# soedinglab/PEnG-motif

Measured on AMD Instinct MI355X. Metric: 4^W pattern z-scores/s + EM PWM-kmer evals/s at W=10; Gbp/s k-mer count, higher is better.
Workload: dtype u32 counts / f32 scores / f32 serial EM sums (f64 tree sums in the throughput EM mode)

## Files before the change

peng-motif_amd/csrc/api.hip:

```cpp
#include <stdarg.h>
#include <stdio.h>
#include <string.h>
#include <stdlib.h>
#include <time.h>

#include <new>

#include "pengk_internal.h"

namespace pengk {

static thread_local char g_err[512] = "";

int fail(int code, const char* fmt, ...) {
  va_list ap;
  va_start(ap, fmt);
  vsnprintf(g_err, sizeof g_err, fmt, ap);
  va_end(ap);
  return code;
}

int hip_fail(hipError_t e, const char* what) {
  return fail(PENGK_ERR_DEVICE, "%s: %s", what, hipGetErrorString(e));
}
// ... 64 lines not shown
  int n = 0;
  hipError_t e = hipGetDeviceCount(&n);
  lap("hipGetDeviceCount (runtime start)");
  if (e != hipSuccess || n <= 0)
    return fail(PENGK_ERR_DEVICE, "pengk_create: no HIP device (%s); this library has no CPU fallback",
                e == hipSuccess ? "device count 0" : hipGetErrorString(e));
  if (device < 0 || device >= n) return fail(PENGK_ERR_ARG, "pengk_create: device %d out of range [0,%d)", device, n);
  PENGK_HIP(hipSetDevice(device));
  hipDeviceProp_t prop;
  PENGK_HIP(hipGetDeviceProperties(&prop, device));
  lap("hipSetDevice + properties");
  if (strncmp(prop.gcnArchName, "gfx950", 6) != 0)
    return fail(PENGK_ERR_DEVICE, "pengk_create: device %d is %s; this build targets gfx950 only", device, prop.gcnArchName);
  pengk_ctx* c = new (std::nothrow) pengk_ctx();
  if (!c) return fail(PENGK_ERR_NOMEM, "pengk_create: out of host memory");
  c->device = device;
  c->num_cu = prop.multiProcessorCount;
  e = hipStreamCreateWithFlags(&c->stream, hipStreamNonBlocking);
  if (e != hipSuccess) {
    delete c;
    return hip_fail(e, "hipStreamCreate");
  }
  c->own_stream = true;
  lap("stream");
  int rc = count_init_device();
  lap("kernel attributes (code object load)");
  if (rc) {
    (void)hipStreamDestroy(c->stream);
    delete c;
    return rc;
  }
  *out = c;
  return PENGK_OK;
}

int pengk_destroy(pengk_ctx* ctx) {
  if (!ctx) return PENGK_OK;
  (void)hipSetDevice(ctx->device);
  (void)hipStreamSynchronize(ctx->stream);
  comm_release(ctx);
  if (ctx->d_defer) (void)hipFree(ctx->d_defer);
  if (ctx->d_em_partials) (void)hipFree(ctx->d_em_partials);
  if (ctx->d_em_tables) (void)hipFree(ctx->d_em_tables);
  if (ctx->d_em_blocks) (void)hipFree(ctx->d_em_blocks);
  if (ctx->d_em_counters) (void)hipFree(ctx->d_em_counters);
  if (ctx->d_em_look) (void)hipFree(ctx->d_em_look);
  if (ctx->d_pair_mids) (void)hipFree(ctx->d_pair_mids);
  for (int l = 0; l < 3; ++l) {
    if (ctx->em_streams[l]) (void)hipStreamDestroy(ctx->em_streams[l]);
    if (ctx->em_join[l]) (void)hipEventDestroy(ctx->em_join[l]);
  }
  if (ctx->em_fork) (void)hipEventDestroy(ctx->em_fork);
  if (ctx->d_misc) (void)hipFree(ctx->d_misc);
  if (ctx->d_keys) (void)hipFree(ctx->d_keys);
  if (ctx->d_iupac_big) (void)hipFree(ctx->d_iupac_big);
  if (ctx->d_bg_partials) (void)hipFree(ctx->d_bg_partials);
  if (ctx->d_count_aux) (void)hipFree(ctx->d_count_aux);
  if (ctx->d_sim) (void)hipFree(ctx->d_sim);
  if (ctx->d_score) (void)hipFree(ctx->d_score);
  if (ctx->d_sites) (void)hipFree(ctx->d_sites);
  if (ctx->own_stream && ctx->stream) (void)hipStreamDestroy(ctx->stream);
  delete ctx;
  return PENGK_OK;
}

int pengk_synchronize(pengk_ctx* ctx) {
  if (!ctx) return fail(PENGK_ERR_ARG, "ctx is NULL");
  PENGK_ENTER(ctx);
  PENGK_HIP(hipStreamSynchronize(ctx->stream));
  return PENGK_OK;
}

int pengk_set_option(pengk_ctx* ctx, const char* name, int64_t value) {
  if (!ctx || !name) return fail(PENGK_ERR_ARG, "pengk_set_option: NULL argument");
  if (strcmp(name, "count_impl") == 0) {
    if (value < 0 || value > 2) return fail(PENGK_ERR_ARG, "count_impl must be 0 (auto), 1 (direct) or 2 (partition)");
    ctx->count_impl = (int)value;
    return PENGK_OK;
  }
  if (strcmp(name, "key_cap_override") == 0) {
    ctx->key_cap_override = (uint64_t)value;
    return PENGK_OK;
  }
  if (strcmp(name, "em_fast") == 0) {
    if (value < 0 || value > 2) return fail(PENGK_ERR_ARG, "em_fast must be 0 (reference terms), 1 (fast) or 2 (serial, bit-exact)");
    ctx->em_fast = (int)value;
    return PENGK_OK;
  }
  if (strcmp(name, "em_serial_scan") == 0) {
    if (value < 2 || value > 3)
      return fail(PENGK_ERR_ARG, "em_serial_scan must be 2 (blocks evaluated ahead of their chain, three launches per iteration) or 3 (two: weights and block evaluation as one kernel); earlier generations: pengk_test_em_generation");
    ctx->em_serial_scan = (int)value;
    return PENGK_OK;
  }
  if (strcmp(name, "em_test_lookback") == 0) {
    if (value < 0 || value > 1000000) return fail(PENGK_ERR_ARG, "em_test_lookback must be 0 (off) or the n of 'every n-th workgroup'");
    ctx->em_test_lookback = (int)value;
    return PENGK_OK;
  }
  if (strcmp(name, "em_test_skew") == 0) {
    if (value < 0 || value > 1000000) return fail(PENGK_ERR_ARG, "em_test_skew must be 0 (off) or the n of 'every n-th block'");
    ctx->em_test_skew = (int)value;
    return PENGK_OK;
  }
  if (strcmp(name, "em_head_blocks") == 0) {
    if (value < 1 || value > 64) return PENGK_ERR_ARG;
    ctx->em_head_blocks = (int)value;
    return PENGK_OK;
  }
  if (strcmp(name, "sweep_pairs") == 0) {
    ctx->sweep_pairs = value != 0;
    return PENGK_OK;
  }
  if (strcmp(name, "em_lean_div") == 0) {
    ctx->em_lean_div = value != 0;
    return PENGK_OK;
  }
  if (strcmp(name, "em_overlap") == 0) {
    if (value < 1 || value > MAX_EM_LANES) return fail(PENGK_ERR_ARG, "em_overlap must be 1 .. %d streams", MAX_EM_LANES);
    ctx->em_overlap = (int)value;
    return PENGK_OK;
  }
  if (strcmp(name, "em_table_budget_mb") == 0) {
    if (value < 0) return fail(PENGK_ERR_ARG, "em_table_budget_mb must be >= 0 (0 = automatic)");
    ctx->em_table_budget_mb = (uint64_t)value;
    return PENGK_OK;
  }
  if (strcmp(name, "iupac_group_bytes") == 0) {
    ctx->iupac_group_bytes = (uint64_t)value;
    return PENGK_OK;
  }
  if (strcmp(name, "sites_record_budget") == 0) {
    if (value < 1) return fail(PENGK_ERR_ARG, "sites_record_budget must be >= 1 record");
    ctx->sites_record_budget = (uint64_t)value;
    return PENGK_OK;
  }
  if (strcmp(name, "scatter_blocks_per_cu") == 0) {
    if (value < 0 || value > 8) return fail(PENGK_ERR_ARG, "scatter_blocks_per_cu must be 0 (default) .. 8");
    ctx->scatter_blocks_per_cu = (int)value;
    return PENGK_OK;
  }
  if (strcmp(name, "n_windows_hint") == 0) {
    ctx->n_windows_hint = (uint64_t)value;
    return PENGK_OK;
  }
  return fail(PENGK_ERR_ARG, "unknown option '%s'", name);
}

int pengk_get_info(pengk_ctx* ctx, const char* name, int64_t* value) {
  if (!ctx || !name || !value) return fail(PENGK_ERR_ARG, "pengk_get_info: NULL argument");
  PENGK_ENTER(ctx);
  if (strcmp(name, "deferred_items") == 0) {
    uint32_t n = 0;
    if (ctx->d_defer) {
      PENGK_HIP(hipMemcpyAsync(&n, ctx->d_defer, sizeof n, hipMemcpyDeviceToHost, ctx->stream));
      PENGK_HIP(hipStreamSynchronize(ctx->stream));
    }
    *value = n;
    return PENGK_OK;
  }
  if (strcmp(name, "sites_record_budget") == 0) {
    *value = (int64_t)ctx->sites_record_budget;
    return PENGK_OK;
  }
  if (strcmp(name, "num_cu") == 0) {
    *value = ctx->num_cu;
    return PENGK_OK;
  }
  static const char* const em_names[4] = {"em_fetched_blocks", "em_mispredicted_blocks", "em_restaged_blocks", "em_restaged_waits"};
  for (int i = 0; i < 4; ++i)
    if (strcmp(name, em_names[i]) == 0) {
      unsigned long long v = 0;
      if (ctx->d_em_counters) {
        PENGK_HIP(hipMemcpyAsync(&v, ctx->d_em_counters + i, sizeof v, hipMemcpyDeviceToHost, ctx->stream));
        PENGK_HIP(hipStreamSynchronize(ctx->stream));
      }
      *value = (int64_t)v;
      return PENGK_OK;
    }
  return fail(PENGK_ERR_ARG, "unknown info '%s'", name);
}

void* pengk_stream(pengk_ctx* ctx) { return ctx ? (void*)ctx->stream : nullptr; }

int pengk_set_stream(pengk_ctx* ctx, void* s) {
  if (!ctx) return fail(PENGK_ERR_ARG, "ctx is NULL");
  PENGK_ENTER(ctx);
  PENGK_HIP(hipStreamSynchronize(ctx->stream));
  if (ctx->own_stream && ctx->stream) PENGK_HIP(hipStreamDestroy(ctx->stream));
  ctx->stream = (hipStream_t)s;
  ctx->own_stream = false;
  return PENGK_OK;
}

int pengk_malloc(pengk_ctx* ctx, size_t bytes, void** d_out) {
  if (!ctx || !d_out) return fail(PENGK_ERR_ARG, "pengk_malloc: NULL argument");
  PENGK_HIP(hipSetDevice(ctx->device));
  hipError_t e = hipMalloc(d_out, bytes ? bytes : 1);
  if (e != hipSuccess) return fail(PENGK_ERR_NOMEM, "hipMalloc(%zu): %s", bytes, hipGetErrorString(e));
  return PENGK_OK;
}

int pengk_free(pengk_ctx* ctx, void* d_ptr) {
  if (!ctx) return fail(PENGK_ERR_ARG, "ctx is NULL");
  PENGK_ENTER(ctx);
  if (d_ptr) {
    PENGK_HIP(hipStreamSynchronize(ctx->stream));
    PENGK_HIP(hipFree(d_ptr));
  }
  return PENGK_OK;
}

int pengk_host_alloc(pengk_ctx* ctx, size_t bytes, void** h_out) {
  if (!ctx || !h_out) return fail(PENGK_ERR_ARG, "pengk_host_alloc: NULL argument");
  PENGK_HIP(hipSetDevice(ctx->device));
  hipError_t e = hipHostMalloc(h_out, bytes ? bytes : 1, hipHostMallocDefault);
  if (e != hipSuccess) return fail(PENGK_ERR_NOMEM, "hipHostMalloc(%zu): %s", bytes, hipGetErrorString(e));
  return PENGK_OK;
}

int pengk_host_free(pengk_ctx* ctx, void* h_ptr) {
  if (!ctx) return fail(PENGK_ERR_ARG, "ctx is NULL");
  PENGK_ENTER(ctx);
  if (h_ptr) {
    PENGK_HIP(hipStreamSynchronize(ctx->stream));
    PENGK_HIP(hipHostFree(h_ptr));
  }
  return PENGK_OK;
}

int pengk_memcpy_h2d(pengk_ctx* ctx, void* d_dst, const void* h_src, size_t bytes) {
  if (!ctx || (bytes && (!d_dst || !h_src))) return fail(PENGK_ERR_ARG, "pengk_memcpy_h2d: NULL argument");
  PENGK_ENTER(ctx);
  PENGK_HIP(hipMemcpyAsync(d_dst, h_src, bytes, hipMemcpyHostToDevice, ctx->stream));
  PENGK_HIP(hipStreamSynchronize(ctx->stream));
  return PENGK_OK;
}

int pengk_warmup(pengk_ctx* ctx) {
  if (!ctx) return fail(PENGK_ERR_ARG, "ctx is NULL");
  PENGK_ENTER(ctx);
  constexpr size_t N = (size_t)4 << 20;
  void* d = nullptr;
  void* h = nullptr;
  hipError_t e = hipMalloc(&d, N);
  if (e == hipSuccess) e = hipHostMalloc(&h, N, hipHostMallocDefault);
  if (e == hipSuccess) e = hipMemcpyAsync(h, d, N, hipMemcpyDeviceToHost, ctx->stream);
  if (e == hipSuccess) e = hipStreamSynchronize(ctx->stream);
  if (h) (void)hipHostFree(h);
  if (d) (void)hipFree(d);
  if (e != hipSuccess) return hip_fail(e, "pengk_warmup");
  return warm_code_objects();
}

int pengk_memcpy_d2h(pengk_ctx* ctx, void* h_dst, const void* d_src, size_t bytes) {
  if (!ctx || (bytes && (!h_dst || !d_src))) return fail(PENGK_ERR_ARG, "pengk_memcpy_d2h: NULL argument");
  PENGK_ENTER(ctx);
  PENGK_HIP(hipMemcpyAsync(h_dst, d_src, bytes, hipMemcpyDeviceToHost, ctx->stream));
  PENGK_HIP(hipStreamSynchronize(ctx->stream));
  return PENGK_OK;
}

int pengk_memset(pengk_ctx* ctx, void* d_dst, int byte, size_t bytes) {
  if (!ctx || (bytes && !d_dst)) return fail(PENGK_ERR_ARG, "pengk_memset: NULL argument");
  PENGK_ENTER(ctx);
  PENGK_HIP(hipMemsetAsync(d_dst, byte, bytes, ctx->stream));
  return PENGK_OK;
}

int pengk_timer_create(pengk_ctx* ctx, void** out) {
  if (!ctx || !out) return fail(PENGK_ERR_ARG, "pengk_timer_create: NULL argument");
  PENGK_ENTER(ctx);
  hipEvent_t ev;
  PENGK_HIP(hipEventCreate(&ev));
  *out = (void*)ev;
  return PENGK_OK;
}
int pengk_timer_record(pengk_ctx* ctx, void* t) {
  if (!ctx || !t) return fail(PENGK_ERR_ARG, "pengk_timer_record: NULL argument");
  PENGK_ENTER(ctx);
  PENGK_HIP(hipEventRecord((hipEvent_t)t, ctx->stream));
  return PENGK_OK;
}
int pengk_timer_elapsed_ms(pengk_ctx* ctx, void* a, void* b, float* ms) {
  if (!ctx || !a || !b || !ms) return fail(PENGK_ERR_ARG, "pengk_timer_elapsed_ms: NULL argument");
  PENGK_ENTER(ctx);
  PENGK_HIP(hipEventSynchronize((hipEvent_t)b));
  PENGK_HIP(hipEventElapsedTime(ms, (hipEvent_t)a, (hipEvent_t)b));
  return PENGK_OK;
}
int pengk_timer_destroy(pengk_ctx* ctx, void* t) {
  (void)ctx;
  if (t) PENGK_HIP(hipEventDestroy((hipEvent_t)t));
  return PENGK_OK;
}

int pengk_set_sequences(pengk_ctx* ctx, const uint64_t* d_words, uint64_t n_words, const uint64_t* d_items,
                        uint64_t n_items, int W, int item_windows, uint64_t max_bin_bound, int all_whole) {
  if (!ctx) return fail(PENGK_ERR_ARG, "ctx is NULL");
  if (!valid_w(W)) return fail(PENGK_ERR_ARG, "pattern length %d unsupported (even, %d..%d)", W, PENGK_MIN_W, PENGK_MAX_W);
  if (item_windows < PENGK_MIN_ITEM_WINDOWS || item_windows > 65535)
    return fail(PENGK_ERR_ARG, "item_windows %d out of range [%d,65535]", item_windows, PENGK_MIN_ITEM_WINDOWS);
  if (!d_words || n_words < (PENGK_FRONT_PAD_BASES / 32) + 2) return fail(PENGK_ERR_ARG, "packed stream missing or too short");
  if (n_items && !d_items) return fail(PENGK_ERR_ARG, "items missing");
  if (n_items >= (1ull << 32)) return fail(PENGK_ERR_RANGE, "too many scan items for one shard (%llu)", (unsigned long long)n_items);
  ctx->d_words = d_words;
  ctx->n_words = n_words;
  ctx->d_items = d_items;
// ... 222 lines not shown
```

peng-motif_amd/csrc/count.hip:

```cpp
#include <stdlib.h>

#include <type_traits>

#include "pengk_internal.h"

namespace pengk {

namespace {

constexpr uint32_t INVALID_ID = 0xFFFFFFFFu;

__device__ __forceinline__ uint32_t funnel(uint32_t hi, uint32_t lo, uint32_t shift) {
  return __builtin_amdgcn_alignbit(hi, lo, shift);
}

template <int W>
struct Geo {
  static constexpr int P = ((3 * W - 3 + 15) / 16) * 16;
  static constexpr uint32_t MASK = (1u << (2 * W)) - 1u;
  static constexpr int TOP = 2 * (W - 1);
  static constexpr int PER = (32 - 2 * W) / 2 + 1;
  static constexpr int NVIEW = (W - 1 + PER - 1) / PER;
};

// ... 138 lines not shown
        const uint32_t hi = words32[wi + 1];
        ++wi;
        const uint32_t chunk = funnel(hi, lo, shift);
        lo = hi;
        pchunk = chunk;
#pragma unroll
        for (int u = 0; u < 16; ++u) {
          const int b = ch * 16 + u;
          const uint32_t c = (chunk >> (2 * u)) & 3u;
          id = (id >> 2) | (c << G::TOP);
          rc = ((rc << 2) & G::MASK) | (c ^ 3u);
          bgc.head(id, b - (G::P - (W - 1)), live && !cont && nw > 0);
          if (b >= W - 1) {
            const uint32_t can = BOTH ? min(id, rc) : id;
            bool match = false;
#pragma unroll
            for (int d = 1; d <= W - 1; ++d)
              if (b - d >= W - 1) match |= (can == ring[(u - d) & 15]);
            dirty |= match;
            ring[u] = (cont && !match) ? can : INVALID_ID;
          }
        }
      }
      if (cont && dirty) {
        const uint32_t slot = atomicAdd(&defer[0], 1u);
        defer[1 + slot] = it;
        nw = 0;
      }
    } else {
      wi += (G::P / 16) - 1;
      lo = words32[wi];
      const uint32_t hi = words32[wi + 1];
      ++wi;
      const uint32_t chunk = funnel(hi, lo, shift);
      lo = hi;
      pchunk = chunk;
#pragma unroll
      for (int u = 0; u < 16; ++u) {
        const uint32_t c = (chunk >> (2 * u)) & 3u;
        id = (id >> 2) | (c << G::TOP);
        rc = ((rc << 2) & G::MASK) | (c ^ 3u);
        bgc.head(id, u - (17 - W), live && nw > 0);
      }
    }

    const uint32_t nw_scan = BG ? nw_all : nw;
    uint32_t nw_max = nw_scan;
#pragma unroll
    for (int off = 32; off > 0; off >>= 1) nw_max = max(nw_max, (uint32_t)__shfl_xor((int)nw_max, off, 64));
    uint32_t nxt = (0u < nw_scan) ? words32[wi + 1] : 0u;
    uint32_t rprev = revcomp16(pchunk);
    for (uint32_t t0 = 0; t0 < nw_max; t0 += 16) {
      const uint32_t hi = nxt;
      ++wi;
      nxt = (t0 + 16u < nw_scan) ? words32[wi + 1] : 0u;
      const uint32_t chunk = funnel(hi, lo, shift);
      lo = hi;
      const uint32_t rchunk = BOTH ? revcomp16(chunk) : 0u;
      uint32_t view[G::NVIEW], rview[G::NVIEW];
#pragma unroll
      for (int j = 0; j < G::NVIEW; ++j) {
        view[j] = funnel(chunk, pchunk, 2u * (uint32_t)(j * G::PER + 17 - W));
        rview[j] = BOTH ? funnel(rprev, rchunk, 2u * (uint32_t)(j * G::PER + 17 - W)) : 0u;
      }
      auto body = [&](auto full_tag) {
        constexpr bool FULL = decltype(full_tag)::value;
#pragma unroll
        for (int u = 0; u < 16; ++u) {
          uint32_t id_u, rc_u = 0;
          if (u >= W - 1) {
            id_u = __builtin_amdgcn_ubfe(chunk, 2u * (uint32_t)(u - (W - 1)), 2u * W);
            if (BOTH) rc_u = __builtin_amdgcn_ubfe(rchunk, 2u * (uint32_t)(15 - u), 2u * W);
          } else {
            const int j = u / G::PER, k = W - 2 - u, jr = k / G::PER;
            id_u = __builtin_amdgcn_ubfe(view[j], 2u * (uint32_t)(u - j * G::PER), 2u * W);
            if (BOTH) rc_u = __builtin_amdgcn_ubfe(rview[jr], 2u * (uint32_t)(k - jr * G::PER), 2u * W);
          }
          const uint32_t can = BOTH ? min(id_u, rc_u) : id_u;
#ifdef PENGK_ABLATE_NOSUPPRESS
          const uint32_t key = can;
#else
          const uint32_t key = Suppress<W>::apply(can, ring, u);
#endif
          ring[u] = key;
          if (FULL) {
            if (BG && (u & 1)) {
              const uint32_t v4 = u >= 3 ? __builtin_amdgcn_ubfe(chunk, 2u * (uint32_t)(u - 3), 8u)
                                         : funnel(chunk, pchunk, 2u * (uint32_t)(13 + u)) & 0xFFu;
              bgc.kmer4(v4);
            }
            emit.full(key);
          } else {
            bgc.kmer3(id_u, t0 + (uint32_t)u < nw_all);
            emit.masked(key, key != INVALID_ID && t0 + (uint32_t)u < nw);
          }
        }
      };
      if (__all((t0 + 16u <= nw && nw == nw_all) ? 1 : 0)) body(std::true_type{});
      else body(std::false_type{});
      pchunk = chunk;
      rprev = rchunk;
    }
  }

#pragma unroll
  for (int off = 32; off > 0; off >>= 1) my_windows += __shfl_down(my_windows, off, 64);
  if ((threadIdx.x & 63u) == 0 && my_windows) atomicAdd(ltot, my_windows);
}

struct DirectEmit {
  uint32_t* __restrict__ hist;
  __device__ __forceinline__ void masked(uint32_t key, bool active) const {
    if (active) __hip_atomic_fetch_add(&hist[key], 1u, __ATOMIC_RELAXED, __HIP_MEMORY_SCOPE_AGENT);
  }
  __device__ __forceinline__ void full(uint32_t key) const { masked(key, key != INVALID_ID); }
};

template <int W, bool BOTH, bool BG>
__global__ __launch_bounds__(256) void count_kernel(const uint32_t* __restrict__ words32,
                                                    const uint64_t* __restrict__ items, uint32_t n_items,
                                                    uint32_t* __restrict__ hist,
                                                    unsigned long long* __restrict__ ltot,
                                                    uint32_t* __restrict__ defer, uint32_t* __restrict__ bg_partials) {
  bg_begin<BG>();
  if (BG) __syncthreads();
  DirectEmit e{hist};
  scan_items<W, BOTH, BG>(words32, items, n_items, ltot, defer, e);
  bg_end<BG>(bg_partials);
}

constexpr int RING_CAP = 128;
constexpr int GROUP = RING_CAP / 2;
constexpr uint32_t KEY_INVALID = 0xFFFFu;
constexpr int PAYLOAD_BITS = 15;

template <int W, int NBITS>
struct KeySplit {
  static constexpr int S = ((2 * W - NBITS) / 2) & ~1;
  static constexpr uint32_t LOW = (1u << S) - 1u;
  static constexpr uint32_t NB = 1u << NBITS;
  __host__ __device__ static inline uint32_t bucket(uint32_t id) { return (id >> S) & (NB - 1u); }
  __host__ __device__ static inline uint32_t payload(uint32_t id) {
#if defined(__HIP_DEVICE_COMPILE__)
    uint32_t r;
    asm("v_bfi_b32 %0, %1, %2, %3" : "=v"(r) : "s"(LOW), "v"(id), "v"(id >> NBITS));
    return r;
#else
    return (id & LOW) | ((id >> NBITS) & ~LOW);
#endif
  }
  __host__ __device__ static inline uint32_t join(uint32_t b, uint32_t p, uint32_t  = 0) {
    return (p & LOW) | (b << S) | ((p >> S) << (S + NBITS));
  }
  __host__ __device__ static inline bool valid(uint32_t p) { return p != KEY_INVALID; }
};

#ifndef PENGK_W12_L1_BITS
#define PENGK_W12_L1_BITS 4
#endif
struct Split12L1 {
  static constexpr int NBITS = PENGK_W12_L1_BITS;
  static constexpr uint32_t NB = 1u << NBITS;
  static constexpr uint32_t PBITS = 24 - NBITS;
  __host__ __device__ static inline uint32_t bucket(uint32_t id) { return (id >> 8) & (NB - 1u); }
  __host__ __device__ static inline uint32_t payload(uint32_t id) { return (id & 0xFFu) | ((id >> (8 + NBITS)) << 8); }
  __host__ __device__ static inline uint32_t join(uint32_t b1, uint32_t p1, uint32_t  = 0) { return (p1 & 0xFFu) | (b1 << 8) | ((p1 >> 8) << (8 + NBITS)); }
  __host__ __device__ static inline bool valid(uint32_t p1) { return p1 < (1u << PBITS); }
};
struct Split12L2 {
  static constexpr int NBITS = 9 - Split12L1::NBITS;
  static constexpr uint32_t NB = 1u << NBITS;
  __host__ __device__ static inline uint32_t bucket(uint32_t p1) { return (p1 >> 8) & (NB - 1u); }
  __host__ __device__ static inline uint32_t payload(uint32_t p1) { return (p1 & 0xFFu) | ((p1 >> (8 + NBITS)) << 8); }
  __host__ __device__ static inline uint32_t join(uint32_t b2, uint32_t p2, uint32_t outer) {
    const uint32_t p1 = (p2 & 0xFFu) | (b2 << 8) | ((p2 >> 8) << (8 + NBITS));
    return Split12L1::join(outer, p1);
  }
  __host__ __device__ static inline bool valid(uint32_t p2) { return p2 != KEY_INVALID; }
};

struct Split14L1 {
  static constexpr int NBITS = 4;
  static constexpr uint32_t NB = 16;
  __host__ __device__ static inline uint32_t bucket(uint32_t id) { return (id >> 10) & 15u; }
  __host__ __device__ static inline uint32_t payload(uint32_t id) { return (id & 0x3FFu) | ((id >> 14) << 10); }
  __host__ __device__ static inline uint32_t join(uint32_t b1, uint32_t p1, uint32_t  = 0) { return (p1 & 0x3FFu) | (b1 << 10) | ((p1 >> 10) << 14); }
  __host__ __device__ static inline bool valid(uint32_t p1) { return p1 < (1u << 24); }
};
struct Split14L2 {
  static constexpr int NBITS = 4;
  static constexpr uint32_t NB = 16;
  __host__ __device__ static inline uint32_t bucket(uint32_t p1) { return (p1 >> 9) & 15u; }
  __host__ __device__ static inline uint32_t payload(uint32_t p1) { return (p1 & 0x1FFu) | ((p1 >> 13) << 9); }
  __host__ __device__ static inline uint32_t join(uint32_t b2, uint32_t p2, uint32_t outer) {
    return Split14L1::join(outer, (p2 & 0x1FFu) | (b2 << 9) | ((p2 >> 9) << 13));
  }
  __host__ __device__ static inline bool valid(uint32_t p2) { return p2 < (1u << 20); }
};
struct Split14L3 {
  static constexpr int NBITS = 5;
  static constexpr uint32_t NB = 32;
  __host__ __device__ static inline uint32_t bucket(uint32_t p2) { return (p2 >> 8) & 31u; }
  __host__ __device__ static inline uint32_t payload(uint32_t p2) { return (p2 & 0xFFu) | ((p2 >> 13) << 8); }
  __host__ __device__ static inline uint32_t join(uint32_t b3, uint32_t p3, uint32_t outer) {
    return Split14L2::join(outer & 15u, (p3 & 0xFFu) | (b3 << 8) | ((p3 >> 8) << 13), outer >> 4);
  }
  __host__ __device__ static inline bool valid(uint32_t p3) { return p3 != KEY_INVALID; }
};

template <class E>
struct ScatterRowT {
  E ring[RING_CAP];
  uint32_t fill4;
};
typedef ScatterRowT<uint16_t> ScatterRow;
template <int NBITS, int WPW, class E = uint16_t>
struct ScatterShared {
  static constexpr int NB = 1 << NBITS;
  ScatterRowT<E> row[WPW][NB];
};

template <int NBITS, int WPW, class E = uint16_t>
__device__ __forceinline__ ScatterShared<NBITS, WPW, E>& scatter_lds() {
  __shared__ ScatterShared<NBITS, WPW, E> sh;
  return sh;
}

template <class KS, int NBITS, int WPW = 4, class E = uint16_t>
struct ScatterEmit {
  static constexpr int NB = 1 << NBITS;
  static constexpr uint32_t ES = (uint32_t)sizeof(E);
  static constexpr uint32_t ESH = ES == 2u ? 1u : 2u;
  static constexpr uint32_t PAD = ES == 2u ? KEY_INVALID : 0xFFFFFFFFu;
  typedef ScatterRowT<E> Row;
  static_assert(GROUP == 64, "a group is one entry per lane");
  static_assert(RING_CAP == 128, "byte 0 of the counter addresses the ring");
  E* __restrict__ keys;
  uint32_t slice_cap;
  uint32_t* __restrict__ slice_fill;
  uint32_t* __restrict__ hist;
  uint32_t wave, lane, wave_global;
  uint32_t outer;

  static __device__ __forceinline__ void init_lds() {
    ScatterShared<NBITS, WPW, E>& sh = scatter_lds<NBITS, WPW, E>();
    static_assert(sizeof(Row) == ES * RING_CAP + 4, "row = ring + counter");
    uint32_t* w = reinterpret_cast<uint32_t*>(&sh.row[0][0]);
    for (uint32_t i = threadIdx.x; i < (uint32_t)WPW * NB * (sizeof(Row) / 4u); i += blockDim.x)
      w[i] = (i % (uint32_t)(sizeof(Row) / 4u)) == (uint32_t)(ES * RING_CAP / 4u) ? 0u : 0xFFFFFFFFu;
  }

  typedef __attribute__((address_space(3))) uint32_t lds_u32_t;
  typedef __attribute__((address_space(3))) E lds_e_t;
  typedef __attribute__((address_space(1))) E global_e_t;

  __device__ __forceinline__ void flush_triggered(unsigned long long trig, uint32_t row, uint32_t b, uint32_t s4) {
    asm volatile("");
    const uint32_t g4 = s4 - 4u * (uint32_t)(GROUP - 1);
    const uint32_t src = row + ((g4 >> (2u - ESH)) & (ES * (uint32_t)GROUP));
    const uint32_t dst = b * (ES * slice_cap) + (g4 >> (2u - ESH));
    const unsigned long long fits = __builtin_amdgcn_ballot_w64(g4 + 4u * GROUP <= 4u * slice_cap);
    unsigned long long todo = trig & fits;
    unsigned long long over = trig & ~fits;
    while (todo) {
      const int p = __builtin_ctzll(todo);
      todo &= todo - 1;
      const uint32_t s_src = (uint32_t)__builtin_amdgcn_readlane((int)src, p);
      const uint32_t s_dst = (uint32_t)__builtin_amdgcn_readlane((int)dst, p);
      uint32_t v = *(lds_e_t*)(uintptr_t)(s_src + ES * lane);
      asm volatile("" : "+v"(v));
      global_e_t* out = (global_e_t*)((char*)region + s_dst);
      __builtin_nontemporal_store((E)v, &out[lane]);
    }
    while (over) {
      const int p = __builtin_ctzll(over);
      over &= over - 1;
      const uint32_t s_src = (uint32_t)__builtin_amdgcn_readlane((int)src, p);
      const uint32_t fb = (uint32_t)__builtin_amdgcn_readlane((int)b, p);
      const uint32_t v = *(lds_e_t*)(uintptr_t)(s_src + ES * lane);
      if (KS::valid(v)) __hip_atomic_fetch_add(&hist[KS::join(fb, v, outer)], 1u, __ATOMIC_RELAXED, __HIP_MEMORY_SCOPE_AGENT);
    }
  }

  uint32_t rowbase = 0;
  __device__ __forceinline__ void bind() {
    rowbase = (uint32_t)(uintptr_t)(__attribute__((address_space(3))) char*)&scatter_lds<NBITS, WPW, E>().row[wave][0];
    asm volatile("" : "+v"(rowbase));
    region = keys + (size_t)wave_global * NB * slice_cap;
  }
  E* region = nullptr;

  __device__ __forceinline__ uint32_t append(uint32_t b, uint32_t key, uint32_t& row) const {
    row = b * (uint32_t)sizeof(Row) + rowbase;
    const uint32_t s4 = __hip_atomic_fetch_add((lds_u32_t*)(uintptr_t)(row + ES * RING_CAP), 4u, __ATOMIC_RELAXED,
                                               __HIP_MEMORY_SCOPE_WORKGROUP);
    *(lds_e_t*)(uintptr_t)(row + ((s4 >> (2u - ESH)) & (ES * RING_CAP - 1u))) = (E)KS::payload(key);
    return s4;
  }

  __device__ __forceinline__ void full(uint32_t key) {
    const uint32_t b = KS::bucket(key);
    uint32_t row;
    const uint32_t s4 = append(b, key, row);
    const unsigned long long trig = __builtin_amdgcn_ballot_w64((s4 & 0xFFu) == 4u * (uint32_t)(GROUP - 1));
    if (trig) flush_triggered(trig, row, b, s4);
  }

  __device__ __forceinline__ void masked(uint32_t key, bool active) {
    const uint32_t b = KS::bucket(key);
    uint32_t s4 = 0, row = 0;
    if (active) s4 = append(b, key, row);
    const unsigned long long trig = __builtin_amdgcn_ballot_w64(active && (s4 & 0xFFu) == 4u * (uint32_t)(GROUP - 1));
    if (trig) flush_triggered(trig, row, b, s4);
  }

  __device__ __forceinline__ void drain() {
    __builtin_amdgcn_wave_barrier();
    uint32_t row = 0, s4_last = 0;
    bool padded = false;
    if (lane < (uint32_t)NB) {
      row = lane * (uint32_t)sizeof(Row) + rowbase;
      const uint32_t c4 = __hip_atomic_load((lds_u32_t*)(uintptr_t)(row + ES * RING_CAP), __ATOMIC_RELAXED, __HIP_MEMORY_SCOPE_WAVEFRONT);
      const uint32_t r = (c4 >> 2) & (uint32_t)(GROUP - 1);
      if (r) {
        for (uint32_t i = r; i < (uint32_t)GROUP; ++i)
          *(lds_e_t*)(uintptr_t)(row + (((c4 >> (2u - ESH)) & (ES * RING_CAP - 1u)) + ES * (i - r))) = (E)PAD;
        s4_last = c4 + 4u * ((uint32_t)GROUP - r) - 4u;
        padded = true;
      }
      const uint32_t full = ((c4 >> 2) + (uint32_t)(GROUP - 1)) & ~(uint32_t)(GROUP - 1);
      slice_fill[(size_t)wave_global * NB + lane] = full < slice_cap ? full : slice_cap;
    }
    __builtin_amdgcn_wave_barrier();
    const unsigned long long trig = __builtin_amdgcn_ballot_w64(padded);
    if (trig) flush_triggered(trig, row, lane, s4_last);
  }
};

#ifndef PENGK_SCATTER_WPW
#define PENGK_SCATTER_WPW 4
#endif
constexpr int SCATTER_WPW = PENGK_SCATTER_WPW;
template <int W, bool BOTH, int NBITS, bool BG>
__global__ __launch_bounds__(64 * SCATTER_WPW) void count_scatter_kernel(const uint32_t* __restrict__ words32,
                                                            const uint64_t* __restrict__ items, uint32_t n_items,
                                                            uint16_t* __restrict__ keys, uint32_t slice_cap,
                                                            uint32_t* __restrict__ slice_fill, uint32_t* __restrict__ hist,
                                                            unsigned long long* __restrict__ ltot,
                                                            uint32_t* __restrict__ defer,
                                                            uint32_t* __restrict__ bg_partials) {
  static_assert(2 * W - NBITS == PAYLOAD_BITS, "payload must be 15 bits");
  ScatterEmit<KeySplit<W, NBITS>, NBITS, SCATTER_WPW>::init_lds();
  bg_begin<BG>();
  __syncthreads();
  const uint32_t wave = (uint32_t)__builtin_amdgcn_readfirstlane((int)(threadIdx.x >> 6));
  ScatterEmit<KeySplit<W, NBITS>, NBITS, SCATTER_WPW> e{keys, slice_cap, slice_fill, hist, wave, threadIdx.x & 63u, blockIdx.x * (uint32_t)SCATTER_WPW + wave, 0u};
  e.bind();
  scan_items<W, BOTH, BG>(words32, items, n_items, ltot, defer, e);
  e.drain();
  bg_end<BG>(bg_partials);
}

#ifndef PENGK_SCATTER12_WPW
#define PENGK_SCATTER12_WPW 3
#endif
constexpr int SCATTER12_WPW = PENGK_SCATTER12_WPW;
#ifndef PENGK_SCATTER12L1_WPW
#define PENGK_SCATTER12L1_WPW (PENGK_W12_L1_BITS == 5 ? 3 : 4)
#endif
constexpr int SCATTER12L1_WPW = PENGK_SCATTER12L1_WPW;
typedef ScatterEmit<Split12L1, Split12L1::NBITS, SCATTER12L1_WPW, uint32_t> Scatter12Emit;

template <bool BOTH, bool BG>
__global__ __launch_bounds__(64 * SCATTER12L1_WPW) void count_scatter12_kernel(const uint32_t* __restrict__ words32,
                                                              const uint64_t* __restrict__ items, uint32_t n_items,
                                                              uint32_t* __restrict__ keys, uint32_t slice_cap,
                                                              uint32_t* __restrict__ slice_fill, uint32_t* __restrict__ hist,
                                                              unsigned long long* __restrict__ ltot,
                                                              uint32_t* __restrict__ defer, uint32_t* __restrict__ bg_partials) {
  Scatter12Emit::init_lds();
  bg_begin<BG>();
  __syncthreads();
  const uint32_t wave = (uint32_t)__builtin_amdgcn_readfirstlane((int)(threadIdx.x >> 6));
  Scatter12Emit e{keys, slice_cap, slice_fill, hist, wave, threadIdx.x & 63u, blockIdx.x * (uint32_t)SCATTER12L1_WPW + wave, 0u};
  e.bind();
  scan_items<12, BOTH, BG>(words32, items, n_items, ltot, defer, e);
  e.drain();
  bg_end<BG>(bg_partials);
}

__global__ __launch_bounds__(256) void count_rescatter12_kernel(const uint32_t* __restrict__ keys1, uint32_t cap1,
                                                                const uint32_t* __restrict__ fill1, uint32_t n_slices1,
                                                                uint32_t bpb1, uint16_t* __restrict__ keys2, uint32_t cap2,
                                                                uint32_t* __restrict__ fill2, uint32_t* __restrict__ hist) {
  ScatterEmit<Split12L2, Split12L2::NBITS>::init_lds();
  __syncthreads();
  const uint32_t b1 = blockIdx.x / bpb1, j = blockIdx.x % bpb1;
  const uint32_t wave = (uint32_t)__builtin_amdgcn_readfirstlane((int)(threadIdx.x >> 6)), lane = threadIdx.x & 63u;
  ScatterEmit<Split12L2, Split12L2::NBITS> e{keys2, cap2, fill2, hist, wave, lane, blockIdx.x * 4u + wave, b1};
  e.bind();
  const uint32_t per = (n_slices1 + bpb1 - 1) / bpb1;
  const uint32_t first = j * per, last = min(n_slices1, first + per);
  for (uint32_t s = first + wave; s < last; s += 4) {
    const uint32_t n = fill1[(size_t)s * Split12L1::NB + b1];
    const uint32_t* src = keys1 + ((size_t)s * Split12L1::NB + b1) * cap1;
    typedef uint32_t u4 __attribute__((ext_vector_type(4)));
    const u4 pad = {0xFFFFFFFFu, 0xFFFFFFFFu, 0xFFFFFFFFu, 0xFFFFFFFFu};
    const u4* src4 = reinterpret_cast<const u4*>(src);
    const uint32_t n4 = n / 4u;
    u4 nxt = lane < n4 ? __builtin_nontemporal_load(&src4[lane]) : pad;
    for (uint32_t i = 0; i < n4; i += 64) {
      const u4 k = nxt;
      nxt = (i + 64u + lane < n4) ? __builtin_nontemporal_load(&src4[i + 64u + lane]) : pad;
      e.full(k.x);
      e.full(k.y);
      e.full(k.z);
      e.full(k.w);
    }
  }
  e.drain();
}

typedef ScatterEmit<Split14L1, Split14L1::NBITS, SCATTER12L1_WPW, uint32_t> Scatter14Emit;

template <bool BOTH, bool BG>
__global__ __launch_bounds__(64 * SCATTER12L1_WPW) void count_scatter14_kernel(const uint32_t* __restrict__ words32,
                                                              const uint64_t* __restrict__ items, uint32_t n_items,
                                                              uint32_t* __restrict__ keys, uint32_t slice_cap,
                                                              uint32_t* __restrict__ slice_fill, uint32_t* __restrict__ hist,
                                                              unsigned long long* __restrict__ ltot,
                                                              uint32_t* __restrict__ defer, uint32_t* __restrict__ bg_partials) {
  Scatter14Emit::init_lds();
  bg_begin<BG>();
  __syncthreads();
  const uint32_t wave = (uint32_t)__builtin_amdgcn_readfirstlane((int)(threadIdx.x >> 6));
  Scatter14Emit e{keys, slice_cap, slice_fill, hist, wave, threadIdx.x & 63u, blockIdx.x * (uint32_t)SCATTER12L1_WPW + wave, 0u};
  e.bind();
  scan_items<14, BOTH, BG>(words32, items, n_items, ltot, defer, e);
  e.drain();
  bg_end<BG>(bg_partials);
}

template <class KS, class E_OUT, uint32_t NB_IN>
__global__ __launch_bounds__(256) void count_rescatter_kernel(const uint32_t* __restrict__ keys_in, uint32_t cap_in,
                                                              const uint32_t* __restrict__ fill_in, uint32_t n_slices_in,
                                                              uint32_t slices_per_group, uint32_t bpb, E_OUT* __restrict__ keys_out,
                                                              uint32_t cap_out, uint32_t* __restrict__ fill_out,
                                                              uint32_t* __restrict__ hist) {
  typedef ScatterEmit<KS, KS::NBITS, 4, E_OUT> Emit;
  Emit::init_lds();
  __syncthreads();
  const uint32_t o = blockIdx.x / bpb, j = blockIdx.x % bpb;
  const uint32_t b_in = slices_per_group ? o % NB_IN : o;
  const uint32_t slice0 = slices_per_group ? (o / NB_IN) * slices_per_group : 0u;
  const uint32_t n_in = slices_per_group ? slices_per_group : n_slices_in;
  const uint32_t wave = (uint32_t)__builtin_amdgcn_readfirstlane((int)(threadIdx.x >> 6)), lane = threadIdx.x & 63u;
  Emit e{keys_out, cap_out, fill_out, hist, wave, lane, blockIdx.x * 4u + wave, o};
  e.bind();
  const uint32_t per = (n_in + bpb - 1) / bpb;
  const uint32_t first = j * per, last = min(n_in, first + per);
  for (uint32_t t = first + wave; t < last; t += 4) {
    const uint32_t sl = slice0 + t;
    const uint32_t n = fill_in[(size_t)sl * NB_IN + b_in];
    typedef uint32_t u4 __attribute__((ext_vector_type(4)));
    const u4 pad = {0xFFFFFFFFu, 0xFFFFFFFFu, 0xFFFFFFFFu, 0xFFFFFFFFu};
    const u4* src4 = reinterpret_cast<const u4*>(keys_in + ((size_t)sl * NB_IN + b_in) * cap_in);
    const uint32_t n4 = n / 4u;
    u4 nxt = lane < n4 ? __builtin_nontemporal_load(&src4[lane]) : pad;
    for (uint32_t i = 0; i < n4; i += 64) {
      const u4 k = nxt;
      nxt = (i + 64u + lane < n4) ? __builtin_nontemporal_load(&src4[i + 64u + lane]) : pad;
      e.full(k.x);
      e.full(k.y);
      e.full(k.z);
      e.full(k.w);
    }
  }
  e.drain();
}

__global__ __launch_bounds__(256) void count_gather14_kernel(const uint32_t* __restrict__ temp, uint32_t* __restrict__ hist) {
  const uint32_t np = 1u << 28;
  for (uint32_t x = blockIdx.x * blockDim.x + threadIdx.x; x < np; x += gridDim.x * blockDim.x) {
    const uint32_t p1 = Split14L1::payload(x), p2 = Split14L2::payload(p1);
    const uint32_t fb = (Split14L1::bucket(x) * Split14L2::NB + Split14L2::bucket(p1)) * Split14L3::NB + Split14L3::bucket(p2);
    const uint32_t v = temp[((size_t)fb << PAYLOAD_BITS) | Split14L3::payload(p2)];
    if (v) hist[x] += v;
  }
}

__global__ __launch_bounds__(1024) void count_hist_kernel(const uint16_t* __restrict__ keys, uint32_t slice_cap,
                                                          uint32_t n_slices, uint32_t nb,
                                                          const uint32_t* __restrict__ slice_fill, uint32_t bpb,
                                                          uint32_t* __restrict__ temp, uint32_t slices_per_outer) {
  extern __shared__ uint32_t h[];
  const uint32_t f = blockIdx.x / bpb, j = blockIdx.x % bpb;
  const uint32_t b = slices_per_outer ? f % nb : f;
  const uint32_t slice0 = slices_per_outer ? (f / nb) * slices_per_outer : 0u;
  if (slices_per_outer) n_slices = slices_per_outer;
  for (uint32_t i = threadIdx.x; i < (1u << PAYLOAD_BITS); i += blockDim.x) h[i] = 0;
  __syncthreads();
  const uint32_t per = (n_slices + bpb - 1) / bpb;
  const uint32_t first = slice0 + j * per, last = slice0 + min(n_slices, j * per + per);
  const uint32_t wave = threadIdx.x >> 6, lane = threadIdx.x & 63u;
  uint32_t fill_next = first + wave < last ? slice_fill[(size_t)(first + wave) * nb + b] : 0u;
  for (uint32_t s = first + wave; s < last; s += 16) {
    const uint32_t n8 = fill_next >> 3;
    if (s + 16 < last) fill_next = slice_fill[(size_t)(s + 16) * nb + b];
    const uint4* src = reinterpret_cast<const uint4*>(keys + ((size_t)s * nb + b) * slice_cap);
    auto count8 = [&](const uint4& v) {
      const uint32_t k[8] = {v.x & 0xFFFFu, v.x >> 16, v.y & 0xFFFFu, v.y >> 16, v.z & 0xFFFFu, v.z >> 16, v.w & 0xFFFFu, v.w >> 16};
#pragma unroll
      for (int q = 0; q < 8; ++q)
        if (k[q] < (1u << PAYLOAD_BITS)) atomicAdd(&h[k[q]], 1u);
    };
    uint32_t i = lane;
    for (; i + 448 < n8; i += 512) {
      uint4 v[8];
#pragma unroll
      for (int q = 0; q < 8; ++q) {
        typedef uint32_t u32x4 __attribute__((ext_vector_type(4)));
        const u32x4 t = __builtin_nontemporal_load(reinterpret_cast<const u32x4*>(&src[i + 64 * q]));
        v[q] = make_uint4(t.x, t.y, t.z, t.w);
      }
#pragma unroll
      for (int q = 0; q < 8; ++q) count8(v[q]);
    }
    if (i < n8) {
      uint4 v[7];
#pragma unroll
      for (int q = 0; q < 7; ++q) {
        typedef uint32_t u32x4 __attribute__((ext_vector_type(4)));
        const u32x4 ones = {0xFFFFFFFFu, 0xFFFFFFFFu, 0xFFFFFFFFu, 0xFFFFFFFFu};
        const u32x4 t = i + 64u * q < n8 ? __builtin_nontemporal_load(reinterpret_cast<const u32x4*>(&src[i + 64 * q])) : ones;
        v[q] = make_uint4(t.x, t.y, t.z, t.w);
      }
#pragma unroll
      for (int q = 0; q < 7; ++q) count8(v[q]);
    }
  }
  __syncthreads();
  uint32_t* dst = temp + ((size_t)f << PAYLOAD_BITS);
  for (uint32_t i = threadIdx.x; i < (1u << PAYLOAD_BITS); i += blockDim.x) {
    const uint32_t v = h[i];
    if (v) __hip_atomic_fetch_add(&dst[i], v, __ATOMIC_RELAXED, __HIP_MEMORY_SCOPE_AGENT);
  }
}

__global__ __launch_bounds__(256) void count_gather12_kernel(const uint32_t* __restrict__ temp, uint32_t* __restrict__ hist) {
  const uint32_t np = 1u << 24;
  for (uint32_t x = blockIdx.x * blockDim.x + threadIdx.x; x < np; x += gridDim.x * blockDim.x) {
    const uint32_t p1 = Split12L1::payload(x);
    const uint32_t fb = Split12L1::bucket(x) * Split12L2::NB + Split12L2::bucket(p1);
    const uint32_t v = temp[((size_t)fb << PAYLOAD_BITS) | Split12L2::payload(p1)];
    if (v) hist[x] += v;
  }
}

template <int W, int NBITS>
__global__ __launch_bounds__(256) void count_gather_kernel(const uint32_t* __restrict__ temp, uint32_t np,
                                                           uint32_t* __restrict__ hist) {
  using KS = KeySplit<W, NBITS>;
  for (uint32_t x = blockIdx.x * blockDim.x + threadIdx.x; x < np; x += gridDim.x * blockDim.x) {
    const uint32_t v = temp[((size_t)KS::bucket(x) << PAYLOAD_BITS) | KS::payload(x)];
    if (v) hist[x] += v;
  }
}

__device__ __forceinline__ uint32_t base_at(const uint32_t* __restrict__ words32, uint64_t g) {
  return (words32[g >> 4] >> (2u * (uint32_t)(g & 15u))) & 3u;
}

__global__ __launch_bounds__(64) void count_fixup_kernel(const uint32_t* __restrict__ words32,
                                                         const uint64_t* __restrict__ items, int W, int both,
                                                         uint32_t* __restrict__ hist,
                                                         const uint32_t* __restrict__ defer) {
  const uint32_t n = defer[0];
  const uint32_t mask = (1u << (2 * W)) - 1u;
  const int top = 2 * (W - 1);
  for (uint32_t q = blockIdx.x * blockDim.x + threadIdx.x; q < n; q += gridDim.x * blockDim.x) {
    const uint32_t it = defer[1 + q];
    const uint64_t rec = items[it];
    const uint32_t nw = (uint32_t)((rec >> ITEM_NW_SHIFT) & ITEM_NW_MASK);
    const uint64_t ws = rec & ITEM_WS_MASK;
    uint32_t j = it;
    while ((items[j] >> ITEM_CONT_SHIFT) & 1ull) --j;
    const uint64_t head = items[j] & ITEM_WS_MASK;
    uint64_t back = 8ull * (uint64_t)(W - 1);
    for (;;) {
      const uint64_t p0 = (ws - head > back) ? ws - back : head;
      bool certified = (p0 == head);
      uint32_t ring[16];
      for (int i = 0; i < 16; ++i) ring[i] = INVALID_ID;
      uint32_t id = 0, rc = 0;
      for (int b = 0; b < W - 1; ++b) {
        const uint32_t c = base_at(words32, p0 + b);
        id = (id >> 2) | (c << top);
        rc = ((rc << 2) & mask) | (c ^ 3u);
      }
      uint32_t clean = 0;
      bool ok = true;
      for (uint64_t t = p0; t < ws + nw; ++t) {
        const uint32_t c = base_at(words32, t + (uint64_t)(W - 1));
        id = (id >> 2) | (c << top);
        rc = ((rc << 2) & mask) | (c ^ 3u);
        const uint32_t can = both ? min(id, rc) : id;
        bool match = false;
        for (int d = 1; d <= W - 1; ++d) match |= (ring[(uint32_t)(t - d) & 15u] == can);
        if (t < ws) {
          clean = match ? 0u : clean + 1u;
          if (clean >= 2u * (uint32_t)(W - 1)) certified = true;
        } else {
          if (!certified) {
            ok = false;
            break;
          }
          if (!match) __hip_atomic_fetch_add(&hist[can], 1u, __ATOMIC_RELAXED, __HIP_MEMORY_SCOPE_AGENT);
        }
        ring[(uint32_t)t & 15u] = match ? INVALID_ID : can;
      }
      if (ok) break;
      back *= 4ull;
    }
  }
}

__global__ __launch_bounds__(256) void mirror_kernel(uint32_t* __restrict__ hist, int W, uint32_t np) {
  for (uint32_t x = blockIdx.x * blockDim.x + threadIdx.x; x < np; x += gridDim.x * blockDim.x) {
    const uint32_t r = revcomp32(x, W);
    if (x > r) hist[x] = hist[r];
  }
}

__global__ __launch_bounds__(256) void bg_count_kernel(const uint32_t* __restrict__ words32,
                                                       const uint64_t* __restrict__ items, uint32_t n_items, int W,
                                                       unsigned long long* __restrict__ out ) {
  __shared__ uint32_t h3[64][65];
  __shared__ uint32_t hfirst[20];
  for (int i = threadIdx.x; i < 64 * 65; i += blockDim.x) (&h3[0][0])[i] = 0;
  if (threadIdx.x < 20) hfirst[threadIdx.x] = 0;
  __syncthreads();
  const uint32_t col = threadIdx.x & 63u;
  for (uint32_t it = blockIdx.x * blockDim.x + threadIdx.x; it < n_items; it += gridDim.x * blockDim.x) {
    const uint64_t rec = items[it];
    const uint32_t nw = (uint32_t)((rec >> ITEM_NW_SHIFT) & ITEM_NW_MASK);
    const uint64_t ws = rec & ITEM_WS_MASK;
    const bool cont = ((rec >> ITEM_CONT_SHIFT) & 1ull) != 0;
    const bool last = (it + 1 == n_items) || (((items[it + 1] >> ITEM_CONT_SHIFT) & 1ull) == 0);
    const uint32_t nb = nw + (last ? (uint32_t)(W - 1) : 0u);
    uint32_t y = 0;
    uint32_t pos = 2;
    if (cont) {
      y = (base_at(words32, ws - 2) << 2) | base_at(words32, ws - 1);
    } else {
      pos = 0;
    }
    for (uint32_t b = 0; b < nb; ++b) {
      const uint32_t c = base_at(words32, ws + b);
      y = ((y << 2) | c) & 63u;
      if (pos >= 2) {
        atomicAdd(&h3[y][col], 1u);
      } else if (pos == 1) {
        atomicAdd(&hfirst[4 + (y & 15u)], 1u);
        pos = 2;
      } else {
        atomicAdd(&hfirst[c], 1u);
        pos = 1;
      }
    }
  }
  __syncthreads();
  if (threadIdx.x < 64) {
    unsigned long long s = 0;
    for (int i = 0; i < 64; ++i) s += h3[threadIdx.x][i];
    if (s) atomicAdd(&out[threadIdx.x], s);
  } else if (threadIdx.x < 84) {
    const uint32_t v = hfirst[threadIdx.x - 64];
    if (v) atomicAdd(&out[threadIdx.x], (unsigned long long)v);
  }
}

__global__ void bg_finish_kernel(const unsigned long long* __restrict__ raw, unsigned long long* __restrict__ out) {
  const int t = threadIdx.x;
  __shared__ unsigned long long n2[16];
  if (t < 16) {
    unsigned long long s = raw[64 + 4 + t];
    for (int c = 0; c < 4; ++c) s += raw[c * 16 + t];
    n2[t] = s;
    out[4 + t] = s;
  }
  __syncthreads();
  if (t < 4) {
    unsigned long long s = raw[64 + t];
    for (int b = 0; b < 4; ++b) s += n2[b * 4 + t];
    out[t] = s;
  }
  if (t < 64) out[20 + t] = raw[t];
}

__global__ void bg_finish_fused_kernel(const uint32_t* __restrict__ partials, uint32_t n_blocks,
                                       unsigned long long* __restrict__ out) {
  __shared__ unsigned long long raw[84];
  __shared__ unsigned long long n3[64];
  __shared__ unsigned long long n2[16];
  __shared__ unsigned long long part[12][84];
  const int t = threadIdx.x;
  {
    const int bin = t % 84, strand = t / 84;
    if (strand < 12) {
      unsigned long long acc[8] = {0, 0, 0, 0, 0, 0, 0, 0};
      uint32_t b = strand;
      for (; b + 31u * 12u < n_blocks; b += 32u * 12u) {
        uint32_t v[32];
#pragma unroll
        for (uint32_t j = 0; j < 32u; ++j) v[j] = partials[(size_t)(b + 12u * j) * 84 + bin];
#pragma unroll
        for (uint32_t j = 0; j < 32u; ++j) acc[j & 7u] += v[j];
      }
      for (; b < n_blocks; b += 12) acc[0] += partials[(size_t)b * 84 + bin];
      part[strand][bin] = ((acc[0] + acc[1]) + (acc[2] + acc[3])) + ((acc[4] + acc[5]) + (acc[6] + acc[7]));
    }
  }
  __syncthreads();
  if (t < 84) {
    unsigned long long s = 0;
    for (int k = 0; k < 12; ++k) s += part[k][t];
    raw[t] = s;
  }
  __syncthreads();
  if (t < 64) {
    const int d0 = t >> 4, d1 = (t >> 2) & 3, d2 = t & 3;
    n3[t] = raw[d0 | (d1 << 2) | (d2 << 4)];
    out[20 + t] = n3[t];
  }
  __syncthreads();
  if (t < 16) {
    const int a = t >> 2, b = t & 3;
    unsigned long long s = raw[68 + (a | (b << 2))];
    for (int c = 0; c < 4; ++c) s += n3[c * 16 + t];
    n2[t] = s;
    out[4 + t] = s;
  }
  __syncthreads();
  if (t < 4) {
    unsigned long long s = raw[64 + t];
    for (int b = 0; b < 4; ++b) s += n2[b * 4 + t];
    out[t] = s;
  }
}

__global__ __launch_bounds__(128) void bg_model_kernel(const unsigned long long* __restrict__ n, int K, float a0, float a1, float a2,
                                                       float* __restrict__ V) {
  __shared__ float cnt[84];
  __shared__ float v[84];
  const int t = threadIdx.x;
  const float alpha[3] = {a0, a1, a2};
  const int off[3] = {0, 4, 20};
  if (t < 84) cnt[t] = (float)n[t];
  __shared__ float base_f;
  if (t == 0) {
    unsigned long long base_counts = 0;
    for (int y = 0; y < 4; ++y) base_counts += n[y];
    base_f = (float)base_counts;
  }
  __syncthreads();
  if (t < 4) v[t] = (cnt[t] + alpha[0] * 0.25f) / (base_f + alpha[0]);
  __syncthreads();
  for (int k = 1; k <= K; ++k) {
    const int ny = 1 << (2 * (k + 1));
    const int yk = 1 << (2 * k);
    if (t < ny) v[off[k] + t] = (cnt[off[k] + t] + alpha[k] * v[off[k - 1] + t % yk]) / (cnt[off[k - 1] + t / 4] + alpha[k]);
    __syncthreads();
    if (t < ny / 4) {
      float* g = v + off[k] + 4 * t;
      float factor = 0.0f;
      for (int a = 0; a < 4; ++a) factor += g[a];
      for (int a = 0; a < 4; ++a) g[a] /= factor;
    }
    __syncthreads();
  }
  const int used = off[K] + (1 << (2 * (K + 1)));
  if (t < 84) V[t] = t < used ? v[t] : 0.0f;
}

__device__ __forceinline__ uint64_t mix64(uint64_t x) {
  x ^= x >> 30;
  x *= 0xBF58476D1CE4E5B9ull;
  x ^= x >> 27;
  x *= 0x94D049BB133111EBull;
  x ^= x >> 31;
  return x;
}

__global__ __launch_bounds__(256) void synth_words_kernel(uint64_t seed, uint64_t seq0, uint64_t n_seq, uint32_t L,
                                                          uint64_t* __restrict__ words, uint64_t n_words) {
  const uint64_t motif = 2ull | (1ull << 2) | (3ull << 4) | (2ull << 6) | (0ull << 8) | (2ull << 10) | (3ull << 12) |
                         (1ull << 14) | (0ull << 16) | (3ull << 18);
  const uint64_t total = n_seq * (uint64_t)L;
  for (uint64_t w = blockIdx.x * (uint64_t)blockDim.x + threadIdx.x; w < n_words; w += (uint64_t)gridDim.x * blockDim.x) {
    uint64_t v = 0;
    for (int k = 0; k < 32; ++k) {
      const uint64_t g = w * 32 + k;
      if (g < PENGK_FRONT_PAD_BASES) continue;
      const uint64_t li = g - PENGK_FRONT_PAD_BASES;
      if (li >= total) break;
      const uint64_t n = seq0 + li / L;
      const uint32_t j = (uint32_t)(li % L);
      uint64_t d = mix64(seed + 0x9E3779B97F4A7C15ull * (n * (uint64_t)L + j + 1)) >> 62;
      if (L >= 10 && mix64(seed ^ 0xA5A5A5A5ull ^ (n + 1)) % 10 == 0) {
        const uint64_t q = mix64(seed ^ 0x5A5A5A5Aull ^ (n + 1)) % (L - 9);
        if (j >= q && j < q + 10) d = (motif >> (2 * (j - q))) & 3ull;
      }
      v |= d << (2 * k);
    }
    words[w] = v;
  }
}

__global__ __launch_bounds__(256) void synth_items_kernel(uint64_t n_seq, uint32_t L, int W, uint32_t M,
                                                          uint64_t* __restrict__ items) {
  const uint64_t nwin = (uint64_t)L - W + 1;
  const uint64_t per = (nwin + M - 1) / M;
  const uint64_t n = n_seq * per;
  for (uint64_t i = blockIdx.x * (uint64_t)blockDim.x + threadIdx.x; i < n; i += (uint64_t)gridDim.x * blockDim.x) {
    const uint64_t s = i / per;
    const uint64_t f = (i % per) * M;
    const uint64_t nw = nwin - f < M ? nwin - f : M;
    items[i] = (PENGK_FRONT_PAD_BASES + s * L + f) | (nw << ITEM_NW_SHIFT) | ((uint64_t)(f ? 1 : 0) << ITEM_CONT_SHIFT);
  }
}

#define PENGK_LAUNCH_BB(KERNEL, TARGS, both, bg, grid, block, ...)                                              \
  do {                                                                                                         \
    if (both) {                                                                                                \
      if (bg) hipLaunchKernelGGL((KERNEL<TARGS(true, true)>), grid, block, 0, ctx->stream, __VA_ARGS__);        \
      else hipLaunchKernelGGL((KERNEL<TARGS(true, false)>), grid, block, 0, ctx->stream, __VA_ARGS__);          \
    } else {                                                                                                   \
      if (bg) hipLaunchKernelGGL((KERNEL<TARGS(false, true)>), grid, block, 0, ctx->stream, __VA_ARGS__);       \
      else hipLaunchKernelGGL((KERNEL<TARGS(false, false)>), grid, block, 0, ctx->stream, __VA_ARGS__);         \
    }                                                                                                          \
  } while (0)

int bg_partials_buffer(pengk_ctx* ctx, uint32_t blocks, uint32_t** out) {
  int rc = ensure_scratch(ctx, &ctx->d_bg_partials, &ctx->bg_partials_bytes, (size_t)blocks * 84 * sizeof(uint32_t));
  *out = (uint32_t*)ctx->d_bg_partials;
  return rc;
}

int bg_finish_fused(pengk_ctx* ctx, uint32_t blocks, uint64_t* d_bg) {
  hipLaunchKernelGGL(bg_finish_fused_kernel, dim3(1), dim3(1024), 0, ctx->stream, (const uint32_t*)ctx->d_bg_partials, blocks,
                     (unsigned long long*)d_bg);
  PENGK_HIP(hipGetLastError());
  return PENGK_OK;
}

template <int W>
int launch_direct_w(pengk_ctx* ctx, int both, uint32_t* d_counts, uint64_t* d_ltot, uint32_t n_items, uint64_t* d_bg) {
  const uint32_t* w32 = (const uint32_t*)ctx->d_words;
  const uint32_t blocks_needed = (n_items + 255) / 256;
  const uint32_t max_blocks = (uint32_t)ctx->num_cu * 8u;
  const uint32_t blocks = blocks_needed < max_blocks ? blocks_needed : max_blocks;
  unsigned long long* lt = (unsigned long long*)d_ltot;
  uint32_t* bgp = nullptr;
  if (d_bg) {
    int rc = bg_partials_buffer(ctx, blocks, &bgp);
    if (rc) return rc;
  }
#define TA_DIRECT(B, G) W, B, G
  PENGK_LAUNCH_BB(count_kernel, TA_DIRECT, both, d_bg != nullptr, dim3(blocks), dim3(256), w32, ctx->d_items, n_items, d_counts,
                  lt, ctx->d_defer, bgp);
#undef TA_DIRECT
  PENGK_HIP(hipGetLastError());
  return d_bg ? bg_finish_fused(ctx, blocks, d_bg) : PENGK_OK;
}

template <int W>
int launch_partition_w(pengk_ctx* ctx, int both, uint32_t* d_counts, uint64_t* d_ltot, uint32_t n_items, uint64_t* d_bg) {
  constexpr int NBITS = 2 * W - PAYLOAD_BITS;
  constexpr uint32_t NB = 1u << NBITS;
  const uint32_t np = 1u << (2 * W);
  const uint32_t* w32 = (const uint32_t*)ctx->d_words;
  constexpr uint32_t TPB = 64u * SCATTER_WPW;
  const uint32_t blocks_needed = (n_items + TPB - 1) / TPB;
  constexpr uint32_t lds_per_wg = (uint32_t)(sizeof(ScatterShared<NBITS, SCATTER_WPW>) + sizeof(BgLds) + 511u) & ~511u;
  const uint32_t per_cu = ctx->scatter_blocks_per_cu ? (uint32_t)ctx->scatter_blocks_per_cu : (160u * 1024u) / lds_per_wg;
  const uint32_t max_blocks = (uint32_t)ctx->num_cu * per_cu;
  const uint32_t blocks = blocks_needed < max_blocks ? blocks_needed : max_blocks;
  const uint32_t n_waves = blocks * (uint32_t)SCATTER_WPW;
  uint64_t windows = ctx->n_windows_hint ? ctx->n_windows_hint : ctx->n_items * (uint64_t)ctx->item_windows;
  const uint64_t share = windows / ((uint64_t)NB * n_waves);
  uint64_t cap64 = share + share / 2 + 512;
  if (ctx->key_cap_override) cap64 = ctx->key_cap_override;
  cap64 = (cap64 + 63) / 64 * 64;
  if (cap64 * NB >= (1ull << 31))
    return fail(PENGK_ERR_RANGE, "shard too large for the partitioned count (slice of %llu keys)", (unsigned long long)cap64);
  const uint32_t slice_cap = (uint32_t)cap64;
  int rc = ensure_scratch(ctx, &ctx->d_keys, &ctx->keys_bytes, (size_t)NB * n_waves * slice_cap * sizeof(uint16_t));
  if (rc) return rc;
  const size_t fill_words = ((size_t)NB * n_waves + 63) / 64 * 64;
  const size_t aux_need = fill_words * sizeof(uint32_t) + (size_t)np * sizeof(uint32_t);
  rc = ensure_scratch(ctx, &ctx->d_count_aux, &ctx->count_aux_bytes, aux_need);
  if (rc) return rc;
  uint32_t* slice_fill = (uint32_t*)ctx->d_count_aux;
  uint32_t* temp = slice_fill + fill_words;
  PENGK_HIP(hipMemsetAsync(ctx->d_count_aux, 0, aux_need, ctx->stream));
  unsigned long long* lt = (unsigned long long*)d_ltot;
  uint16_t* keys = (uint16_t*)ctx->d_keys;
  uint32_t* bgp = nullptr;
  if (d_bg) {
    rc = bg_partials_buffer(ctx, blocks, &bgp);
    if (rc) return rc;
  }
#define TA_SCATTER(B, G) W, B, NBITS, G
  PENGK_LAUNCH_BB(count_scatter_kernel, TA_SCATTER, both, d_bg != nullptr, dim3(blocks), dim3(TPB), w32, ctx->d_items, n_items,
                  keys, slice_cap, slice_fill, d_counts, lt, ctx->d_defer, bgp);
#undef TA_SCATTER
  PENGK_HIP(hipGetLastError());
  if (d_bg) {
    rc = bg_finish_fused(ctx, blocks, d_bg);
    if (rc) return rc;
  }
  uint32_t bpb = ((uint32_t)ctx->num_cu * 2u + NB - 1) / NB;
  const uint64_t per_bucket = windows / NB + 1;
  const uint32_t useful = (uint32_t)((per_bucket + 65535) / 65536);
  if (bpb > useful) bpb = useful;
  if (bpb > n_waves) bpb = n_waves;
  if (bpb < 1) bpb = 1;
  hipLaunchKernelGGL(count_hist_kernel, dim3(NB * bpb), dim3(1024), 4 << PAYLOAD_BITS, ctx->stream, keys, slice_cap, n_waves,
                     NB, slice_fill, bpb, temp, 0u);
  PENGK_HIP(hipGetLastError());
  const uint32_t gb = (np + 255) / 256 < 2048u ? (np + 255) / 256 : 2048u;
  hipLaunchKernelGGL((count_gather_kernel<W, NBITS>), dim3(gb), dim3(256), 0, ctx->stream, temp, np, d_counts);
  PENGK_HIP(hipGetLastError());
  return PENGK_OK;
}

int launch_partition12(pengk_ctx* ctx, int both, uint32_t* d_counts, uint64_t* d_ltot, uint32_t n_items, uint64_t* d_bg) {
  const uint32_t np = 1u << 24;
  const uint32_t* w32 = (const uint32_t*)ctx->d_words;
  constexpr uint32_t TPB1 = 64u * SCATTER12L1_WPW;
  constexpr uint32_t NB1 = Split12L1::NB, NB2 = Split12L2::NB;
  const uint32_t blocks_needed = (n_items + TPB1 - 1) / TPB1;
  constexpr uint32_t lds_per_wg1 = (uint32_t)(sizeof(ScatterShared<Split12L1::NBITS, SCATTER12L1_WPW, uint32_t>) + sizeof(BgLds) + 511u) & ~511u;
  const uint32_t max_blocks = (uint32_t)ctx->num_cu * ((160u * 1024u) / lds_per_wg1);
  const uint32_t blocks1 = blocks_needed < max_blocks ? blocks_needed : max_blocks;
  const uint32_t n_waves1 = blocks1 * (uint32_t)SCATTER12L1_WPW;
  const uint64_t windows = ctx->n_windows_hint ? ctx->n_windows_hint : ctx->n_items * (uint64_t)ctx->item_windows;
  uint64_t share1 = windows / ((uint64_t)NB1 * n_waves1);
  uint64_t cap1_64 = share1 + share1 / 2 + 256;
  if (ctx->key_cap_override) cap1_64 = ctx->key_cap_override;
  cap1_64 = (cap1_64 + 63) / 64 * 64;
  uint32_t bpb1 = ((uint32_t)ctx->num_cu * 8u + NB1 - 1u) / NB1;
  if (bpb1 > n_waves1) bpb1 = n_waves1;
  if (bpb1 < 1) bpb1 = 1;
  const uint32_t blocks2 = NB1 * bpb1;
  const uint32_t n_waves2 = blocks2 * 4u;
  uint64_t share2 = windows / ((uint64_t)NB2 * n_waves2);
  uint64_t cap2_64 = share2 + share2 / 2 + 512;
  if (ctx->key_cap_override) cap2_64 = ctx->key_cap_override;
  cap2_64 = (cap2_64 + 63) / 64 * 64;
  if (cap1_64 * NB1 >= (1ull << 30) || cap2_64 * NB2 >= (1ull << 31)) return fail(
      PENGK_ERR_RANGE, "shard too large for the partitioned count");
  const uint32_t cap1 = (uint32_t)cap1_64, cap2 = (uint32_t)cap2_64;
  const size_t bytes1 = (size_t)n_waves1 * NB1 * cap1 * sizeof(uint32_t);
  const size_t bytes2 = (size_t)n_waves2 * NB2 * cap2 * sizeof(uint16_t);
  int rc = ensure_scratch(ctx, &ctx->d_keys, &ctx->keys_bytes, bytes1 + bytes2);
  if (rc) return rc;
  uint32_t* keys1 = (uint32_t*)ctx->d_keys;
  uint16_t* keys2 = (uint16_t*)((char*)ctx->d_keys + bytes1);
  const size_t fill1_words = ((size_t)n_waves1 * NB1 + 63) / 64 * 64, fill2_words = ((size_t)n_waves2 * NB2 + 63) / 64 * 64;
  const size_t aux_need = (fill1_words + fill2_words + (size_t)np) * sizeof(uint32_t);
  rc = ensure_scratch(ctx, &ctx->d_count_aux, &ctx->count_aux_bytes, aux_need);
  if (rc) return rc;
  uint32_t* fill1 = (uint32_t*)ctx->d_count_aux;
  uint32_t* fill2 = fill1 + fill1_words;
  uint32_t* temp = fill2 + fill2_words;
  PENGK_HIP(hipMemsetAsync(ctx->d_count_aux, 0, aux_need, ctx->stream));
  unsigned long long* lt = (unsigned long long*)d_ltot;
  uint32_t* bgp = nullptr;
  if (d_bg) {
    rc = bg_partials_buffer(ctx, blocks1, &bgp);
    if (rc) return rc;
  }
#define TA_S12(B, G) B, G
  PENGK_LAUNCH_BB(count_scatter12_kernel, TA_S12, both, d_bg != nullptr, dim3(blocks1), dim3(TPB1), w32, ctx->d_items, n_items, keys1,
                  cap1, fill1, d_counts, lt, ctx->d_defer, bgp);
#undef TA_S12
  PENGK_HIP(hipGetLastError());
  if (d_bg) {
    rc = bg_finish_fused(ctx, blocks1, d_bg);
    if (rc) return rc;
  }
  hipLaunchKernelGGL(count_rescatter12_kernel, dim3(blocks2), dim3(256), 0, ctx->stream, keys1, cap1, fill1, n_waves1, bpb1, keys2,
                     cap2, fill2, d_counts);
  PENGK_HIP(hipGetLastError());
  hipLaunchKernelGGL(count_hist_kernel, dim3(512), dim3(1024), 4 << PAYLOAD_BITS, ctx->stream, keys2, cap2, n_waves2, NB2, fill2, 1u,
                     temp, bpb1 * 4u);
  PENGK_HIP(hipGetLastError());
  hipLaunchKernelGGL(count_gather12_kernel, dim3(4096), dim3(256), 0, ctx->stream, temp, d_counts);
  PENGK_HIP(hipGetLastError());
  return PENGK_OK;
}

int launch_partition14(pengk_ctx* ctx, int both, uint32_t* d_counts, uint64_t* d_ltot, uint32_t n_items, uint64_t* d_bg) {
  const size_t np = (size_t)1 << 28;
  const uint32_t* w32 = (const uint32_t*)ctx->d_words;
  constexpr uint32_t TPB1 = 64u * SCATTER12L1_WPW;
  constexpr uint32_t NB1 = Split14L1::NB, NB2 = Split14L2::NB, NB3 = Split14L3::NB;
  static_assert(NB1 * NB2 * NB3 == 8192, "2^13 LDS histograms");
  const uint32_t blocks_needed = (n_items + TPB1 - 1) / TPB1;
  constexpr uint32_t lds_per_wg1 = (uint32_t)(sizeof(ScatterShared<Split14L1::NBITS, SCATTER12L1_WPW, uint32_t>) + sizeof(BgLds) + 511u) & ~511u;
  const uint32_t max_blocks = (uint32_t)ctx->num_cu * ((160u * 1024u) / lds_per_wg1);
  const uint32_t blocks1 = blocks_needed < max_blocks ? blocks_needed : max_blocks;
  const uint32_t n_waves1 = blocks1 * (uint32_t)SCATTER12L1_WPW;
  const uint64_t windows = ctx->n_windows_hint ? ctx->n_windows_hint : ctx->n_items * (uint64_t)ctx->item_windows;
  auto cap_of = [&](uint64_t slices, uint64_t slack) {
    uint64_t c = windows / slices;
    c = c + c / 2 + slack;
    if (ctx->key_cap_override) c = ctx->key_cap_override;
    return (c + 63) / 64 * 64;
  };
  uint32_t bpb1 = ((uint32_t)ctx->num_cu * 8u + NB1 - 1u) / NB1;
  if (bpb1 > n_waves1) bpb1 = n_waves1;
  if (bpb1 < 1) bpb1 = 1;
  const uint32_t blocks2 = NB1 * bpb1, n_waves2 = blocks2 * 4u;
  uint32_t bpb2 = ((uint32_t)ctx->num_cu * 8u + NB1 * NB2 - 1u) / (NB1 * NB2);
  if (bpb2 > bpb1 * 4u) bpb2 = bpb1 * 4u;
  if (bpb2 < 1) bpb2 = 1;
  const uint32_t blocks3 = NB1 * NB2 * bpb2, n_waves3 = blocks3 * 4u;
  const uint64_t cap1_64 = cap_of((uint64_t)NB1 * n_waves1, 256), cap2_64 = cap_of((uint64_t)NB2 * n_waves2, 256), cap3_64 = cap_of((uint64_t)NB3 * n_waves3, 256);
  if (cap1_64 * NB1 >= (1ull << 30) || cap2_64 * NB2 >= (1ull << 30) || cap3_64 * NB3 >= (1ull << 31))
    return fail(PENGK_ERR_RANGE, "shard too large for the partitioned count");
  const uint32_t cap1 = (uint32_t)cap1_64, cap2 = (uint32_t)cap2_64, cap3 = (uint32_t)cap3_64;
  const size_t bytes1 = (size_t)n_waves1 * NB1 * cap1 * sizeof(uint32_t);
  const size_t bytes2 = (size_t)n_waves2 * NB2 * cap2 * sizeof(uint32_t);
  const size_t bytes3 = (size_t)n_waves3 * NB3 * cap3 * sizeof(uint16_t);
  int rc = ensure_scratch(ctx, &ctx->d_keys, &ctx->keys_bytes, bytes1 + bytes2 + bytes3);
  if (rc) return rc;
  uint32_t* keys1 = (uint32_t*)ctx->d_keys;
  uint32_t* keys2 = (uint32_t*)((char*)ctx->d_keys + bytes1);
  uint16_t* keys3 = (uint16_t*)((char*)ctx->d_keys + bytes1 + bytes2);
  const size_t f1 = ((size_t)n_waves1 * NB1 + 63) / 64 * 64, f2 = ((size_t)n_waves2 * NB2 + 63) / 64 * 64,
               f3 = ((size_t)n_waves3 * NB3 + 63) / 64 * 64;
  const size_t aux_need = (f1 + f2 + f3 + np) * sizeof(uint32_t);
  rc = ensure_scratch(ctx, &ctx->d_count_aux, &ctx->count_aux_bytes, aux_need);
  if (rc) return rc;
  uint32_t* fill1 = (uint32_t*)ctx->d_count_aux;
  uint32_t* fill2 = fill1 + f1;
  uint32_t* fill3 = fill2 + f2;
  uint32_t* temp = fill3 + f3;
  PENGK_HIP(hipMemsetAsync(ctx->d_count_aux, 0, aux_need, ctx->stream));
  unsigned long long* lt = (unsigned long long*)d_ltot;
  uint32_t* bgp = nullptr;
  if (d_bg) {
    rc = bg_partials_buffer(ctx, blocks1, &bgp);
    if (rc) return rc;
  }
#define TA_S14(B, G) B, G
  PENGK_LAUNCH_BB(count_scatter14_kernel, TA_S14, both, d_bg != nullptr, dim3(blocks1), dim3(TPB1), w32, ctx->d_items, n_items, keys1,
                  cap1, fill1, d_counts, lt, ctx->d_defer, bgp);
#undef TA_S14
  PENGK_HIP(hipGetLastError());
  if (d_bg) {
    rc = bg_finish_fused(ctx, blocks1, d_bg);
    if (rc) return rc;
  }
  hipLaunchKernelGGL((count_rescatter_kernel<Split14L2, uint32_t, NB1>), dim3(blocks2), dim3(256), 0, ctx->stream, keys1, cap1, fill1,
                     n_waves1, 0u, bpb1, keys2, cap2, fill2, d_counts);
  PENGK_HIP(hipGetLastError());
  hipLaunchKernelGGL((count_rescatter_kernel<Split14L3, uint16_t, NB2>), dim3(blocks3), dim3(256), 0, ctx->stream, keys2, cap2, fill2,
                     n_waves2, bpb1 * 4u, bpb2, keys3, cap3, fill3, d_counts);
  PENGK_HIP(hipGetLastError());
  hipLaunchKernelGGL(count_hist_kernel, dim3(8192), dim3(1024), 4 << PAYLOAD_BITS, ctx->stream, keys3, cap3, n_waves3, NB3, fill3, 1u,
                     temp, bpb2 * 4u);
  PENGK_HIP(hipGetLastError());
  hipLaunchKernelGGL(count_gather14_kernel, dim3(8192), dim3(256), 0, ctx->stream, temp, d_counts);
  PENGK_HIP(hipGetLastError());
  return PENGK_OK;
}

template <int W>
int launch_count_w(pengk_ctx* ctx, int both, uint32_t* d_counts, uint64_t* d_ltot, uint64_t* d_bg) {
  const uint32_t n_items = (uint32_t)ctx->n_items;
  if (n_items == 0) {
    if (d_bg) PENGK_HIP(hipMemsetAsync(d_bg, 0, 84 * sizeof(uint64_t), ctx->stream));
    return PENGK_OK;
  }
  if constexpr (W < 4) {
    if (d_bg) {
      const int rc_bg = launch_bg_count(ctx, d_bg);
      if (rc_bg) return rc_bg;
      d_bg = nullptr;
    }
  }
  int impl = ctx->count_impl;
  constexpr bool can_partition = (W == 8 || W == 10 || W == 12 || W == 14);
  if (impl == 0) impl = can_partition ? 2 : 1;
  if (impl == 2 && !can_partition) return fail(PENGK_ERR_UNSUPPORTED, "partitioned count is built for W = 8 .. 14 only");
  int rc;
  if constexpr (W == 14) {
    rc = impl == 2 ? launch_partition14(ctx, both, d_counts, d_ltot, n_items, d_bg)
                   : launch_direct_w<W>(ctx, both, d_counts, d_ltot, n_items, d_bg);
  } else if constexpr (W == 12) {
    rc = impl == 2 ? launch_partition12(ctx, both, d_counts, d_ltot, n_items, d_bg)
                   : launch_direct_w<W>(ctx, both, d_counts, d_ltot, n_items, d_bg);
  } else if constexpr (can_partition) {
    rc = impl == 2 ? launch_partition_w<W>(ctx, both, d_counts, d_ltot, n_items, d_bg)
                   : launch_direct_w<W>(ctx, both, d_counts, d_ltot, n_items, d_bg);
  } else {
    rc = launch_direct_w<W>(ctx, both, d_counts, d_ltot, n_items, d_bg);
  }
  if (rc) return rc;
  hipLaunchKernelGGL(count_fixup_kernel, dim3(64), dim3(64), 0, ctx->stream, (const uint32_t*)ctx->d_words, ctx->d_items, W,
                     both, d_counts, ctx->d_defer);
  PENGK_HIP(hipGetLastError());
  return PENGK_OK;
}

}

int count_init_device() {
  PENGK_HIP(hipFuncSetAttribute((const void*)count_hist_kernel, hipFuncAttributeMaxDynamicSharedMemorySize, 4 << PAYLOAD_BITS));
  return PENGK_OK;
}

int launch_count(pengk_ctx* ctx, int both, uint32_t* d_counts, uint64_t* d_ltot, uint64_t* d_bg) {
  const int W = ctx->W;
  const size_t np = (size_t)1 << (2 * W);
  {
    const size_t need = (ctx->n_items + 2) * sizeof(uint32_t);
    size_t have = ctx->defer_cap * sizeof(uint32_t);
    if (have < need) {
      int rc = ensure_scratch(ctx, (void**)&ctx->d_defer, &have, need);
      if (rc) return rc;
      ctx->defer_cap = have / sizeof(uint32_t);
    }
  }
  PENGK_HIP(hipMemsetAsync(ctx->d_defer, 0, sizeof(uint32_t), ctx->stream));
  PENGK_HIP(hipMemsetAsync(d_counts, 0, np * sizeof(uint32_t), ctx->stream));
  PENGK_HIP(hipMemsetAsync(d_ltot, 0, sizeof(uint64_t), ctx->stream));
  switch (W) {
    case 2: return launch_count_w<2>(ctx, both, d_counts, d_ltot, d_bg);
    case 4: return launch_count_w<4>(ctx, both, d_counts, d_ltot, d_bg);
    case 6: return launch_count_w<6>(ctx, both, d_counts, d_ltot, d_bg);
    case 8: return launch_count_w<8>(ctx, both, d_counts, d_ltot, d_bg);
    case 10: return launch_count_w<10>(ctx, both, d_counts, d_ltot, d_bg);
    case 12: return launch_count_w<12>(ctx, both, d_counts, d_ltot, d_bg);
    case 14: return launch_count_w<14>(ctx, both, d_counts, d_ltot, d_bg);
    default: return fail(PENGK_ERR_ARG, "pattern length %d unsupported", W);
  }
}

int launch_mirror(pengk_ctx* ctx, int W, uint32_t* d_counts) {
  const uint32_t np = 1u << (2 * W);
  const uint32_t blocks = (np + 255) / 256 < 4096u ? (np + 255) / 256 : 4096u;
  hipLaunchKernelGGL(mirror_kernel, dim3(blocks), dim3(256), 0, ctx->stream, d_counts, W, np);
  PENGK_HIP(hipGetLastError());
  return PENGK_OK;
}

int launch_bg_count(pengk_ctx* ctx, uint64_t* d_bg) {
  int rc = ensure_scratch(ctx, &ctx->d_misc, &ctx->misc_bytes, 84 * sizeof(uint64_t));
  if (rc) return rc;
  unsigned long long* raw = (unsigned long long*)ctx->d_misc;
  PENGK_HIP(hipMemsetAsync(raw, 0, 84 * sizeof(uint64_t), ctx->stream));
  const uint32_t n_items = (uint32_t)ctx->n_items;
  if (n_items) {
    const uint32_t need = (n_items + 255) / 256;
    const uint32_t blocks = need < (uint32_t)ctx->num_cu * 4u ? need : (uint32_t)ctx->num_cu * 4u;
    hipLaunchKernelGGL(bg_count_kernel, dim3(blocks), dim3(256), 0, ctx->stream, (const uint32_t*)ctx->d_words,
                       ctx->d_items, n_items, ctx->W, raw);
    PENGK_HIP(hipGetLastError());
  }
  hipLaunchKernelGGL(bg_finish_kernel, dim3(1), dim3(64), 0, ctx->stream, raw, (unsigned long long*)d_bg);
  PENGK_HIP(hipGetLastError());
  return PENGK_OK;
}

int launch_bg_model(pengk_ctx* ctx, const uint64_t* d_bg, int K, const float* h_alpha, float* d_V) {
  hipLaunchKernelGGL(bg_model_kernel, dim3(1), dim3(128), 0, ctx->stream, (const unsigned long long*)d_bg, K, h_alpha[0],
                     h_alpha[1], h_alpha[2], d_V);
  PENGK_HIP(hipGetLastError());
  return PENGK_OK;
}

int launch_synth(pengk_ctx* ctx, uint64_t seed, uint64_t seq0, uint64_t n_seq, uint32_t L, int W, int item_windows,
                 uint64_t* d_words, uint64_t* d_items) {
  uint64_t nw = 0, ni = 0;
  int rc = pengk_synth_sizes(n_seq, L, W, item_windows, &nw, &ni);
  if (rc) return rc;
  hipLaunchKernelGGL(synth_words_kernel, dim3(4096), dim3(256), 0, ctx->stream, seed, seq0, n_seq, L, d_words, nw);
  PENGK_HIP(hipGetLastError());
  if (ni) {
    hipLaunchKernelGGL(synth_items_kernel, dim3(2048), dim3(256), 0, ctx->stream, n_seq, L, W, (uint32_t)item_windows, d_items);
    PENGK_HIP(hipGetLastError());
  }
  return PENGK_OK;
}

}
```

peng-motif_amd/csrc/em.hip:

```cpp
#include "em_serial.h"

namespace pengk {
namespace {
#ifdef PENGK_WG_TRACE
constexpr unsigned WG_TRACE_MAX = 1u << 20;
__device__ unsigned long long g_wg_trace[3 * WG_TRACE_MAX];
__device__ unsigned g_wg_trace_n;
struct WgTrace {
  unsigned long long t0;
  unsigned kernel;
  __device__ __forceinline__ WgTrace(unsigned k) : t0(__builtin_amdgcn_s_memrealtime()), kernel(k) {}
  __device__ __forceinline__ void end(unsigned kind, unsigned wg) const {
    if (threadIdx.x != 0) return;
    const unsigned long long t1 = __builtin_amdgcn_s_memrealtime();
    const unsigned xcc = __builtin_amdgcn_s_getreg((4 << 11) | (0 << 6) | 20) & 0xFu;
    const unsigned i = atomicAdd(&g_wg_trace_n, 1u);
    if (i < WG_TRACE_MAX) {
      g_wg_trace[3 * i] = ((unsigned long long)kernel << 56) | ((unsigned long long)kind << 48) | ((unsigned long long)xcc << 40) | wg;
      g_wg_trace[3 * i + 1] = t0;
      g_wg_trace[3 * i + 2] = t1;
    }
  }
};
#define PENGK_WG_TRACE_BEGIN(k) const WgTrace wg_trace(k)
// ... 87 lines not shown
  if constexpr (G::HI == 0) {
    leaf(xlow, pr, S);
  } else {
    static_assert(G::HI >= 2, "EM geometry");
    constexpr int OUT = G::HI - 2;
    double so[P][OUT > 0 ? OUT : 1];
#pragma unroll
    for (int q = 0; q < P; ++q)
#pragma unroll
      for (int jo = 0; jo < (OUT > 0 ? OUT : 1); ++jo) so[q][jo] = 0.0;
#pragma unroll 1
    for (int o = 0; o < (1 << (2 * OUT)); ++o) {
      float po[P];
      uint32_t xo = xlow;
#pragma unroll
      for (int q = 0; q < P; ++q) po[q] = pr[q];
#pragma unroll
      for (int jo = 0; jo < OUT; ++jo) {
        const int dj = (o >> (2 * jo)) & 3;
        xo |= (uint32_t)dj << (2 * (G::PB + jo));
#pragma unroll
        for (int q = 0; q < P; ++q) po[q] = po[q] * s_pwm[q][(G::PB + jo) * 4 + dj];
      }
      double s1[P];
#pragma unroll
      for (int q = 0; q < P; ++q) s1[q] = 0.0;
      if constexpr (FAST) {
        float wf[P][4][4];
#pragma unroll
        for (int d2 = 0; d2 < 4; ++d2) {
          float p2[P];
#pragma unroll
          for (int q = 0; q < P; ++q) p2[q] = po[q] * s_pwm[q][(G::PB + OUT) * 4 + d2];
#pragma unroll
          for (int d3 = 0; d3 < 4; ++d3) {
            const uint32_t off = (xo | ((uint32_t)d2 << (2 * (G::PB + OUT))) | ((uint32_t)d3 << (2 * (G::PB + OUT + 1)))) << 2;
            const float cs = *reinterpret_cast<const float*>(reinterpret_cast<const char*>(counts) + off);
            const float sb = *reinterpret_cast<const float*>(reinterpret_cast<const char*>(bg) + off);
#pragma unroll
            for (int q = 0; q < P; ++q) {
              const float p3 = p2[q] * s_pwm[q][(G::PB + OUT + 1) * 4 + d3];
              wf[q][d2][d3] = cs * p3 * __builtin_amdgcn_rcpf(sb + p3);
            }
          }
        }
#pragma unroll
        for (int q = 0; q < P; ++q) {
          float tot = 0.0f;
#pragma unroll
          for (int d = 0; d < 4; ++d) {
            const float row = (wf[q][d][0] + wf[q][d][1]) + (wf[q][d][2] + wf[q][d][3]);
            const float col = (wf[q][0][d] + wf[q][1][d]) + (wf[q][2][d] + wf[q][3][d]);
            acc[q][OUT][d] += (double)row;
            acc[q][OUT + 1][d] += (double)col;
            tot += row;
          }
          s1[q] = (double)tot;
        }
      } else
#pragma unroll
      for (int d2 = 0; d2 < 4; ++d2) {
        float p2[P];
        double s2[P];
#pragma unroll
        for (int q = 0; q < P; ++q) {
          p2[q] = po[q] * s_pwm[q][(G::PB + OUT) * 4 + d2];
          s2[q] = 0.0;
        }
#pragma unroll
        for (int d3 = 0; d3 < 4; ++d3) {
          float p3[P];
          double w[P];
#pragma unroll
          for (int q = 0; q < P; ++q) p3[q] = p2[q] * s_pwm[q][(G::PB + OUT + 1) * 4 + d3];
          const uint32_t x = xo | ((uint32_t)d2 << (2 * (G::PB + OUT))) | ((uint32_t)d3 << (2 * (G::PB + OUT + 1)));
          leaf(x, p3, w);
#pragma unroll
          for (int q = 0; q < P; ++q) {
            acc[q][OUT + 1][d3] += w[q];
            s2[q] += w[q];
          }
        }
#pragma unroll
        for (int q = 0; q < P; ++q) {
          acc[q][OUT][d2] += s2[q];
          s1[q] += s2[q];
        }
      }
#pragma unroll
      for (int q = 0; q < P; ++q) {
#pragma unroll
        for (int jo = 0; jo < OUT; ++jo) {
          so[q][jo] += s1[q];
          if ((o & ((1 << (2 * jo)) - 1)) == (1 << (2 * jo)) - 1) {
            const int dj = (o >> (2 * jo)) & 3;
#pragma unroll
            for (int a = 0; a < 4; ++a) acc[q][jo][a] += (a == dj) ? so[q][jo] : 0.0;
            so[q][jo] = 0.0;
          }
        }
        S[q] += s1[q];
      }
    }
  }

  const int wave = tid >> 6, lane = tid & 63;
#pragma unroll
  for (int q = 0; q < P; ++q) {
#pragma unroll
    for (int p = 0; p < 3; ++p) {
      double v = S[q];
#pragma unroll
      for (int b = 0; b < 6; ++b)
        if ((b >> 1) != p) v += __shfl_xor(v, 1 << b, 64);
      if ((lane & ~(3 << (2 * p))) == 0) s_cls[q][wave][p][(lane >> (2 * p)) & 3] = v;
      if (p == 0) {
        double t = v;
        t += __shfl_xor(t, 1, 64);
        t += __shfl_xor(t, 2, 64);
        if (lane == 0) s_T[q][wave] = t;
      }
    }
    if constexpr (G::HI > 0) {
#pragma unroll
      for (int h = 0; h < G::HI; ++h)
#pragma unroll
        for (int a = 0; a < 4; ++a) {
          const double v = wave_sum(acc[q][h][a]);
          if (lane == 0) s_red[q][wave][h * 4 + a] = v;
        }
    }
  }
  __syncthreads();
  if (tid < (uint32_t)G::CELLS) {
    const int p = tid >> 2, a = tid & 3;
#pragma unroll
    for (int q = 0; q < P; ++q) {
      if (!live[q]) continue;
      double v = 0.0;
      if (p < 3) {
        v = ((s_cls[q][0][p][a] + s_cls[q][1][p][a]) + s_cls[q][2][p][a]) + s_cls[q][3][p][a];
      } else if (p == 3) {
        v = s_T[q][a];
      } else if (p < G::PB) {
        if ((int)((mid >> (2 * (p - G::LO))) & 3u) == a) v = ((s_T[q][0] + s_T[q][1]) + s_T[q][2]) + s_T[q][3];
      } else {
        if constexpr (G::HI > 0) {
          const int h = p - G::PB;
          v = ((s_red[q][0][h * 4 + a] + s_red[q][1][h * 4 + a]) + s_red[q][2][h * 4 + a]) + s_red[q][3][h * 4 + a];
        }
      }
      partials[((size_t)(pw0 + q) * G::NB + blockIdx.x) * G::CELLS + tid] = v;
    }
  }
}

__global__ __launch_bounds__(1024) void em_bg_range_kernel(const float* __restrict__ bg, uint32_t np, uint32_t* __restrict__ range) {
  __shared__ uint32_t s_lo[16], s_hi[16];
  uint32_t lo = 0xFFFFFFFFu, hi = 0u;
  const uint4* v = reinterpret_cast<const uint4*>(bg);
  for (uint32_t i = blockIdx.x * 1024u + threadIdx.x; i < np / 4u; i += gridDim.x * 1024u) {
    const uint4 b = v[i];
    lo = min(min(lo, b.x), min(min(b.y, b.z), b.w));
    hi = max(max(hi, b.x), max(max(b.y, b.z), b.w));
  }
#pragma unroll
  for (int m = 1; m < 64; m <<= 1) {
    lo = min(lo, (uint32_t)__shfl_xor((int)lo, m, 64));
    hi = max(hi, (uint32_t)__shfl_xor((int)hi, m, 64));
  }
  if ((threadIdx.x & 63u) == 0u) {
    s_lo[threadIdx.x >> 6] = lo;
    s_hi[threadIdx.x >> 6] = hi;
  }
  __syncthreads();
  if (threadIdx.x == 0) {
    for (int w = 1; w < 16; ++w) {
      lo = min(lo, s_lo[w]);
      hi = max(hi, s_hi[w]);
    }
    atomicMin(range, lo);
    atomicMax(range + 1, hi);
  }
}

__global__ __launch_bounds__(256) void em_div_check_kernel(unsigned long long seed, uint32_t per_thread, unsigned long long* __restrict__ out) {
  unsigned long long st = seed + 0x9E3779B97F4A7C15ull * (blockIdx.x * 256ull + threadIdx.x + 1ull);
  auto next = [&]() {
    unsigned long long z = (st += 0x9E3779B97F4A7C15ull);
    z = (z ^ (z >> 30)) * 0xBF58476D1CE4E5B9ull;
    z = (z ^ (z >> 27)) * 0x94D049BB133111EBull;
    return z ^ (z >> 31);
  };
  unsigned long long checked = 0, bad = 0, zero = 0;
  for (uint32_t i = 0; i < per_thread; ++i) {
    const unsigned long long r = next(), q = next();
    uint32_t ma = (uint32_t)r & 0x7FFFFFu, mb = (uint32_t)(r >> 23) & 0x7FFFFFu;
    const uint32_t kind = (uint32_t)(q >> 60);
    if (kind == 0u) ma = 0u;
    else if (kind == 1u) mb = 0u;
    else if (kind == 2u) ma = 0x7FFFFFu;
    else if (kind == 3u) mb = 0x7FFFFFu;
    else if (kind == 4u) mb = 1u << ((q >> 40) % 23u);
    const uint32_t ea = 1u + (uint32_t)(q % 254ull), eb = 1u + (uint32_t)((q >> 8) % 254ull);
    float a = __uint_as_float((ea << 23) | ma);
    const float b = __uint_as_float((eb << 23) | mb);
    if (!lean_div_ok(a, a, b, b)) continue;
    if (((q >> 50) & 63ull) == 0ull) {
      a = 0.0f;
      ++zero;
    }
    const float lean = lean_div(a, b);
    float full;
    asm volatile("" : "+v"(a));
    full = a / b;
    ++checked;
    bad += __float_as_uint(lean) != __float_as_uint(full);
  }
  atomicAdd(out, checked);
  atomicAdd(out + 1, bad);
  atomicAdd(out + 2, zero);
}

template <int W>
__global__ __launch_bounds__(256) void em_weights_span_kernel(const uint32_t* __restrict__ counts, const float* __restrict__ bg,
                                                              float saturation, float* __restrict__ wbuf,
                                                              float* __restrict__ sums, const uint32_t* __restrict__ bg_range,
                                                              FusedState fs, uint32_t k, float threshold, int max_it) {
  using G = BlockGeo<W>;
  PENGK_WG_TRACE_BEGIN(1);
  const uint32_t pw = blockIdx.y, sp = blockIdx.x;
  __shared__ __attribute__((aligned(16))) float s_pwm[W * 4], s_old[W * 4];
  __shared__ float part[4][28];
  __shared__ uint32_t s_lean;
  const uint32_t t = threadIdx.x, lane = t & 63u, wave = t >> 6;
  const uint32_t bg_lo = bg_range[0], bg_hi = bg_range[1];
  if (!fused_head<W>(fs, pw, k, threshold, max_it, sp == 0u, s_pwm, s_old, t)) return;
  uint32_t* bad = fs.bad + (size_t)(k & 1u) * fs.bad_stride;
  if (t == 0) s_lean = lean_ranges_ok<W>(s_pwm, bg_lo, bg_hi, saturation) ? 1u : 0u;
  __syncthreads();
  const bool lean = s_lean != 0u;
  float* out = wbuf + (size_t)pw * G::NP + (size_t)sp * 16384u;
  const uint32_t* cnt = counts + (size_t)sp * 16384u;
  const float* bgs = bg + (size_t)sp * 16384u;
  float p3 = 1.0f;
#pragma unroll
  for (int p = 0; p < 4; ++p) p3 = p3 * s_pwm[p * 4 + ((t >> (2 * p)) & 3u)];
  float hi[W - 7];
#pragma unroll
  for (int p = 7; p < W; ++p) hi[p - 7] = s_pwm[p * 4 + ((sp >> (2 * (p - 7))) & 3u)];
  float f4_[4], f5_[4], f6_[4];
#pragma unroll
  for (int a = 0; a < 4; ++a) {
    f4_[a] = s_pwm[16 + a];
    f5_[a] = s_pwm[20 + a];
    f6_[a] = s_pwm[24 + a];
  }
  float c4[4] = {0, 0, 0, 0}, c5[4] = {0, 0, 0, 0}, c6[4] = {0, 0, 0, 0};
  bool flagged = false;
  auto body = [&](auto lean_tag) {
    constexpr bool LEAN = decltype(lean_tag)::value;
#pragma unroll 1
    for (uint32_t d6 = 0; d6 < 4u; ++d6) {
#pragma unroll
      for (uint32_t d5 = 0; d5 < 4u; ++d5) {
        float s5 = 0.0f;
#pragma unroll
        for (uint32_t d4 = 0; d4 < 4u; ++d4) {
          const uint32_t xl = t + 256u * (d4 + 4u * d5 + 16u * d6);
          float pr = ((p3 * f4_[d4]) * f5_[d5]) * f6_[d6];
#pragma unroll
          for (int p = 7; p < W; ++p) pr = pr * hi[p - 7];
          const float odds = em_div<LEAN>(pr, bgs[xl]);
          const float v = em_div<LEAN>((float)cnt[xl] * saturation, 1 + em_div<LEAN>(saturation, odds));
          out[xl] = v;
          flagged |= __float_as_uint(v) > 0x7F7FFFFFu;
          c4[d4] += v;
          s5 += v;
        }
        c5[d5] += s5;
        c6[d6] += s5;
      }
    }
  };
  if (lean) body(std::true_type{});
  else body(std::false_type{});
  if (flagged) bad[pw] = 1u;
  const float tot = (c6[0] + c6[1]) + (c6[2] + c6[3]);
  auto all = [](float v) {
#pragma unroll
    for (int m = 1; m < 64; m <<= 1) v += __shfl_xor(v, m, 64);
    return v;
  };
#pragma unroll
  for (int a = 0; a < 4; ++a) {
    const float s4 = all(c4[a]), s5 = all(c5[a]), s6 = all(c6[a]);
    if (lane == 0) {
      part[wave][12 + a] = s4;
      part[wave][16 + a] = s5;
      part[wave][20 + a] = s6;
    }
  }
#pragma unroll
  for (int d = 0; d < 3; ++d) {
    float v = tot;
#pragma unroll
    for (int m = 1; m < 64; m <<= 1)
      if (m != (1 << (2 * d)) && m != (2 << (2 * d))) v += __shfl_xor(v, m, 64);
    if ((lane & ~(3u << (2 * d))) == 0u) part[wave][4 * d + (lane >> (2 * d))] = v;
  }
  {
    const float v = all(tot);
    if (lane == 0) part[wave][24] = v;
  }
  __syncthreads();
  if (t < G::CELLS) {
    const uint32_t p = t >> 2, a = t & 3u;
    float* o = sums + (size_t)pw * G::CELLS * G::NBLK;
    if (p <= 6u) {
      float v;
      if (p == 3u) v = part[a][24];
      else {
        const uint32_t at = p <= 2u ? 4u * p + a : 4u * (p - 1u) + a;
        v = (part[0][at] + part[1][at]) + (part[2][at] + part[3][at]);
      }
      o[(size_t)t * G::NBLK + sp] = v;
    } else {
      const float v = (part[0][20 + a] + part[1][20 + a]) + (part[2][20 + a] + part[3][20 + a]);
      o[(size_t)(4u * p + G::high_digit(p, sp)) * G::NBLK + G::high_block(p, sp, a)] = v;
    }
  }
  PENGK_WG_TRACE_END(0, blockIdx.x + gridDim.x * blockIdx.y);
}

template <int W>
__global__ __launch_bounds__(64) void em_block_predict_kernel(const uint32_t* __restrict__ run_now, const uint32_t* __restrict__ bad,
                                                              const float* __restrict__ sums, seqsum::BlockRecord* __restrict__ rec,
                                                              uint32_t skew) {
  using G = BlockGeo<W>;
  const uint32_t pw = blockIdx.y, cell = blockIdx.x, lane = threadIdx.x;
  if (run_now[pw] == 0u || bad[pw]) return;
  constexpr uint32_t PER = G::NBLK / 64u;
  static_assert(G::NBLK % 64u == 0u, "whole lanes");
  const float* in = sums + ((size_t)pw * G::CELLS + cell) * G::NBLK + (size_t)lane * PER;
  seqsum::BlockRecord* out = rec + ((size_t)pw * G::CELLS + cell) * G::NBLK + (size_t)lane * PER;
  double mine = 0.0;
  for (uint32_t i = 0; i < PER; ++i) mine += (double)in[i];
  double before = mine;
#pragma unroll
  for (int d = 1; d < 64; d <<= 1) {
    const double o = __shfl_up(before, d, 64);
    if ((int)lane >= d) before += o;
  }
  before -= mine;
  for (uint32_t i = 0; i < PER; ++i) {
    const double after = before + (double)in[i];
    const uint32_t e = block_binade(before, after, skew, cell * G::NBLK + lane * PER + i);
    seqsum::BlockRecord r;
    r.e = e;
    r.d0 = 0.0f;
    r.d1 = 0.0f;
    r.pad = 0u;
    out[i] = r;
    before = after;
  }
}

constexpr uint32_t SPAN_EVAL_WAVES = 8;
template <int W>
__global__ __launch_bounds__(64 * SPAN_EVAL_WAVES) void em_span_eval_kernel(const uint32_t* __restrict__ run_now, const float* __restrict__ wbuf,
                                                                            seqsum::BlockRecord* __restrict__ rec,
                                                                            const uint32_t* __restrict__ bad, uint32_t n_pwm,
                                                                            const float* __restrict__ sums, uint32_t skew,
                                                                            uint32_t extra_wgs, uint32_t head_blocks) {
  using G = BlockGeo<W>;
  PENGK_WG_TRACE_BEGIN(2);
  const uint32_t lin = blockIdx.x + gridDim.x * blockIdx.y;
  __shared__ __attribute__((aligned(16))) float span[16384];
  const uint32_t t = threadIdx.x, lane = t & 63u;
  const uint32_t wave = (uint32_t)__builtin_amdgcn_readfirstlane((int)(t >> 6));
  if (lin < extra_wgs) {
    constexpr uint32_t XW = (G::CELLS + 3u) / 4u;
    uint32_t pw, xunit;
    if (!group_map(lin, n_pwm, XW, pw, xunit)) return;
    const uint32_t cell = 4u * xunit + wave;
    if (wave >= 4u || cell >= G::CELLS || run_now[pw] == 0u || bad[pw]) return;
    seqsum::lds_float* buf = (seqsum::lds_float*)span + wave * seqsum::BLOCK;
    const float* w = wbuf + (size_t)pw * G::NP;
    seqsum::Row mine;
// ... 51 lines not shown
  uint32_t binades = seqsum::NO_BINADE;
  if constexpr (G::PREDICT_IN_EVAL) {
    constexpr uint32_t LOADS = G::NBLK / 64u, GROUP = LOADS <= 4u ? TASKS : 2u;
#pragma unroll 1
    for (uint32_t i0 = 0; i0 < TASKS; i0 += GROUP) {
      float part[GROUP], own[GROUP];
#pragma unroll
      for (uint32_t g = 0; g < GROUP; ++g) {
        const uint32_t task = min(wave + SPAN_EVAL_WAVES * (i0 + g), G::CELLS - 1u);
        const uint32_t cell = cell_of(task), b = block_of(task);
        const float* cs = sums + ((size_t)pw * G::CELLS + cell) * G::NBLK;
        float acc = 0.0f;
#pragma unroll
        for (uint32_t c = 0; c < G::NBLK; c += 64u) {
          const float x = cs[c + lane];
          acc += c + lane < b ? x : 0.0f;
        }
        part[g] = acc;
        own[g] = cs[b];
      }
#pragma unroll
      for (uint32_t g = 0; g < GROUP; ++g) {
        const uint32_t i = i0 + g, task = wave + SPAN_EVAL_WAVES * i;
        float acc = part[g];
#pragma unroll
        for (int m = 1; m < 64; m <<= 1) acc += __shfl_xor(acc, m, 64);
        if (i < TASKS && task < G::CELLS) {
          const uint32_t e = block_binade((double)acc, (double)acc + (double)own[g], skew, cell_of(task) * G::NBLK + block_of(task));
          if (lane == i) binades = e;
        }
      }
    }
  } else {
#pragma unroll 1
    for (uint32_t i = 0; i < TASKS; ++i) {
      const uint32_t task = wave + SPAN_EVAL_WAVES * i;
      if (task < G::CELLS) {
        const uint32_t e = cells[(size_t)cell_of(task) * G::NBLK + block_of(task)].e;
        if (lane == i) binades = e;
      }
    }
  }
  if (running == 0 || flagged) return;
  {
    seqsum::f4* dst = reinterpret_cast<seqsum::f4*>(span);
#pragma unroll
    for (uint32_t k = 0; k < PER; ++k) {
      const uint32_t idx = t + T * k;
      dst[SpanLds::slot_of(idx >> 4, idx & 15u)] = v[k];
    }
  }
  __syncthreads();
  PENGK_WG_TRACE_END(2, lin);
#pragma unroll 1
  for (uint32_t task = wave, i = 0; task < G::CELLS; task += SPAN_EVAL_WAVES, ++i) {
    const uint32_t p = task >> 2, j = task & 3u;
    if (block_of(task) < head_blocks) continue;
    seqsum::BlockRecord* r = cells + (size_t)cell_of(task) * G::NBLK + block_of(task);
    const uint32_t e = (uint32_t)__builtin_amdgcn_readlane((int)binades, (int)i);
    if (e == seqsum::NO_BINADE) {
      if (G::PREDICT_IN_EVAL && lane == 0) r->e = seqsum::NO_BINADE;
      continue;
    }
    seqsum::Row mine;
    span_row<W>(span, p, j, lane, mine);
    float d0, d1;
    const bool ok = seqsum::block_increments(mine, lane, seqsum::bases_of_binade(e), d0, d1);
    if (lane == 0) {
      seqsum::BlockRecord out;
      out.e = ok ? e : seqsum::NO_BINADE;
      out.d0 = d0;
      out.d1 = d1;
      out.pad = 0u;
      *r = out;
    }
  }
  PENGK_WG_TRACE_END(0, lin);
}

template <int W>
__global__ __launch_bounds__(64) void em_chain_store_kernel(const uint32_t* __restrict__ run, const uint32_t* __restrict__ bad,
                                                            const float* __restrict__ wbuf, const seqsum::BlockRecord* __restrict__ rec,
                                                            float* __restrict__ cellsum, uint32_t n_pwm,
                                                            unsigned long long* __restrict__ counters) {
  using G = BlockGeo<W>;
  PENGK_WG_TRACE_BEGIN(3);
  const uint32_t lin = blockIdx.x + gridDim.x * blockIdx.y;
  uint32_t pw, cell;
  if (!group_map(lin, n_pwm, G::CELLS, pw, cell)) return;
  __shared__ __attribute__((aligned(16))) float lds[seqsum::WALK_LDS_FLOATS];
  seqsum::WalkCounts wc;
  const uint32_t lane = threadIdx.x;
  const seqsum::BlockRecord* r = rec + ((size_t)pw * G::CELLS + cell) * G::NBLK;
  uint32_t running = run[pw];
  uint32_t flagged = bad[pw];
  uint4 first = reinterpret_cast<const uint4*>(r)[lane];
  asm volatile("" : "+s"(running), "+s"(flagged), "+v"(first.x), "+v"(first.y), "+v"(first.z), "+v"(first.w));
  if (running == 0u) return;
  float s = 0.0f;
  const float* w = wbuf + (size_t)pw * G::NP;
  if (flagged) {
    const uint32_t p = cell >> 2, a = cell & 3u;
    for (uint32_t c = 0; c < (1u << (2 * W - 2)); ++c)
      s += w[((c >> (2u * p)) << (2u * p + 2u)) | (a << (2u * p)) | (c & ((1u << (2u * p)) - 1u))];
  } else if ((cell >> 2) == 0u) {
    EmTerms0<W> src0{w, cell & 3u};
    src0.bind_stage(lane);
    s = seqsum::walk_chain(src0, r, first, G::NBLK, (seqsum::lds_float*)lds, lane, wc);
  } else {
    EmTerms<W> src{w, cell >> 2, cell & 3u};
    src.bind_stage(lane);
    s = seqsum::walk_chain(src, r, first, G::NBLK, (seqsum::lds_float*)lds, lane, wc);
  }
  if (lane == 0) {
    cellsum[(size_t)pw * G::CELLS + cell] = s;
    if (wc.fetched) __hip_atomic_fetch_add(counters + 0, (unsigned long long)wc.fetched, __ATOMIC_RELAXED, __HIP_MEMORY_SCOPE_AGENT);
    if (wc.mispredicted) __hip_atomic_fetch_add(counters + 1, (unsigned long long)wc.mispredicted, __ATOMIC_RELAXED, __HIP_MEMORY_SCOPE_AGENT);
    if (wc.restaged) __hip_atomic_fetch_add(counters + 2, (unsigned long long)wc.restaged, __ATOMIC_RELAXED, __HIP_MEMORY_SCOPE_AGENT);
    if (wc.restaged_waits) __hip_atomic_fetch_add(counters + 3, (unsigned long long)wc.restaged_waits, __ATOMIC_RELAXED, __HIP_MEMORY_SCOPE_AGENT);
  }
  PENGK_WG_TRACE_END(wc.fetched > 255u ? 255u : wc.fetched, lin);
}

template <int W>
__global__ __launch_bounds__(64) void em_serial_finish_kernel(FusedState fs, uint32_t K, float threshold, int max_it) {
  constexpr uint32_t CELLS = 4u * W;
  const uint32_t pw = blockIdx.x, t = threadIdx.x;
  __shared__ __attribute__((aligned(16))) float s_pwm[CELLS], s_old[CELLS];
  const uint32_t running = fs.run[(size_t)((K - 1u) & 1u) * fs.run_stride + pw];
  if (running) {
    const float* prev = ((K - 1u) & 1u) ? fs.pwm1 : fs.pwm0;
    if (t < CELLS) {
      s_old[t] = prev[(size_t)pw * CELLS + t];
      s_pwm[t] = fs.cellsum[(size_t)pw * CELLS + t];
    }
    __syncthreads();
    const float change = finalize_rows<W>(s_pwm, s_old, t);
    if (t < CELLS) fs.pwm0[(size_t)pw * CELLS + t] = s_pwm[t];
    if (t == 0) {
      fs.state[2 * pw] = (int)K;
      fs.state[2 * pw + 1] = !(change <= threshold || (int)K >= max_it);
      fs.change[pw] = change;
    }
  } else {
    const int it = fs.state[2 * pw];
    if ((it & 1) && t < CELLS) fs.pwm0[(size_t)pw * CELLS + t] = fs.pwm1[(size_t)pw * CELLS + t];
  }
  if (t == 0) {
    fs.bad[pw] = 0u;
    fs.bad[(size_t)fs.bad_stride + pw] = 0u;
  }
}

__global__ __launch_bounds__(256) void em_serial_setup_kernel(uint32_t n, int W, float threshold, int max_it, int32_t* __restrict__ state,
                                                             float* __restrict__ change, uint32_t* __restrict__ run,
                                                             unsigned long long* __restrict__ counters, uint32_t* __restrict__ bg_range,
                                                             uint32_t lean, uint32_t* __restrict__ bad, uint32_t bad_words) {
  const uint32_t i = blockIdx.x * 256u + threadIdx.x;
  if (i < (uint32_t)EM_COUNTERS) counters[i] = 0ull;
  if (i == 0) {
    bg_range[0] = lean ? 0xFFFFFFFFu : 0u;
    bg_range[1] = lean ? 0u : 0xFFFFFFFFu;
  }
  for (uint32_t j = i; j < bad_words; j += gridDim.x * 256u) bad[j] = 0u;
  if (i >= n) return;
  const float c0 = (float)W;
  const uint32_t r = !(c0 <= threshold || 0 >= max_it);
  state[2 * i] = 0;
  state[2 * i + 1] = (int32_t)r;
  change[i] = c0;
  run[i] = r;
  run[n + i] = r;
}

template <int W, int HIMAX, bool FAST, int P>
int launch_geo(pengk_ctx* ctx, int64_t n_pwm, float* d_pwms, float saturation, float threshold, int max_it,
               const uint32_t* d_counts, const float* d_bg, int32_t* d_state, float* d_change) {
  using G = EmGeo<W, HIMAX>;
  hipLaunchKernelGGL(em_init_kernel, dim3((unsigned)((n_pwm + 255) / 256)), dim3(256), 0, ctx->stream, (int)n_pwm, W, threshold,
                     max_it, d_state, d_change);
  PENGK_HIP(hipGetLastError());
  const size_t per_pwm = (size_t)G::NB * G::CELLS * sizeof(double);
  const size_t budget = (size_t)256 << 20;
  int64_t batch = (int64_t)(budget / per_pwm);
  if (batch < 1) batch = 1;
  if (batch > n_pwm) batch = n_pwm;
  if (batch > 65535) batch = 65535;
  if (batch > P) batch -= batch % P;
  int rc = ensure_scratch(ctx, (void**)&ctx->d_em_partials, &ctx->em_partials_bytes, (size_t)batch * per_pwm);
  if (rc) return rc;
  if (FAST) {
    const uint32_t np = 1u << (2 * W);
    rc = ensure_scratch(ctx, (void**)&ctx->d_em_tables, &ctx->em_tables_bytes, (size_t)2 * np * sizeof(float));
    if (rc) return rc;
    float* cs = ctx->d_em_tables;
    float* sb = cs + np;
    const unsigned pb = (np + 255) / 256 < 4096u ? (np + 255) / 256 : 4096u;
    hipLaunchKernelGGL(em_prepare_kernel, dim3(pb), dim3(256), 0, ctx->stream, d_counts, d_bg, saturation, np, cs, sb);
    PENGK_HIP(hipGetLastError());
    d_counts = reinterpret_cast<const uint32_t*>(cs);
    d_bg = sb;
  }
  for (int64_t first = 0; first < n_pwm; first += batch) {
    const int64_t nb = n_pwm - first < batch ? n_pwm - first : batch;
    for (int it = 0; it < max_it; ++it) {
      hipLaunchKernelGGL((em_accumulate_kernel<W, HIMAX, FAST, P>), dim3(G::NB, (unsigned)((nb + P - 1) / P)), dim3(256), 0,
                         ctx->stream, d_pwms + (size_t)first * W * 4, d_state + 2 * first, d_counts, d_bg, saturation,
                         ctx->d_em_partials, (int)nb);
      hipLaunchKernelGGL((em_finalize_kernel<W, HIMAX>), dim3((unsigned)nb), dim3(64), 0, ctx->stream,
                         d_pwms + (size_t)first * W * 4, d_state + 2 * first, d_change + first, ctx->d_em_partials, threshold, max_it,
                         (uint32_t*)nullptr, (const float*)nullptr, 0u);
    }
    PENGK_HIP(hipGetLastError());
  }
  return PENGK_OK;
}

#ifdef PENGK_WG_TRACE
}
}
extern "C" __attribute__((visibility("default"))) long long pengk_debug_wg_trace(unsigned long long* out, unsigned max) {
  unsigned n = 0;
  if (hipDeviceSynchronize() != hipSuccess) return -1;
  if (hipMemcpyFromSymbol(&n, HIP_SYMBOL(pengk::g_wg_trace_n), sizeof n) != hipSuccess) return -1;
  const unsigned m = n < max ? n : max;
  if (m && hipMemcpyFromSymbol(out, HIP_SYMBOL(pengk::g_wg_trace), (size_t)m * 3 * sizeof(unsigned long long)) != hipSuccess) return -1;
  const unsigned zero = 0;
  if (hipMemcpyToSymbol(HIP_SYMBOL(pengk::g_wg_trace_n), &zero, sizeof zero) != hipSuccess) return -1;
  return (long long)n;
}
namespace pengk {
namespace {
#endif

#ifdef PENGK_SEQSUM_STATS
}
}
extern "C" __attribute__((visibility("default"))) int pengk_debug_seqsum_stats(unsigned long long* out, int reset) {
  if (hipMemcpyFromSymbol(out, HIP_SYMBOL(pengk::seqsum::g_stats), 12 * sizeof(unsigned long long)) != hipSuccess) return 1;
  if (reset) {
    unsigned long long z[12] = {0};
    if (hipMemcpyToSymbol(HIP_SYMBOL(pengk::seqsum::g_stats), z, sizeof z) != hipSuccess) return 1;
  }
  return 0;
}
namespace pengk {
namespace {
#endif

template <int W>
int launch_serial_ahead(pengk_ctx* ctx, int64_t n_pwm, float* d_pwms, float saturation, float threshold, int max_it,
                        const uint32_t* d_counts, const float* d_bg, int32_t* d_state, float* d_change, size_t budget, bool split) {
  using B = BlockGeo<W>;
  using LG = LookGeo<W>;
  const size_t np = (size_t)1 << (2 * W);
  int lanes = ctx->em_overlap < 1 ? 1 : ctx->em_overlap > MAX_EM_LANES ? MAX_EM_LANES : ctx->em_overlap;
  while (lanes > 1 && n_pwm < 8 * (int64_t)lanes) --lanes;
  const int64_t fit = std::max<int64_t>(1, (int64_t)(budget / lanes / (np * sizeof(float))));
  int64_t batch = fit;
  if (batch * lanes > n_pwm) {
    batch = lanes > 1 ? ((n_pwm + lanes - 1) / lanes + 7) / 8 * 8 : n_pwm;
    if (batch > fit) batch = fit >= 8 ? fit / 8 * 8 : fit;
  }
  if (batch > 16384) batch = 16384;
  const size_t tables_b = (size_t)batch * np * sizeof(float);
  const size_t sums_b = split ? ((size_t)batch * B::CELLS * B::NBLK * sizeof(float) + 255) / 256 * 256 : 0;
  const size_t rec_b = sums_b + ((size_t)batch * B::CELLS * B::NBLK * sizeof(seqsum::BlockRecord) + 255) / 256 * 256;
  const size_t look_b = split ? 0 : ((size_t)batch * LG::WORDS_PER_PWM * sizeof(unsigned long long) + 255) / 256 * 256;
  const size_t flags_at = ((size_t)batch * B::CELLS * sizeof(float) + 255) / 256 * 256;
  const size_t small_b = (flags_at + (size_t)2 * batch * sizeof(uint32_t) + 255) / 256 * 256;
  const size_t run_at = lanes * small_b;
  const size_t pwm1_at = (run_at + (size_t)2 * n_pwm * sizeof(uint32_t) + 255) / 256 * 256;
  int rc = ensure_scratch(ctx, (void**)&ctx->d_em_tables, &ctx->em_tables_bytes, lanes * tables_b);
  if (rc) return rc;
  rc = ensure_scratch(ctx, (void**)&ctx->d_em_partials, &ctx->em_partials_bytes, pwm1_at + (size_t)n_pwm * B::CELLS * sizeof(float));
  if (rc) return rc;
  rc = ensure_scratch(ctx, &ctx->d_em_blocks, &ctx->em_blocks_bytes, lanes * rec_b);
  if (rc) return rc;
  if (look_b) {
    const size_t had = ctx->em_look_bytes;
    rc = ensure_scratch(ctx, &ctx->d_em_look, &ctx->em_look_bytes, lanes * look_b);
    if (rc) return rc;
    if (ctx->em_look_bytes != had || ctx->em_epoch >= 0xFFFF0000u) {
      PENGK_HIP(hipStreamSynchronize(ctx->stream));
      for (int l = 0; l < MAX_EM_LANES - 1; ++l)
        if (ctx->em_streams[l]) PENGK_HIP(hipStreamSynchronize(ctx->em_streams[l]));
      PENGK_HIP(hipMemsetAsync(ctx->d_em_look, 0, ctx->em_look_bytes, ctx->stream));
      ctx->em_epoch = 0;
    }
  }
  if (!ctx->d_em_counters) PENGK_HIP(hipMalloc((void**)&ctx->d_em_counters, (EM_COUNTERS + 1) * sizeof(unsigned long long)));
  uint32_t* bg_range = reinterpret_cast<uint32_t*>(ctx->d_em_counters + EM_COUNTERS);
  char* small = reinterpret_cast<char*>(ctx->d_em_partials);
  uint32_t* run = reinterpret_cast<uint32_t*>(small + run_at);
  float* pwm1 = reinterpret_cast<float*>(small + pwm1_at);
  {
    const uint32_t words = (uint32_t)((run_at - flags_at) / sizeof(uint32_t));
    hipLaunchKernelGGL(em_serial_setup_kernel, dim3((unsigned)((std::max<int64_t>(n_pwm, 1024) + 255) / 256)), dim3(256), 0, ctx->stream,
                       (uint32_t)n_pwm, W, threshold, max_it, d_state, d_change, run, ctx->d_em_counters, bg_range,
                       ctx->em_lean_div ? 1u : 0u, reinterpret_cast<uint32_t*>(small + flags_at), words);
    if (ctx->em_lean_div)
      hipLaunchKernelGGL(em_bg_range_kernel, dim3(32), dim3(1024), 0, ctx->stream, d_bg, (uint32_t)np, bg_range);
    PENGK_HIP(hipGetLastError());
  }
  if (max_it <= 0) return PENGK_OK;
  hipStream_t streams[MAX_EM_LANES];
  streams[0] = ctx->stream;
  for (int l = 1; l < lanes; ++l) {
    if (!ctx->em_streams[l - 1]) PENGK_HIP(hipStreamCreateWithFlags(&ctx->em_streams[l - 1], hipStreamNonBlocking));
    if (!ctx->em_join[l - 1]) PENGK_HIP(hipEventCreateWithFlags(&ctx->em_join[l - 1], hipEventDisableTiming));
    streams[l] = ctx->em_streams[l - 1];
  }
  if (lanes > 1 && !ctx->em_fork) PENGK_HIP(hipEventCreateWithFlags(&ctx->em_fork, hipEventDisableTiming));
  if (lanes > 1) {
    PENGK_HIP(hipEventRecord(ctx->em_fork, ctx->stream));
    for (int l = 1; l < lanes; ++l) PENGK_HIP(hipStreamWaitEvent(streams[l], ctx->em_fork, 0));
  }
  const int rc_launch = [&]() -> int {
    for (int64_t round0 = 0; round0 < n_pwm; round0 += batch * lanes) {
      for (int it = 1; it <= max_it + 1; ++it) {
        for (int l = 0; l < lanes; ++l) {
          const int64_t first = round0 + (int64_t)l * batch;
          if (first >= n_pwm) break;
          const int64_t nb = n_pwm - first < batch ? n_pwm - first : batch;
          hipStream_t st = streams[l];
          float* tables = reinterpret_cast<float*>(reinterpret_cast<char*>(ctx->d_em_tables) + l * tables_b);
          float* sums = reinterpret_cast<float*>(reinterpret_cast<char*>(ctx->d_em_blocks) + l * rec_b);
          seqsum::BlockRecord* rec = reinterpret_cast<seqsum::BlockRecord*>(reinterpret_cast<char*>(ctx->d_em_blocks) + l * rec_b + sums_b);
          unsigned long long* look = reinterpret_cast<unsigned long long*>(reinterpret_cast<char*>(ctx->d_em_look) + l * look_b);
          float* cellsum = reinterpret_cast<float*>(small + l * small_b);
          uint32_t* bad = reinterpret_cast<uint32_t*>(small + l * small_b + flags_at);
          FusedState fs;
          fs.run = run + first;
          fs.pwm0 = d_pwms + (size_t)first * W * 4;
          fs.pwm1 = pwm1 + (size_t)first * W * 4;
          fs.bad = bad;
          fs.cellsum = cellsum;
          fs.state = d_state + 2 * first;
          fs.change = d_change + first;
          fs.n = (uint32_t)nb;
          fs.run_stride = (uint32_t)n_pwm;
          fs.bad_stride = (uint32_t)batch;
          if (it > max_it) {
            hipLaunchKernelGGL((em_serial_finish_kernel<W>), dim3((unsigned)nb), dim3(64), 0, st, fs, (uint32_t)max_it, threshold, max_it);
            continue;
          }
          const uint32_t k = (uint32_t)it;
          const unsigned groups = (unsigned)((nb + 7) / 8 * 8);
          const uint32_t* run_now = run + (size_t)((k - 1u) & 1u) * n_pwm + first;
          const uint32_t* bad_now = bad + (size_t)(k & 1u) * batch;
          if (split) {
            hipLaunchKernelGGL((em_weights_span_kernel<W>), dim3(B::SPANS, (unsigned)nb), dim3(256), 0, st, d_counts, d_bg, saturation, tables,
                               sums, (const uint32_t*)bg_range, fs, k, threshold, max_it);
            if (!B::PREDICT_IN_EVAL)
              hipLaunchKernelGGL((em_block_predict_kernel<W>), dim3(B::CELLS, (unsigned)nb), dim3(64), 0, st, run_now, bad_now,
                                 (const float*)sums, rec, (uint32_t)ctx->em_test_skew);
            const uint64_t xwgs = (uint64_t)nb * ((B::CELLS + 3) / 4), swgs = xwgs + (uint64_t)nb * B::SPANS;
            hipLaunchKernelGGL((em_span_eval_kernel<W>), dim3(1024u, (unsigned)((swgs + 1023u) / 1024u)), dim3(64 * SPAN_EVAL_WAVES), 0, st,
                               run_now, (const float*)tables, rec, bad_now, (uint32_t)nb, (const float*)sums,
                               (uint32_t)ctx->em_test_skew, (uint32_t)xwgs, (uint32_t)std::min<uint64_t>(ctx->em_head_blocks, B::NBLK));
            hipLaunchKernelGGL((em_chain_store_kernel<W>), dim3((unsigned)(4 * W), (unsigned)nb), dim3(64), 0, st, run_now, bad_now,
                               (const float*)tables, (const seqsum::BlockRecord*)rec, cellsum, (uint32_t)nb, ctx->d_em_counters);
            continue;
          }
          if constexpr (LG::SUPPORTED) {
            const uint64_t wgs = (uint64_t)groups * B::SPANS;
            const unsigned gx = 1024u;
            const uint32_t epoch = ++ctx->em_epoch;
            const int rc_fused = launch_span_fused(W, gx, (unsigned)((wgs + gx - 1) / gx), st, fs, k, threshold, max_it, d_counts, d_bg, saturation,
                                                   tables, rec, look, epoch, (const uint32_t*)bg_range, (uint32_t)ctx->em_test_skew,
                                                   (uint32_t)ctx->em_test_lookback);
            if (rc_fused) return rc_fused;
          }
          hipLaunchKernelGGL((em_chain_store_kernel<W>), dim3((unsigned)(4 * W), (unsigned)nb), dim3(64), 0, st, run_now, bad_now,
                             (const float*)tables, (const seqsum::BlockRecord*)rec, cellsum, (uint32_t)nb, ctx->d_em_counters);
        }
      }
      PENGK_HIP(hipGetLastError());
    }
    return PENGK_OK;
  }();
  int rc_join = PENGK_OK;
  for (int l = 1; l < lanes; ++l) {
    hipError_t e = hipEventRecord(ctx->em_join[l - 1], streams[l]);
    if (e == hipSuccess) e = hipStreamWaitEvent(ctx->stream, ctx->em_join[l - 1], 0);
    if (e != hipSuccess) {
      (void)hipStreamSynchronize(streams[l]);
      if (!rc_join) rc_join = hip_fail(e, "joining the EM's streams");
    }
  }
  return rc_launch ? rc_launch : rc_join;
}

#ifndef PENGK_EM_BUDGET_GIB
#define PENGK_EM_BUDGET_GIB 24
#endif
template <int W>
int launch_serial(pengk_ctx* ctx, int64_t n_pwm, float* d_pwms, float saturation, float threshold, int max_it,
                  const uint32_t* d_counts, const float* d_bg, int32_t* d_state, float* d_change) {
  const size_t np = (size_t)1 << (2 * W);
  size_t budget = (size_t)ctx->em_table_budget_mb << 20;
  if (budget == 0) {
    if (2 * np * sizeof(float) <= ((size_t)16 << 20)) {
      budget = (size_t)192 << 20;
    } else {
      size_t free_b = 0, total_b = 0;
      budget = (size_t)1 << 30;
      if (hipMemGetInfo(&free_b, &total_b) == hipSuccess)
        budget = std::min(std::max(budget, (free_b + ctx->em_tables_bytes) / 4), (size_t)PENGK_EM_BUDGET_GIB << 30);
    }
  }
  if constexpr (W >= 10) {
    if (ctx->em_serial_scan >= 2)
      return launch_serial_ahead<W>(ctx, n_pwm, d_pwms, saturation, threshold, max_it, d_counts, d_bg, d_state, d_change, budget,
                                    ctx->em_serial_scan != 3 || !LookGeo<W>::SUPPORTED);
  }
  return launch_em_serial_legacy(ctx, W, ctx->em_serial_scan != 0 ? 1 : 0, n_pwm, d_pwms, saturation, threshold, max_it, d_counts, d_bg,
                                 d_state, d_change, budget);
}

__global__ __launch_bounds__(64) void em_w2_kernel(float* __restrict__ pwms, int32_t* __restrict__ state, float* __restrict__ change_out,
                                                   const uint32_t* __restrict__ counts, const float* __restrict__ bg, float saturation,
                                                   float threshold, int max_it, int mode) {
  const int pw = blockIdx.x, lane = threadIdx.x;
  __shared__ float s_pwm[8], s_w[16];
  __shared__ int s_active;
  float* old = pwms + (size_t)pw * 8;
  if (lane < 8) s_pwm[lane] = old[lane];
  if (lane == 0) s_active = state[2 * pw + 1];
  __syncthreads();
  const float cs = lane < 16 ? (float)counts[lane] * saturation : 0.0f;
  const float b = lane < 16 ? bg[lane] : 1.0f;
  while (s_active) {
    if (lane < 16) {
      const float pr = (1.0f * s_pwm[lane & 3]) * s_pwm[4 + (lane >> 2)];
      float w;
      if (mode == 1) {
        w = cs * pr * __builtin_amdgcn_rcpf(saturation * b + pr);
      } else {
        const float odds = pr / b;
        w = cs / (1 + saturation / odds);
      }
      s_w[lane] = w;
    }
    __syncthreads();
    if (lane == 0) {
      float nw[8];
      for (int c = 0; c < 8; ++c) {
        const int p = c >> 2, a = c & 3;
        if (mode == 2) {
          float acc = 0.0f;
          for (int x = 0; x < 16; ++x)
            if (((x >> (2 * p)) & 3) == a) acc += s_w[x];
          nw[c] = acc;
        } else {
          double acc = 0.0;
          for (int x = 0; x < 16; ++x)
            if (((x >> (2 * p)) & 3) == a) acc += (double)s_w[x];
          nw[c] = (float)acc;
        }
      }
      float change = 0.0f;
      for (int p = 0; p < 2; ++p) {
        float sum = 0.0f;
        for (int a = 0; a < 4; ++a) sum += nw[p * 4 + a];
        for (int a = 0; a < 4; ++a) nw[p * 4 + a] /= sum;
      }
      for (int c = 0; c < 8; ++c) {
        change += fabsf(nw[c] - s_pwm[c]);
        s_pwm[c] = nw[c];
      }
      const int it = state[2 * pw] + 1;
      state[2 * pw] = it;
      s_active = !(change <= threshold || it >= max_it);
      state[2 * pw + 1] = s_active;
      change_out[pw] = change;
    }
    __syncthreads();
  }
  if (lane < 8) old[lane] = s_pwm[lane];
}

template <int W>
int launch_w(pengk_ctx* ctx, int64_t n_pwm, float* d_pwms, float saturation, float threshold, int max_it,
             const uint32_t* d_counts, const float* d_bg, int32_t* d_state, float* d_change) {
#define PENGK_EM_GEO(H, F, PP) launch_geo<W, H, F, PP>(ctx, n_pwm, d_pwms, saturation, threshold, max_it, d_counts, d_bg, d_state, d_change)
  if (ctx->em_fast == 2) return launch_serial<W>(ctx, n_pwm, d_pwms, saturation, threshold, max_it, d_counts, d_bg, d_state, d_change);
  const bool fast = ctx->em_fast != 0;
  if constexpr (W >= 8) {
    const int64_t wg4 = n_pwm * EmGeo<W, 4>::NB;
    if (wg4 * 4 < (int64_t)ctx->num_cu * 4) return fast ? PENGK_EM_GEO(2, true, 1) : PENGK_EM_GEO(2, false, 1);
    if (wg4 < (int64_t)ctx->num_cu * 8) return fast ? PENGK_EM_GEO(3, true, 1) : PENGK_EM_GEO(3, false, 1);
  }
  return fast ? PENGK_EM_GEO(4, true, 1) : PENGK_EM_GEO(4, false, 1);
#undef PENGK_EM_GEO
}

}

int launch_em(pengk_ctx* ctx, int W, int64_t n_pwm, float* d_pwms, float saturation, float threshold, int max_it,
              const uint32_t* d_counts, const float* d_bg, int32_t* d_state, float* d_change) {
  if (ctx->d_em_counters) PENGK_HIP(hipMemsetAsync(ctx->d_em_counters, 0, EM_COUNTERS * sizeof(unsigned long long), ctx->stream));
  switch (W) {
    case 2:
      hipLaunchKernelGGL(em_init_kernel, dim3((unsigned)((n_pwm + 255) / 256)), dim3(256), 0, ctx->stream, (int)n_pwm, W, threshold, max_it,
                         d_state, d_change);
      hipLaunchKernelGGL(em_w2_kernel, dim3((unsigned)n_pwm), dim3(64), 0, ctx->stream, d_pwms, d_state, d_change, d_counts, d_bg,
                         saturation, threshold, max_it, ctx->em_fast);
      PENGK_HIP(hipGetLastError());
      return PENGK_OK;
    case 4: return launch_w<4>(ctx, n_pwm, d_pwms, saturation, threshold, max_it, d_counts, d_bg, d_state, d_change);
    case 6: return launch_w<6>(ctx, n_pwm, d_pwms, saturation, threshold, max_it, d_counts, d_bg, d_state, d_change);
    case 8: return launch_w<8>(ctx, n_pwm, d_pwms, saturation, threshold, max_it, d_counts, d_bg, d_state, d_change);
    case 10: return launch_w<10>(ctx, n_pwm, d_pwms, saturation, threshold, max_it, d_counts, d_bg, d_state, d_change);
    case 12: return launch_w<12>(ctx, n_pwm, d_pwms, saturation, threshold, max_it, d_counts, d_bg, d_state, d_change);
    case 14: return launch_w<14>(ctx, n_pwm, d_pwms, saturation, threshold, max_it, d_counts, d_bg, d_state, d_change);
    default: return fail(PENGK_ERR_ARG, "pattern length %d unsupported", W);
  }
}

int warm_em() {
  hipFuncAttributes a;
  PENGK_HIP(hipFuncGetAttributes(&a, (const void*)em_init_kernel));
  return PENGK_OK;
}

}

extern "C" int pengk_selftest_division(pengk_ctx* ctx, uint64_t seed, uint32_t pairs_per_thread, uint64_t* h_out) {
  using namespace pengk;
  if (!ctx || !h_out) return fail(PENGK_ERR_ARG, "pengk_selftest_division: NULL argument");
  int rc = enter(ctx);
  if (rc) return rc;
  rc = ensure_scratch(ctx, &ctx->d_misc, &ctx->misc_bytes, 3 * sizeof(unsigned long long));
  if (rc) return rc;
  PENGK_HIP(hipMemsetAsync(ctx->d_misc, 0, 3 * sizeof(unsigned long long), ctx->stream));
  hipLaunchKernelGGL(em_div_check_kernel, dim3(4096), dim3(256), 0, ctx->stream, (unsigned long long)seed, pairs_per_thread,
                     (unsigned long long*)ctx->d_misc);
  PENGK_HIP(hipGetLastError());
  PENGK_HIP(hipMemcpyAsync(h_out, ctx->d_misc, 3 * sizeof(unsigned long long), hipMemcpyDeviceToHost, ctx->stream));
  PENGK_HIP(hipStreamSynchronize(ctx->stream));
  return PENGK_OK;
}
```

peng-motif_amd/csrc/em_fused.hip:

```cpp
#include "em_serial.h"

#define PENGK_WG_TRACE_BEGIN(k)
#define PENGK_WG_TRACE_END(kind, wg)

namespace pengk {
namespace {
__device__ __forceinline__ unsigned long long look_word(uint32_t epoch, float v) {
  uint32_t b = __float_as_uint(v);
  if (b > 0x7F800000u) b = 0x7F800000u;
  return ((unsigned long long)epoch << 32) | b;
}
__device__ __forceinline__ unsigned long long look_load(const unsigned long long* p) {
  return __hip_atomic_load(p, __ATOMIC_RELAXED, __HIP_MEMORY_SCOPE_AGENT);
}

template <int W>
__global__ __launch_bounds__(FusedGeo::THREADS) __attribute__((amdgpu_waves_per_eu(4, 4))) void em_span_fused_kernel(FusedState fs, uint32_t k, float threshold, int max_it,
                                                                          const uint32_t* __restrict__ counts,
                                                                          const float* __restrict__ bg, float saturation,
                                                                          float* __restrict__ wbuf, seqsum::BlockRecord* __restrict__ rec,
                                                                          unsigned long long* __restrict__ look, uint32_t epoch,
                                                                          const uint32_t* __restrict__ bg_range, uint32_t skew,
                                                                          uint32_t test_lookback) {
  using G = BlockGeo<W>;
  using LG = LookGeo<W>;
  constexpr uint32_t CELLS = G::CELLS, WAVES = FusedGeo::WAVES;
  PENGK_WG_TRACE_BEGIN(2);
  const uint32_t lin = blockIdx.x + gridDim.x * blockIdx.y;
  __shared__ __attribute__((aligned(16))) float span[16384];
  __shared__ __attribute__((aligned(16))) float s_pwm[CELLS], s_old[CELLS];
  __shared__ float s_part[WAVES][28];
  __shared__ float s_cell[CELLS];
  __shared__ float s_look[2][WAVES][CELLS];
  __shared__ uint32_t s_ok[WAVES];
  __shared__ uint32_t s_lean;
  const uint32_t t = threadIdx.x, lane = t & 63u;
  const uint32_t wave = (uint32_t)__builtin_amdgcn_readfirstlane((int)(t >> 6));
  uint32_t* bad_now = fs.bad + (size_t)(k & 1u) * fs.bad_stride;
  const uint32_t bg_lo = bg_range[0], bg_hi = bg_range[1];

  const uint32_t sl = lin, slot = sl >> 3;
  const uint32_t pw = (sl & 7u) + 8u * (slot / G::SPANS), sp = slot % G::SPANS;
  if (pw >= fs.n) return;
  const uint32_t* cnt = counts + (size_t)sp * 16384u;
  const float* bgs = bg + (size_t)sp * 16384u;
  if (!fused_head<W>(fs, pw, k, threshold, max_it, sp == 0u, s_pwm, s_old, t)) return;
  if (t == 0) s_lean = lean_ranges_ok<W>(s_pwm, bg_lo, bg_hi, saturation) ? 1u : 0u;
  __syncthreads();
  const bool lean = s_lean != 0u;
  PENGK_WG_TRACE_END(4, lin);

  unsigned long long* my_look = look + (size_t)pw * LG::WORDS_PER_PWM;
  const uint32_t chunk = sp / FusedGeo::CHUNK, c0 = chunk * FusedGeo::CHUNK, n0 = sp - c0;
  constexpr uint32_t PER = FusedGeo::CHUNK / WAVES;
  constexpr uint32_t PERC = (LG::CHUNKS + WAVES - 1u) / WAVES;
  const unsigned long long* src[PER + PERC];
  unsigned long long v[PER + PERC];
  bool need[PER + PERC];
  {
    float* out_t = wbuf + (size_t)pw * G::NP + (size_t)sp * 16384u + (t & 255u);
    const uint32_t* cnt_t = cnt + (t & 255u);
    const float* bg_t = bgs + (t & 255u);
    const uint32_t tl = t & 255u, h = t >> 8, w3 = (t >> 6) & 3u;
    float p3 = 1.0f;
#pragma unroll
    for (int p = 0; p < 4; ++p) p3 = p3 * s_pwm[p * 4 + ((tl >> (2 * p)) & 3u)];
    float hi[W - 7];
#pragma unroll
    for (int p = 7; p < W; ++p) hi[p - 7] = s_pwm[p * 4 + ((sp >> (2 * (p - 7))) & 3u)];
    float f4_[4], f5_[4];
#pragma unroll
    for (int a = 0; a < 4; ++a) {
      f4_[a] = s_pwm[16 + a];
      f5_[a] = s_pwm[20 + a];
    }
    float c4[4] = {0, 0, 0, 0}, c5[4] = {0, 0, 0, 0}, c6[2] = {0, 0};
    uint32_t worst = 0u;
    const uint32_t kslot = (tl >> 2) & 15u, comp = tl & 3u;
    char* span_b = reinterpret_cast<char*>(span);
    auto body = [&](auto lean_tag) {
      constexpr bool LEAN = decltype(lean_tag)::value;
#pragma unroll 1
      for (uint32_t i6 = 0; i6 < 2u; ++i6) {
        const uint32_t d6 = 2u * h + i6;
        const float f6 = s_pwm[24 + d6];
        const uint32_t g6 = (((d6 & 1u) << 3) ^ ((d6 & 3u) << 2)) & 15u;
        const uint32_t a6 = 256u * (w3 + 64u * d6) + 4u * comp + 16u * ((kslot ^ w3 ^ g6) & 15u);
        float* out6 = out_t + 4096u * d6;
        const uint32_t* cnt6 = cnt_t + 4096u * d6;
        const float* bg6 = bg_t + 4096u * d6;
        float s6 = 0.0f;
#pragma unroll
        for (uint32_t d5 = 0; d5 < 4u; ++d5) {
          float s5 = 0.0f;
#pragma unroll
          for (uint32_t d4 = 0; d4 < 4u; ++d4) {
            constexpr uint32_t dummy = 0u;
            (void)dummy;
            const uint32_t m2 = d4 + 4u * d5;
            const uint32_t cc = ((d4 << 2) ^ (d4 >> 1) ^ (d5 << 1) ^ d5) & 15u;
            float pr = ((p3 * f4_[d4]) * f5_[d5]) * f6;
#pragma unroll
            for (int p = 7; p < W; ++p) pr = pr * hi[p - 7];
            const float odds = em_div<LEAN>(pr, bg6[256u * m2]);
            const float v = em_div<LEAN>((float)cnt6[256u * m2] * saturation, 1 + em_div<LEAN>(saturation, odds));
            out6[256u * m2] = v;
            *reinterpret_cast<float*>(span_b + ((a6 ^ (16u * cc)) + 256u * (4u * d4 + 16u * d5))) = v;
            worst = max(worst, __float_as_uint(v));
            c4[d4] += v;
            s5 += v;
          }
          c5[d5] += s5;
          s6 += s5;
        }
        c6[0] += i6 ? 0.0f : s6;
        c6[1] += i6 ? s6 : 0.0f;
      }
    };
    if (lean) body(std::true_type{});
    else body(std::false_type{});
    if (worst > 0x7F7FFFFFu) bad_now[pw] = 1u;
#pragma unroll
    for (uint32_t i = 0; i < PER; ++i) {
      const uint32_t j = wave + WAVES * i;
      need[i] = j < n0 && lane < CELLS;
      src[i] = my_look + (size_t)(c0 + (j < n0 ? j : 0u)) * CELLS + (lane < CELLS ? lane : 0u);
    }
#pragma unroll
    for (uint32_t i = 0; i < PERC; ++i) {
      const uint32_t c = wave + WAVES * i;
      need[PER + i] = c < chunk && lane < CELLS;
      src[PER + i] = my_look + (size_t)(G::SPANS + (c < chunk ? c : 0u)) * CELLS + (lane < CELLS ? lane : 0u);
    }
#pragma unroll
    for (uint32_t i = 0; i < PER + PERC; ++i) v[i] = need[i] ? look_load(src[i]) : 0ull;
    const float tot = c6[0] + c6[1];
    auto all = [](float v) {
#pragma unroll
      for (int m = 1; m < 64; m <<= 1) v += __shfl_xor(v, m, 64);
      return v;
    };
#pragma unroll
    for (int a = 0; a < 4; ++a) {
      const float s4 = all(c4[a]), s5 = all(c5[a]);
      if (lane == 0) {
        s_part[wave][12 + a] = s4;
        s_part[wave][16 + a] = s5;
      }
    }
#pragma unroll
    for (int i = 0; i < 2; ++i) {
      const float s6 = all(c6[i]);
      if (lane == 0) s_part[wave][20 + i] = s6;
    }
#pragma unroll
    for (int d = 0; d < 3; ++d) {
      float v = tot;
#pragma unroll
      for (int m = 1; m < 64; m <<= 1)
        if (m != (1 << (2 * d)) && m != (2 << (2 * d))) v += __shfl_xor(v, m, 64);
      if ((lane & ~(3u << (2 * d))) == 0u) s_part[wave][4 * d + (lane >> (2 * d))] = v;
    }
    {
      const float v = all(tot);
      if (lane == 0) s_part[wave][24] = v;
    }
  }
  PENGK_WG_TRACE_END(3, lin);
  __syncthreads();

  if (t < CELLS) {
    const uint32_t p = t >> 2, a = t & 3u;
    auto over_waves = [&](uint32_t at) {
      float v = 0.0f;
#pragma unroll
      for (uint32_t w = 0; w < WAVES; ++w) v += s_part[w][at];
      return v;
    };
    float v;
    if (p <= 2u) v = over_waves(4u * p + a);
    else if (p == 3u) v = s_part[a][24] + s_part[a + 4u][24];
    else if (p <= 5u) v = over_waves(4u * (p - 1u) + a);
    else {
      const uint32_t w0 = 4u * (a >> 1), at = 20u + (a & 1u);
      const float q = (s_part[w0][at] + s_part[w0 + 1u][at]) + (s_part[w0 + 2u][at] + s_part[w0 + 3u][at]);
      if (p == 6u) v = q;
      else v = a == G::high_digit(p, sp) ? over_waves(24u) : 0.0f;
    }
    s_cell[t] = v;
    __hip_atomic_store(my_look + (size_t)sp * CELLS + t, look_word(epoch, v), __ATOMIC_RELAXED, __HIP_MEMORY_SCOPE_AGENT);
  }

// ... 102 lines not shown
```

peng-motif_amd/csrc/em_serial.h:

```cpp
#pragma once
#include "em_common.h"

namespace pengk {
struct FusedState {
  uint32_t* run;
  float* pwm0;
  float* pwm1;
  uint32_t* bad;
  const float* cellsum;
  int32_t* state;
  float* change;
  uint32_t n;
  uint32_t run_stride, bad_stride;
};

int launch_span_fused(int W, unsigned grid_x, unsigned grid_y, hipStream_t st, const FusedState& fs, uint32_t k, float threshold, int max_it,
                      const uint32_t* d_counts, const float* d_bg, float saturation, float* tables, seqsum::BlockRecord* rec,
                      unsigned long long* look, uint32_t epoch, const uint32_t* bg_range, uint32_t skew, uint32_t lookback);

namespace {
template <int W>
struct BlockGeo {
  static_assert(W >= 8, "a span is 4^7 x");
  static constexpr uint32_t NP = 1u << (2 * W);
// ... 52 lines not shown
  auto fin = [](float x) { return __float_as_uint(x) - 0x00800000u < 0x7F000000u; };
  if (!(fin(a_lo) && fin(a_hi) && fin(b_lo) && fin(b_hi)) || a_lo > a_hi || b_lo > b_hi) return false;
  const int ea_lo = (int)(__float_as_uint(a_lo) >> 23), ea_hi = (int)(__float_as_uint(a_hi) >> 23);
  const int eb_lo = (int)(__float_as_uint(b_lo) >> 23), eb_hi = (int)(__float_as_uint(b_hi) >> 23);
  return eb_hi <= 251 && ea_lo >= 25 && ea_hi - eb_lo <= 94 && ea_lo - eb_hi >= -123;
}
template <int W>
__device__ __forceinline__ bool lean_ranges_ok(const float* s_pwm, uint32_t bg_lo_bits, uint32_t bg_hi_bits, float saturation) {
  float p_lo = 1.0f, p_hi = 1.0f;
  for (int p = 0; p < W; ++p) {
    const float a = s_pwm[p * 4], b = s_pwm[p * 4 + 1], c = s_pwm[p * 4 + 2], d = s_pwm[p * 4 + 3];
    if (!(a > 0.0f && b > 0.0f && c > 0.0f && d > 0.0f)) return false;
    p_lo *= fminf(fminf(a, b), fminf(c, d));
    p_hi *= fmaxf(fmaxf(a, b), fmaxf(c, d));
  }
  p_lo *= 0.5f;
  p_hi *= 2.0f;
  const float b_lo = __uint_as_float(bg_lo_bits), b_hi = __uint_as_float(bg_hi_bits);
  if (bg_hi_bits > 0x7F7FFFFFu || !(saturation > 0.0f)) return false;
  if (!lean_div_ok(p_lo, p_hi, b_lo, b_hi)) return false;
  const float o_lo = p_lo / b_hi * 0.5f, o_hi = p_hi / b_lo * 2.0f;
  if (!lean_div_ok(saturation, saturation, o_lo, o_hi)) return false;
  const float t_hi = saturation / o_lo * 2.0f;
  const float n_lo = saturation * 0.5f, n_hi = saturation * 8589934592.0f;
  return lean_div_ok(n_lo, n_hi, 1.0f, (1.0f + t_hi) * 2.0f);
}

template <int W>
__device__ __forceinline__ float finalize_rows(float* s_new, float* s_old, uint32_t t) {
  typedef seqsum::f4 f4;
  float mine = 0.0f, diff = 0.0f;
  if (t < 4u * W) {
    const f4 row = reinterpret_cast<const f4*>(s_new)[t >> 2];
    float sum = 0.0f;
    sum += row.x;
    sum += row.y;
    sum += row.z;
    sum += row.w;
    mine = s_new[t] / sum;
    diff = fabsf(mine - s_old[t]);
  }
  __syncthreads();
  if (t < 4u * W) {
    s_new[t] = mine;
    s_old[t] = diff;
  }
  __syncthreads();
  float change = 0.0f;
  f4 d[W];
#pragma unroll
  for (int p = 0; p < W; ++p) d[p] = reinterpret_cast<const f4*>(s_old)[p];
#pragma unroll
  for (int p = 0; p < W; ++p) {
    change += d[p].x;
    change += d[p].y;
    change += d[p].z;
    change += d[p].w;
  }
  return change;
}

template <int W>
__device__ __forceinline__ bool fused_head(const FusedState& fs, uint32_t pw, uint32_t k, float threshold, int max_it, bool writer,
                                           float* s_pwm, float* s_old, uint32_t t) {
  constexpr uint32_t CELLS = 4u * W;
  const uint32_t was_running = fs.run[(size_t)(k & 1u) * fs.run_stride + pw];
  const float* prev = (k >= 2u && (k & 1u)) ? fs.pwm1 : fs.pwm0;
  float old = 0.0f, sum = 0.0f;
  if (t < CELLS) {
    old = prev[(size_t)pw * CELLS + t];
    if (k >= 2u) sum = fs.cellsum[(size_t)pw * CELLS + t];
  }
  if (!was_running) {
    if (writer && t == 0) {
      fs.run[(size_t)((k - 1u) & 1u) * fs.run_stride + pw] = 0u;
      fs.bad[(size_t)((k + 1u) & 1u) * fs.bad_stride + pw] = 0u;
    }
    return false;
  }
  if (k < 2u) {
    if (t < CELLS) s_pwm[t] = old;
    if (writer && t == 0) fs.bad[(size_t)((k + 1u) & 1u) * fs.bad_stride + pw] = 0u;
    __syncthreads();
    return true;
  }
  if (t < CELLS) {
    s_pwm[t] = sum;
    s_old[t] = old;
  }
  __syncthreads();
  const float change = finalize_rows<W>(s_pwm, s_old, t);
  const int it = (int)k - 1;
  const bool running = !(change <= threshold || it >= max_it);
  if (writer) {
    float* next = (k & 1u) ? fs.pwm0 : fs.pwm1;
    if (t < CELLS) next[(size_t)pw * CELLS + t] = s_pwm[t];
    if (t == 0) {
      fs.state[2 * pw] = it;
      fs.state[2 * pw + 1] = running ? 1 : 0;
      fs.change[pw] = change;
      fs.run[(size_t)((k - 1u) & 1u) * fs.run_stride + pw] = running ? 1u : 0u;
      fs.bad[(size_t)((k + 1u) & 1u) * fs.bad_stride + pw] = 0u;
    }
  }
  return running;
}

struct SpanLds {
  static __device__ __forceinline__ uint32_t g(uint32_t R) { return (R ^ (R >> 3) ^ (R >> 4)) & 15u; }
  static __device__ __forceinline__ uint32_t slot_of(uint32_t R, uint32_t k) { return R * 16u + (k ^ g(R)); }
};

template <int W>
__device__ __forceinline__ void span_row(const float* span, uint32_t p, uint32_t j, uint32_t l, seqsum::Row& row) {
  typedef seqsum::f4 f4;
  const f4* s4 = reinterpret_cast<const f4*>(span);
  if (p >= 3u) {
    uint32_t R;
    if (p >= 6u) {
      R = 64u * j + l;
    } else {
      const uint32_t sh = 2u * p - 6u;
      R = ((l >> sh) << (sh + 2u)) | (j << sh) | (l & ((1u << sh) - 1u));
    }
    const uint32_t base = R * 16u + SpanLds::g(R);
#pragma unroll
    for (uint32_t k = 0; k < 16u; ++k) row.q[k] = s4[base ^ k];
  } else if (p != 0u) {
    const uint32_t base = 64u * l + SpanLds::g(4u * l);
    if (p == 2u) {
#pragma unroll
      for (uint32_t k = 0; k < 16u; ++k) row.q[k] = s4[base ^ (16u * (k >> 2) + (((k & 3u) + 4u * j) ^ (k >> 2)))];
    } else {
#pragma unroll
      for (uint32_t k = 0; k < 16u; ++k) row.q[k] = s4[base ^ (16u * (k >> 2) + ((4u * (k & 3u) + j) ^ (k >> 2)))];
    }
  } else {
    const uint32_t base = 4u * (64u * l + SpanLds::g(4u * l)) + j;
#pragma unroll
    for (uint32_t k = 0; k < 16u; ++k) {
      const uint32_t c = k >> 2;
      row.q[k].x = span[base ^ (4u * (16u * c + ((4u * (k & 3u) + 0u) ^ c)))];
      row.q[k].y = span[base ^ (4u * (16u * c + ((4u * (k & 3u) + 1u) ^ c)))];
      row.q[k].z = span[base ^ (4u * (16u * c + ((4u * (k & 3u) + 2u) ^ c)))];
      row.q[k].w = span[base ^ (4u * (16u * c + ((4u * (k & 3u) + 3u) ^ c)))];
    }
  }
  asm volatile("" : "+v"(row.q[0]), "+v"(row.q[1]), "+v"(row.q[2]), "+v"(row.q[3]), "+v"(row.q[4]), "+v"(row.q[5]), "+v"(row.q[6]),
               "+v"(row.q[7]), "+v"(row.q[8]), "+v"(row.q[9]), "+v"(row.q[10]), "+v"(row.q[11]), "+v"(row.q[12]), "+v"(row.q[13]),
               "+v"(row.q[14]), "+v"(row.q[15]));
}

constexpr int EM_COUNTERS = 4;
struct FusedGeo {
  static constexpr uint32_t THREADS = 512, WAVES = 8, CHUNK = 64;
  static constexpr unsigned long long LOOKBACK_TICKS = 50000ull;
};
template <int W>
struct LookGeo {
  using G = BlockGeo<W>;
  static constexpr uint32_t CHUNKS = (G::SPANS + FusedGeo::CHUNK - 1u) / FusedGeo::CHUNK;
  static constexpr bool SUPPORTED = CHUNKS <= 64u;
  static constexpr size_t WORDS_PER_PWM = (size_t)(G::SPANS + CHUNKS) * G::CELLS;
};
}
}
```

peng-motif_amd/csrc/pengk_internal.h:

```cpp
#pragma once
#include <hip/hip_runtime.h>
#include <stdint.h>

#include "pengk.h"

struct pengk_ctx {
  int device = 0;
  hipStream_t stream = nullptr;
  bool own_stream = false;
  int num_cu = 256;
  const uint64_t* d_words = nullptr;
  uint64_t n_words = 0;
  const uint64_t* d_items = nullptr;
  uint64_t n_items = 0;
  int W = 0;
  int item_windows = 0;
  uint64_t max_bin_bound = 0;
  int all_whole = 0;
  uint32_t* d_defer = nullptr;
  uint64_t defer_cap = 0;
  double* d_em_partials = nullptr;
  size_t em_partials_bytes = 0;
  float* d_em_tables = nullptr;
  size_t em_tables_bytes = 0;
  void* d_em_blocks = nullptr;
  size_t em_blocks_bytes = 0;
  void* d_pair_mids = nullptr;
  size_t pair_mids_bytes = 0;
  int pair_mids_W = 0;
  void* d_em_look = nullptr;
  size_t em_look_bytes = 0;
  uint32_t em_epoch = 0;
  int em_test_lookback = 0;
  unsigned long long* d_em_counters = nullptr;
  hipStream_t em_streams[3] = {nullptr, nullptr, nullptr};
  hipEvent_t em_fork = nullptr, em_join[3] = {nullptr, nullptr, nullptr};
  void* d_misc = nullptr;
  size_t misc_bytes = 0;
  void* d_bg_partials = nullptr;
  size_t bg_partials_bytes = 0;
  void* d_iupac_big = nullptr;
  size_t iupac_big_bytes = 0;
  void* d_keys = nullptr;
  size_t keys_bytes = 0;
  void* d_count_aux = nullptr;
  size_t count_aux_bytes = 0;
  uint64_t n_windows_hint = 0;
  uint64_t key_cap_override = 0;
  uint64_t iupac_group_bytes = 0;
  uint64_t em_table_budget_mb = 0;
  int em_test_skew = 0;
  int em_overlap = 2;
  int em_serial_scan = 2;
  int em_head_blocks = 1;
  int sweep_pairs = 1;
  int em_lean_div = 1;
  int em_fast = 2;
  int count_impl = 0;
  int scatter_blocks_per_cu = 0;
  void* d_sim = nullptr;
  size_t sim_bytes = 0;
  void* d_score = nullptr;
  size_t score_bytes = 0;
  void* d_sites = nullptr;
  size_t sites_bytes = 0;
  uint64_t sites_record_budget = 1ull << 24;
  void* comm = nullptr;
  int comm_transport = 0;
  int comm_rank = 0, comm_world = 1;
};

enum { PENGK_TRANSPORT_NONE = 0, PENGK_TRANSPORT_RCCL = 1, PENGK_TRANSPORT_TCP = 2 };

namespace pengk {

int fail(int code, const char* fmt, ...);
int hip_fail(hipError_t e, const char* what);
int ensure_scratch(pengk_ctx* ctx, void** slot, size_t* have, size_t need);
int enter(pengk_ctx* ctx);
int count_init_device();
int warm_stats();
int warm_iupac();
int warm_similarity();
int warm_em();
void comm_release(pengk_ctx* ctx);

#define PENGK_HIP(call)                                   \
  do {                                                    \
    hipError_t e_ = (call);                               \
    if (e_ != hipSuccess) return ::pengk::hip_fail(e_, #call); \
  } while (0)

inline bool valid_w(int W) { return W >= PENGK_MIN_W && W <= PENGK_MAX_W && (W % 2) == 0; }

constexpr int MAX_EM_LANES = 4;

constexpr uint64_t ITEM_WS_MASK = (1ull << 40) - 1;
constexpr int ITEM_NW_SHIFT = 40;
constexpr uint64_t ITEM_NW_MASK = 0xFFFF;
constexpr int ITEM_CONT_SHIFT = 56;

__host__ __device__ inline uint32_t revcomp32(uint32_t id, int W) {
  uint32_t v = ~id;
#if defined(__HIP_DEVICE_COMPILE__)
  v = __brev(v);
#else
  v = ((v >> 1) & 0x55555555u) | ((v & 0x55555555u) << 1);
  v = ((v >> 2) & 0x33333333u) | ((v & 0x33333333u) << 2);
  v = ((v >> 4) & 0x0F0F0F0Fu) | ((v & 0x0F0F0F0Fu) << 4);
  v = ((v >> 8) & 0x00FF00FFu) | ((v & 0x00FF00FFu) << 8);
  v = (v >> 16) | (v << 16);
#endif
  v = ((v & 0xAAAAAAAAu) >> 1) | ((v & 0x55555555u) << 1);
  return v >> (32 - 2 * W);
}

int launch_count(pengk_ctx* ctx, int both, uint32_t* d_counts, uint64_t* d_ltot, uint64_t* d_bg );
int launch_mirror(pengk_ctx* ctx, int W, uint32_t* d_counts);
int launch_bg_count(pengk_ctx* ctx, uint64_t* d_bg);
int launch_bg_model(pengk_ctx* ctx, const uint64_t* d_bg, int K, const float* h_alpha, float* d_V);
int launch_synth(pengk_ctx* ctx, uint64_t seed, uint64_t seq0, uint64_t n_seq, uint32_t L, int W, int item_windows,
                 uint64_t* d_words, uint64_t* d_items);
int launch_stats(pengk_ctx* ctx, int W, int both, int k, int max_k, const float* d_V, const uint64_t* d_ltot,
                 const uint32_t* d_counts, float* d_bgprob, float* d_expected, float* d_logp, float* d_z);
int launch_seed_candidates(pengk_ctx* ctx, int W, const float* d_z, const uint32_t* d_counts, float z_threshold,
                           uint64_t count_threshold, uint32_t cap, uint32_t* d_n, uint32_t* d_ids, float* d_zs);
int launch_sequential_sum(pengk_ctx* ctx, const float* d_terms, uint64_t n_chains, uint64_t chain_len, float* d_out);
int launch_similarity(pengk_ctx* ctx, int n, const float* d_pwm, const float* d_comp, const int32_t* d_len,
                      const uint64_t* d_sites, int both, const float* h_bg, int first_new, float* d_out);
int launch_iupac(pengk_ctx* ctx, int W, int both, const uint64_t* h_ids, int64_t n, const uint32_t* d_counts,
                 const float* d_bgp, const float* d_expected, pengk_iupac_stats* h_out);
int launch_em(pengk_ctx* ctx, int W, int64_t n_pwm, float* d_pwms, float saturation, float threshold, int max_it,
              const uint32_t* d_counts, const float* d_bg, int32_t* d_state, float* d_change);

}
```

Baseline: 531.7.

## Fold count finishing and EM prologue work into fewer launches and memsets

The k-mer count path now writes its scatter histogram straight into a slot-permuted temp table. A single gather kernel copies it into the final counts and also finishes the ltot and background-model reduction, so the per-width gather kernels and the separate bg_finish launch go away. Deferred fixup items now add into the permuted table layout, and the background partial sums are reduced inside extra blocks of the fixup launch. On the EM side, the setup kernel and the bg-range min/max kernel are merged into one prologue that writes per-block partial ranges, which consumers now reduce on load. The counter memset is also skipped in the fast serial mode. The aim is fewer kernel launches and memsets and less sequential hist read-modify-write, in exchange for more complex indexing and a 32-entry range reduction done by every consumer thread.

```diff
diff --git a/peng-motif_amd/csrc/api.hip b/peng-motif_amd/csrc/api.hip
--- a/peng-motif_amd/csrc/api.hip
+++ b/peng-motif_amd/csrc/api.hip
@@ -240,8 +240,8 @@
   PENGK_ENTER(ctx);
   if (strcmp(name, "deferred_items") == 0) {
     uint32_t n = 0;
-    if (ctx->d_defer) {
-      PENGK_HIP(hipMemcpyAsync(&n, ctx->d_defer, sizeof n, hipMemcpyDeviceToHost, ctx->stream));
+    if (ctx->d_defer_count) {
+      PENGK_HIP(hipMemcpyAsync(&n, ctx->d_defer_count, sizeof n, hipMemcpyDeviceToHost, ctx->stream));
       PENGK_HIP(hipStreamSynchronize(ctx->stream));
     }
     *value = n;
diff --git a/peng-motif_amd/csrc/count.hip b/peng-motif_amd/csrc/count.hip
--- a/peng-motif_amd/csrc/count.hip
+++ b/peng-motif_amd/csrc/count.hip
@@ -314,6 +314,7 @@
   __host__ __device__ static inline uint32_t join(uint32_t b, uint32_t p, uint32_t  = 0) {
     return (p & LOW) | (b << S) | ((p >> S) << (S + NBITS));
   }
+  __host__ __device__ static inline uint32_t slot(uint32_t b, uint32_t p, uint32_t  = 0) { return (b << PAYLOAD_BITS) | p; }
   __host__ __device__ static inline bool valid(uint32_t p) { return p != KEY_INVALID; }
 };
 
@@ -328,6 +329,7 @@
   __host__ __device__ static inline uint32_t payload(uint32_t id) { return (id & 0xFFu) | ((id >> (8 + NBITS)) << 8); }
   __host__ __device__ static inline uint32_t join(uint32_t b1, uint32_t p1, uint32_t  = 0) { return (p1 & 0xFFu) | (b1 << 8) | ((p1 >> 8) << (8 + NBITS)); }
   __host__ __device__ static inline bool valid(uint32_t p1) { return p1 < (1u << PBITS); }
+  __host__ __device__ static inline uint32_t slot(uint32_t b1, uint32_t p1, uint32_t  = 0);
 };
 struct Split12L2 {
   static constexpr int NBITS = 9 - Split12L1::NBITS;
@@ -339,7 +341,11 @@
     return Split12L1::join(outer, p1);
   }
   __host__ __device__ static inline bool valid(uint32_t p2) { return p2 != KEY_INVALID; }
+  __host__ __device__ static inline uint32_t slot(uint32_t b2, uint32_t p2, uint32_t outer) { return ((outer * NB + b2) << PAYLOAD_BITS) | p2; }
 };
+__host__ __device__ inline uint32_t Split12L1::slot(uint32_t b1, uint32_t p1, uint32_t) {
+  return Split12L2::slot(Split12L2::bucket(p1), Split12L2::payload(p1), b1);
+}
 
 struct Split14L1 {
   static constexpr int NBITS = 4;
@@ -348,6 +354,7 @@
   __host__ __device__ static inline uint32_t payload(uint32_t id) { return (id & 0x3FFu) | ((id >> 14) << 10); }
   __host__ __device__ static inline uint32_t join(uint32_t b1, uint32_t p1, uint32_t  = 0) { return (p1 & 0x3FFu) | (b1 << 10) | ((p1 >> 10) << 14); }
   __host__ __device__ static inline bool valid(uint32_t p1) { return p1 < (1u << 24); }
+  __host__ __device__ static inline uint32_t slot(uint32_t b1, uint32_t p1, uint32_t  = 0);
 };
 struct Split14L2 {
   static constexpr int NBITS = 4;
@@ -358,6 +365,7 @@
     return Split14L1::join(outer, (p2 & 0x1FFu) | (b2 << 9) | ((p2 >> 9) << 13));
   }
   __host__ __device__ static inline bool valid(uint32_t p2) { return p2 < (1u << 20); }
+  __host__ __device__ static inline uint32_t slot(uint32_t b2, uint32_t p2, uint32_t outer);
 };
 struct Split14L3 {
   static constexpr int NBITS = 5;
@@ -368,7 +376,24 @@
     return Split14L2::join(outer & 15u, (p3 & 0xFFu) | (b3 << 8) | ((p3 >> 8) << 13), outer >> 4);
   }
   __host__ __device__ static inline bool valid(uint32_t p3) { return p3 != KEY_INVALID; }
+  __host__ __device__ static inline uint32_t slot(uint32_t b3, uint32_t p3, uint32_t outer) { return ((outer * NB + b3) << PAYLOAD_BITS) | p3; }
 };
+__host__ __device__ inline uint32_t Split14L2::slot(uint32_t b2, uint32_t p2, uint32_t outer) {
+  return Split14L3::slot(Split14L3::bucket(p2), Split14L3::payload(p2), outer * NB + b2);
+}
+__host__ __device__ inline uint32_t Split14L1::slot(uint32_t b1, uint32_t p1, uint32_t) {
+  return Split14L2::slot(Split14L2::bucket(p1), Split14L2::payload(p1), b1);
+}
+
+template <int W>
+__host__ __device__ inline uint32_t table_slot(uint32_t x) {
+  if constexpr (W == 14) return Split14L1::slot(Split14L1::bucket(x), Split14L1::payload(x));
+  else if constexpr (W == 12) return Split12L1::slot(Split12L1::bucket(x), Split12L1::payload(x));
+  else {
+    using KS = KeySplit<W, 2 * W - PAYLOAD_BITS>;
+    return KS::slot(KS::bucket(x), KS::payload(x));
+  }
+}
 
 template <class E>
 struct ScatterRowT {
@@ -440,7 +465,7 @@
       const uint32_t s_src = (uint32_t)__builtin_amdgcn_readlane((int)src, p);
       const uint32_t fb = (uint32_t)__builtin_amdgcn_readlane((int)b, p);
       const uint32_t v = *(lds_e_t*)(uintptr_t)(s_src + ES * lane);
-      if (KS::valid(v)) __hip_atomic_fetch_add(&hist[KS::join(fb, v, outer)], 1u, __ATOMIC_RELAXED, __HIP_MEMORY_SCOPE_AGENT);
+      if (KS::valid(v)) __hip_atomic_fetch_add(&hist[KS::slot(fb, v, outer)], 1u, __ATOMIC_RELAXED, __HIP_MEMORY_SCOPE_AGENT);
     }
   }
 
@@ -641,16 +666,6 @@
   e.drain();
 }
 
-__global__ __launch_bounds__(256) void count_gather14_kernel(const uint32_t* __restrict__ temp, uint32_t* __restrict__ hist) {
-  const uint32_t np = 1u << 28;
-  for (uint32_t x = blockIdx.x * blockDim.x + threadIdx.x; x < np; x += gridDim.x * blockDim.x) {
-    const uint32_t p1 = Split14L1::payload(x), p2 = Split14L2::payload(p1);
-    const uint32_t fb = (Split14L1::bucket(x) * Split14L2::NB + Split14L2::bucket(p1)) * Split14L3::NB + Split14L3::bucket(p2);
-    const uint32_t v = temp[((size_t)fb << PAYLOAD_BITS) | Split14L3::payload(p2)];
-    if (v) hist[x] += v;
-  }
-}
-
 __global__ __launch_bounds__(1024) void count_hist_kernel(const uint16_t* __restrict__ keys, uint32_t slice_cap,
                                                           uint32_t n_slices, uint32_t nb,
                                                           const uint32_t* __restrict__ slice_fill, uint32_t bpb,
@@ -709,23 +724,42 @@
   }
 }
 
-__global__ __launch_bounds__(256) void count_gather12_kernel(const uint32_t* __restrict__ temp, uint32_t* __restrict__ hist) {
-  const uint32_t np = 1u << 24;
-  for (uint32_t x = blockIdx.x * blockDim.x + threadIdx.x; x < np; x += gridDim.x * blockDim.x) {
-    const uint32_t p1 = Split12L1::payload(x);
-    const uint32_t fb = Split12L1::bucket(x) * Split12L2::NB + Split12L2::bucket(p1);
-    const uint32_t v = temp[((size_t)fb << PAYLOAD_BITS) | Split12L2::payload(p1)];
-    if (v) hist[x] += v;
-  }
-}
-
-template <int W, int NBITS>
-__global__ __launch_bounds__(256) void count_gather_kernel(const uint32_t* __restrict__ temp, uint32_t np,
-                                                           uint32_t* __restrict__ hist) {
-  using KS = KeySplit<W, NBITS>;
-  for (uint32_t x = blockIdx.x * blockDim.x + threadIdx.x; x < np; x += gridDim.x * blockDim.x) {
-    const uint32_t v = temp[((size_t)KS::bucket(x) << PAYLOAD_BITS) | KS::payload(x)];
-    if (v) hist[x] += v;
+__device__ __forceinline__ void bg_finish_block(const unsigned long long* raw, unsigned long long* __restrict__ out) {
+  __shared__ unsigned long long n3[64];
+  __shared__ unsigned long long n2[16];
+  const int t = threadIdx.x;
+  if (t < 64) {
+    const int d0 = t >> 4, d1 = (t >> 2) & 3, d2 = t & 3;
+    n3[t] = raw[d0 | (d1 << 2) | (d2 << 4)];
+    out[20 + t] = n3[t];
+  }
+  __syncthreads();
+  if (t < 16) {
+    const int a = t >> 2, b = t & 3;
+    unsigned long long s = raw[68 + (a | (b << 2))];
+    for (int c = 0; c < 4; ++c) s += n3[c * 16 + t];
+    n2[t] = s;
+    out[4 + t] = s;
+  }
+  __syncthreads();
+  if (t < 4) {
+    unsigned long long s = raw[64 + t];
+    for (int b = 0; b < 4; ++b) s += n2[b * 4 + t];
+    out[t] = s;
+  }
+}
+
+template <int W>
+__global__ __launch_bounds__(256) void count_gather_kernel(const uint32_t* __restrict__ temp, uint32_t* __restrict__ hist,
+                                                           const unsigned long long* __restrict__ ltot_sum,
+                                                           unsigned long long* __restrict__ ltot,
+                                                           const unsigned long long* __restrict__ bg_raw,
+                                                           unsigned long long* __restrict__ bg_out) {
+  constexpr uint32_t np = 1u << (2 * W);
+  for (uint32_t x = blockIdx.x * blockDim.x + threadIdx.x; x < np; x += gridDim.x * blockDim.x) hist[x] = temp[table_slot<W>(x)];
+  if (blockIdx.x == 0) {
+    if (threadIdx.x == 0) *ltot = *ltot_sum;
+    if (bg_out) bg_finish_block(bg_raw, bg_out);
   }
 }
 
@@ -733,14 +767,45 @@
   return (words32[g >> 4] >> (2u * (uint32_t)(g & 15u))) & 3u;
 }
 
+__device__ __forceinline__ uint32_t table_slot_of(int layout, uint32_t x) {
+  switch (layout) {
+    case 8: return table_slot<8>(x);
+    case 10: return table_slot<10>(x);
+    case 12: return table_slot<12>(x);
+    case 14: return table_slot<14>(x);
+    default: return x;
+  }
+}
+
+constexpr uint32_t FIXUP_BLOCKS = 64;
 __global__ __launch_bounds__(64) void count_fixup_kernel(const uint32_t* __restrict__ words32,
                                                          const uint64_t* __restrict__ items, int W, int both,
-                                                         uint32_t* __restrict__ hist,
-                                                         const uint32_t* __restrict__ defer) {
+                                                         uint32_t* __restrict__ hist, int layout,
+                                                         const uint32_t* __restrict__ defer,
+                                                         const uint32_t* __restrict__ bg_partials, uint32_t n_bg_blocks,
+                                                         unsigned long long* __restrict__ bg_raw) {
+  if (blockIdx.x >= FIXUP_BLOCKS) {
+    const uint32_t bin = blockIdx.x - FIXUP_BLOCKS;
+    unsigned long long s = 0;
+    for (uint32_t b0 = 0; b0 < n_bg_blocks; b0 += 64u * 16u) {
+      uint32_t v[16];
+#pragma unroll
+      for (uint32_t j = 0; j < 16u; ++j) {
+        const uint32_t b = b0 + 64u * j + threadIdx.x;
+        v[j] = b < n_bg_blocks ? bg_partials[(size_t)b * 84 + bin] : 0u;
+      }
+#pragma unroll
+      for (uint32_t j = 0; j < 16u; ++j) s += v[j];
+    }
+#pragma unroll
+    for (int m = 1; m < 64; m <<= 1) s += __shfl_xor(s, m, 64);
+    if (threadIdx.x == 0) bg_raw[bin] = s;
+    return;
+  }
   const uint32_t n = defer[0];
   const uint32_t mask = (1u << (2 * W)) - 1u;
   const int top = 2 * (W - 1);
-  for (uint32_t q = blockIdx.x * blockDim.x + threadIdx.x; q < n; q += gridDim.x * blockDim.x) {
+  for (uint32_t q = blockIdx.x * blockDim.x + threadIdx.x; q < n; q += FIXUP_BLOCKS * blockDim.x) {
     const uint32_t it = defer[1 + q];
     const uint64_t rec = items[it];
     const uint32_t nw = (uint32_t)((rec >> ITEM_NW_SHIFT) & ITEM_NW_MASK);
@@ -777,7 +842,7 @@
             ok = false;
             break;
           }
-          if (!match) __hip_atomic_fetch_add(&hist[can], 1u, __ATOMIC_RELAXED, __HIP_MEMORY_SCOPE_AGENT);
+          if (!match) __hip_atomic_fetch_add(&hist[table_slot_of(layout, can)], 1u, __ATOMIC_RELAXED, __HIP_MEMORY_SCOPE_AGENT);
         }
         ring[(uint32_t)t & 15u] = match ? INVALID_ID : can;
       }
@@ -863,8 +928,6 @@
 __global__ void bg_finish_fused_kernel(const uint32_t* __restrict__ partials, uint32_t n_blocks,
                                        unsigned long long* __restrict__ out) {
   __shared__ unsigned long long raw[84];
-  __shared__ unsigned long long n3[64];
-  __shared__ unsigned long long n2[16];
   __shared__ unsigned long long part[12][84];
   const int t = threadIdx.x;
   {
@@ -890,25 +953,7 @@
     raw[t] = s;
   }
   __syncthreads();
-  if (t < 64) {
-    const int d0 = t >> 4, d1 = (t >> 2) & 3, d2 = t & 3;
-    n3[t] = raw[d0 | (d1 << 2) | (d2 << 4)];
-    out[20 + t] = n3[t];
-  }
-  __syncthreads();
-  if (t < 16) {
-    const int a = t >> 2, b = t & 3;
-    unsigned long long s = raw[68 + (a | (b << 2))];
-    for (int c = 0; c < 4; ++c) s += n3[c * 16 + t];
-    n2[t] = s;
-    out[4 + t] = s;
-  }
-  __syncthreads();
-  if (t < 4) {
-    unsigned long long s = raw[64 + t];
-    for (int b = 0; b < 4; ++b) s += n2[b * 4 + t];
-    out[t] = s;
-  }
+  bg_finish_block(raw, out);
 }
 
 __global__ __launch_bounds__(128) void bg_model_kernel(const unsigned long long* __restrict__ n, int K, float a0, float a1, float a2,
@@ -992,6 +1037,11 @@
   }
 }
 
+inline uint64_t slice_cap_of(const pengk_ctx* ctx, uint64_t sized) {
+  if (ctx->key_cap_override) return ctx->key_cap_override < 64 ? 0 : (ctx->key_cap_override + 63) / 64 * 64;
+  return (sized + 63) / 64 * 64;
+}
+
 #define PENGK_LAUNCH_BB(KERNEL, TARGS, both, bg, grid, block, ...)                                              \
   do {                                                                                                         \
     if (both) {                                                                                                \
@@ -1016,8 +1066,49 @@
   return PENGK_OK;
 }
 
+int launch_fixup(pengk_ctx* ctx, int both, uint32_t* table, int layout, const uint32_t* defer, uint32_t bg_blocks,
+                 unsigned long long* bg_raw) {
+  hipLaunchKernelGGL(count_fixup_kernel, dim3(FIXUP_BLOCKS + (bg_raw ? 84u : 0u)), dim3(64), 0, ctx->stream,
+                     (const uint32_t*)ctx->d_words, ctx->d_items, ctx->W, both, table, layout, defer,
+                     (const uint32_t*)ctx->d_bg_partials, bg_blocks, bg_raw);
+  PENGK_HIP(hipGetLastError());
+  return PENGK_OK;
+}
+
+struct CountAux {
+  unsigned long long* ltot_sum;
+  unsigned long long* bg_raw;
+  uint32_t* defer;
+};
+int count_aux_block(pengk_ctx* ctx, size_t front_bytes, CountAux* a) {
+  const size_t tail = (1 + 84 + 1) * sizeof(unsigned long long);
+  const size_t clear = front_bytes + tail;
+  int rc = ensure_scratch(ctx, &ctx->d_count_aux, &ctx->count_aux_bytes, clear + (size_t)(ctx->n_items + 1) * sizeof(uint32_t));
+  if (rc) return rc;
+  char* p = (char*)ctx->d_count_aux + front_bytes;
+  a->ltot_sum = (unsigned long long*)p;
+  a->bg_raw = a->ltot_sum + 1;
+  a->defer = (uint32_t*)(p + tail) - 1;
+  ctx->d_defer_count = a->defer;
+  PENGK_HIP(hipMemsetAsync(ctx->d_count_aux, 0, clear, ctx->stream));
+  return PENGK_OK;
+}
+
 template <int W>
 int launch_direct_w(pengk_ctx* ctx, int both, uint32_t* d_counts, uint64_t* d_ltot, uint32_t n_items, uint64_t* d_bg) {
+  {
+    const size_t need = (ctx->n_items + 2) * sizeof(uint32_t);
+    size_t have = ctx->defer_cap * sizeof(uint32_t);
+    if (have < need) {
+      int rc = ensure_scratch(ctx, (void**)&ctx->d_defer, &have, need);
+      if (rc) return rc;
+      ctx->defer_cap = have / sizeof(uint32_t);
+    }
+  }
+  ctx->d_defer_count = ctx->d_defer;
+  PENGK_HIP(hipMemsetAsync(ctx->d_defer, 0, sizeof(uint32_t), ctx->stream));
+  PENGK_HIP(hipMemsetAsync(d_counts, 0, ((size_t)1 << (2 * W)) * sizeof(uint32_t), ctx->stream));
+  PENGK_HIP(hipMemsetAsync(d_ltot, 0, sizeof(uint64_t), ctx->stream));
   const uint32_t* w32 = (const uint32_t*)ctx->d_words;
   const uint32_t blocks_needed = (n_items + 255) / 256;
   const uint32_t max_blocks = (uint32_t)ctx->num_cu * 8u;
@@ -1033,7 +1124,11 @@
                   lt, ctx->d_defer, bgp);
 #undef TA_DIRECT
   PENGK_HIP(hipGetLastError());
-  return d_bg ? bg_finish_fused(ctx, blocks, d_bg) : PENGK_OK;
+  if (d_bg) {
+    int rc = bg_finish_fused(ctx, blocks, d_bg);
+    if (rc) return rc;
+  }
+  return launch_fixup(ctx, both, d_counts, 0, ctx->d_defer, 0u, nullptr);
 }
 
 template <int W>
@@ -1052,21 +1147,18 @@
   uint64_t windows = ctx->n_windows_hint ? ctx->n_windows_hint : ctx->n_items * (uint64_t)ctx->item_windows;
   const uint64_t share = windows / ((uint64_t)NB * n_waves);
   uint64_t cap64 = share + share / 2 + 512;
-  if (ctx->key_cap_override) cap64 = ctx->key_cap_override;
-  cap64 = (cap64 + 63) / 64 * 64;
+  cap64 = slice_cap_of(ctx, cap64);
   if (cap64 * NB >= (1ull << 31))
     return fail(PENGK_ERR_RANGE, "shard too large for the partitioned count (slice of %llu keys)", (unsigned long long)cap64);
   const uint32_t slice_cap = (uint32_t)cap64;
   int rc = ensure_scratch(ctx, &ctx->d_keys, &ctx->keys_bytes, (size_t)NB * n_waves * slice_cap * sizeof(uint16_t));
   if (rc) return rc;
   const size_t fill_words = ((size_t)NB * n_waves + 63) / 64 * 64;
-  const size_t aux_need = fill_words * sizeof(uint32_t) + (size_t)np * sizeof(uint32_t);
-  rc = ensure_scratch(ctx, &ctx->d_count_aux, &ctx->count_aux_bytes, aux_need);
+  CountAux aux;
+  rc = count_aux_block(ctx, fill_words * sizeof(uint32_t) + (size_t)np * sizeof(uint32_t), &aux);
   if (rc) return rc;
   uint32_t* slice_fill = (uint32_t*)ctx->d_count_aux;
   uint32_t* temp = slice_fill + fill_words;
-  PENGK_HIP(hipMemsetAsync(ctx->d_count_aux, 0, aux_need, ctx->stream));
-  unsigned long long* lt = (unsigned long long*)d_ltot;
   uint16_t* keys = (uint16_t*)ctx->d_keys;
   uint32_t* bgp = nullptr;
   if (d_bg) {
@@ -1075,13 +1167,9 @@
   }
 #define TA_SCATTER(B, G) W, B, NBITS, G
   PENGK_LAUNCH_BB(count_scatter_kernel, TA_SCATTER, both, d_bg != nullptr, dim3(blocks), dim3(TPB), w32, ctx->d_items, n_items,
-                  keys, slice_cap, slice_fill, d_counts, lt, ctx->d_defer, bgp);
+                  keys, slice_cap, slice_fill, temp, aux.ltot_sum, aux.defer, bgp);
 #undef TA_SCATTER
   PENGK_HIP(hipGetLastError());
-  if (d_bg) {
-    rc = bg_finish_fused(ctx, blocks, d_bg);
-    if (rc) return rc;
-  }
   uint32_t bpb = ((uint32_t)ctx->num_cu * 2u + NB - 1) / NB;
   const uint64_t per_bucket = windows / NB + 1;
   const uint32_t useful = (uint32_t)((per_bucket + 65535) / 65536);
@@ -1091,8 +1179,12 @@
   hipLaunchKernelGGL(count_hist_kernel, dim3(NB * bpb), dim3(1024), 4 << PAYLOAD_BITS, ctx->stream, keys, slice_cap, n_waves,
                      NB, slice_fill, bpb, temp, 0u);
   PENGK_HIP(hipGetLastError());
+  rc = launch_fixup(ctx, both, temp, W, aux.defer, blocks, d_bg ? aux.bg_raw : nullptr);
+  if (rc) return rc;
   const uint32_t gb = (np + 255) / 256 < 2048u ? (np + 255) / 256 : 2048u;
-  hipLaunchKernelGGL((count_gather_kernel<W, NBITS>), dim3(gb), dim3(256), 0, ctx->stream, temp, np, d_counts);
+  hipLaunchKernelGGL((count_gather_kernel<W>), dim3(gb), dim3(256), 0, ctx->stream, (const uint32_t*)temp, d_counts,
+                     (const unsigned long long*)aux.ltot_sum, (unsigned long long*)d_ltot, (const unsigned long long*)aux.bg_raw,
+                     (unsigned long long*)d_bg);
   PENGK_HIP(hipGetLastError());
   return PENGK_OK;
 }
@@ -1110,8 +1202,7 @@
   const uint64_t windows = ctx->n_windows_hint ? ctx->n_windows_hint : ctx->n_items * (uint64_t)ctx->item_windows;
   uint64_t share1 = windows / ((uint64_t)NB1 * n_waves1);
   uint64_t cap1_64 = share1 + share1 / 2 + 256;
-  if (ctx->key_cap_override) cap1_64 = ctx->key_cap_override;
-  cap1_64 = (cap1_64 + 63) / 64 * 64;
+  cap1_64 = slice_cap_of(ctx, cap1_64);
   uint32_t bpb1 = ((uint32_t)ctx->num_cu * 8u + NB1 - 1u) / NB1;
   if (bpb1 > n_waves1) bpb1 = n_waves1;
   if (bpb1 < 1) bpb1 = 1;
@@ -1119,8 +1210,7 @@
   const uint32_t n_waves2 = blocks2 * 4u;
   uint64_t share2 = windows / ((uint64_t)NB2 * n_waves2);
   uint64_t cap2_64 = share2 + share2 / 2 + 512;
-  if (ctx->key_cap_override) cap2_64 = ctx->key_cap_override;
-  cap2_64 = (cap2_64 + 63) / 64 * 64;
+  cap2_64 = slice_cap_of(ctx, cap2_64);
   if (cap1_64 * NB1 >= (1ull << 30) || cap2_64 * NB2 >= (1ull << 31)) return fail(
       PENGK_ERR_RANGE, "shard too large for the partitioned count");
   const uint32_t cap1 = (uint32_t)cap1_64, cap2 = (uint32_t)cap2_64;
@@ -1131,14 +1221,12 @@
   uint32_t* keys1 = (uint32_t*)ctx->d_keys;
   uint16_t* keys2 = (uint16_t*)((char*)ctx->d_keys + bytes1);
   const size_t fill1_words = ((size_t)n_waves1 * NB1 + 63) / 64 * 64, fill2_words = ((size_t)n_waves2 * NB2 + 63) / 64 * 64;
-  const size_t aux_need = (fill1_words + fill2_words + (size_t)np) * sizeof(uint32_t);
-  rc = ensure_scratch(ctx, &ctx->d_count_aux, &ctx->count_aux_bytes, aux_need);
+  CountAux aux;
+  rc = count_aux_block(ctx, (fill1_words + fill2_words + (size_t)np) * sizeof(uint32_t), &aux);
   if (rc) return rc;
   uint32_t* fill1 = (uint32_t*)ctx->d_count_aux;
   uint32_t* fill2 = fill1 + fill1_words;
   uint32_t* temp = fill2 + fill2_words;
-  PENGK_HIP(hipMemsetAsync(ctx->d_count_aux, 0, aux_need, ctx->stream));
-  unsigned long long* lt = (unsigned long long*)d_ltot;
   uint32_t* bgp = nullptr;
   if (d_bg) {
     rc = bg_partials_buffer(ctx, blocks1, &bgp);
@@ -1146,20 +1234,20 @@
   }
 #define TA_S12(B, G) B, G
   PENGK_LAUNCH_BB(count_scatter12_kernel, TA_S12, both, d_bg != nullptr, dim3(blocks1), dim3(TPB1), w32, ctx->d_items, n_items, keys1,
-                  cap1, fill1, d_counts, lt, ctx->d_defer, bgp);
+                  cap1, fill1, temp, aux.ltot_sum, aux.defer, bgp);
 #undef TA_S12
   PENGK_HIP(hipGetLastError());
-  if (d_bg) {
-    rc = bg_finish_fused(ctx, blocks1, d_bg);
-    if (rc) return rc;
-  }
   hipLaunchKernelGGL(count_rescatter12_kernel, dim3(blocks2), dim3(256), 0, ctx->stream, keys1, cap1, fill1, n_waves1, bpb1, keys2,
-                     cap2, fill2, d_counts);
+                     cap2, fill2, temp);
   PENGK_HIP(hipGetLastError());
   hipLaunchKernelGGL(count_hist_kernel, dim3(512), dim3(1024), 4 << PAYLOAD_BITS, ctx->stream, keys2, cap2, n_waves2, NB2, fill2, 1u,
                      temp, bpb1 * 4u);
   PENGK_HIP(hipGetLastError());
-  hipLaunchKernelGGL(count_gather12_kernel, dim3(4096), dim3(256), 0, ctx->stream, temp, d_counts);
+  rc = launch_fixup(ctx, both, temp, 12, aux.defer, blocks1, d_bg ? aux.bg_raw : nullptr);
+  if (rc) return rc;
+  hipLaunchKernelGGL((count_gather_kernel<12>), dim3(4096), dim3(256), 0, ctx->stream, (const uint32_t*)temp, d_counts,
+                     (const unsigned long long*)aux.ltot_sum, (unsigned long long*)d_ltot, (const unsigned long long*)aux.bg_raw,
+                     (unsigned long long*)d_bg);
   PENGK_HIP(hipGetLastError());
   return PENGK_OK;
 }
@@ -1178,9 +1266,7 @@
   const uint64_t windows = ctx->n_windows_hint ? ctx->n_windows_hint : ctx->n_items * (uint64_t)ctx->item_windows;
   auto cap_of = [&](uint64_t slices, uint64_t slack) {
     uint64_t c = windows / slices;
-    c = c + c / 2 + slack;
-    if (ctx->key_cap_override) c = ctx->key_cap_override;
-    return (c + 63) / 64 * 64;
+    return slice_cap_of(ctx, c + c / 2 + slack);
   };
   uint32_t bpb1 = ((uint32_t)ctx->num_cu * 8u + NB1 - 1u) / NB1;
   if (bpb1 > n_waves1) bpb1 = n_waves1;
@@ -1204,15 +1290,13 @@
   uint16_t* keys3 = (uint16_t*)((char*)ctx->d_keys + bytes1 + bytes2);
   const size_t f1 = ((size_t)n_waves1 * NB1 + 63) / 64 * 64, f2 = ((size_t)n_waves2 * NB2 + 63) / 64 * 64,
                f3 = ((size_t)n_waves3 * NB3 + 63) / 64 * 64;
-  const size_t aux_need = (f1 + f2 + f3 + np) * sizeof(uint32_t);
-  rc = ensure_scratch(ctx, &ctx->d_count_aux, &ctx->count_aux_bytes, aux_need);
+  CountAux aux;
+  rc = count_aux_block(ctx, (f1 + f2 + f3 + np) * sizeof(uint32_t), &aux);
   if (rc) return rc;
   uint32_t* fill1 = (uint32_t*)ctx->d_count_aux;
   uint32_t* fill2 = fill1 + f1;
   uint32_t* fill3 = fill2 + f2;
   uint32_t* temp = fill3 + f3;
-  PENGK_HIP(hipMemsetAsync(ctx->d_count_aux, 0, aux_need, ctx->stream));
-  unsigned long long* lt = (unsigned long long*)d_ltot;
   uint32_t* bgp = nullptr;
   if (d_bg) {
     rc = bg_partials_buffer(ctx, blocks1, &bgp);
@@ -1220,23 +1304,23 @@
   }
 #define TA_S14(B, G) B, G
   PENGK_LAUNCH_BB(count_scatter14_kernel, TA_S14, both, d_bg != nullptr, dim3(blocks1), dim3(TPB1), w32, ctx->d_items, n_items, keys1,
-                  cap1, fill1, d_counts, lt, ctx->d_defer, bgp);
+                  cap1, fill1, temp, aux.ltot_sum, aux.defer, bgp);
 #undef TA_S14
   PENGK_HIP(hipGetLastError());
-  if (d_bg) {
-    rc = bg_finish_fused(ctx, blocks1, d_bg);
-    if (rc) return rc;
-  }
   hipLaunchKernelGGL((count_rescatter_kernel<Split14L2, uint32_t, NB1>), dim3(blocks2), dim3(256), 0, ctx->stream, keys1, cap1, fill1,
-                     n_waves1, 0u, bpb1, keys2, cap2, fill2, d_counts);
+                     n_waves1, 0u, bpb1, keys2, cap2, fill2, temp);
   PENGK_HIP(hipGetLastError());
   hipLaunchKernelGGL((count_rescatter_kernel<Split14L3, uint16_t, NB2>), dim3(blocks3), dim3(256), 0, ctx->stream, keys2, cap2, fill2,
-                     n_waves2, bpb1 * 4u, bpb2, keys3, cap3, fill3, d_counts);
+                     n_waves2, bpb1 * 4u, bpb2, keys3, cap3, fill3, temp);
   PENGK_HIP(hipGetLastError());
   hipLaunchKernelGGL(count_hist_kernel, dim3(8192), dim3(1024), 4 << PAYLOAD_BITS, ctx->stream, keys3, cap3, n_waves3, NB3, fill3, 1u,
                      temp, bpb2 * 4u);
   PENGK_HIP(hipGetLastError());
-  hipLaunchKernelGGL(count_gather14_kernel, dim3(8192), dim3(256), 0, ctx->stream, temp, d_counts);
+  rc = launch_fixup(ctx, both, temp, 14, aux.defer, blocks1, d_bg ? aux.bg_raw : nullptr);
+  if (rc) return rc;
+  hipLaunchKernelGGL((count_gather_kernel<14>), dim3(8192), dim3(256), 0, ctx->stream, (const uint32_t*)temp, d_counts,
+                     (const unsigned long long*)aux.ltot_sum, (unsigned long long*)d_ltot, (const unsigned long long*)aux.bg_raw,
+                     (unsigned long long*)d_bg);
   PENGK_HIP(hipGetLastError());
   return PENGK_OK;
 }
@@ -1245,6 +1329,9 @@
 int launch_count_w(pengk_ctx* ctx, int both, uint32_t* d_counts, uint64_t* d_ltot, uint64_t* d_bg) {
   const uint32_t n_items = (uint32_t)ctx->n_items;
   if (n_items == 0) {
+    ctx->d_defer_count = nullptr;
+    PENGK_HIP(hipMemsetAsync(d_counts, 0, ((size_t)1 << (2 * W)) * sizeof(uint32_t), ctx->stream));
+    PENGK_HIP(hipMemsetAsync(d_ltot, 0, sizeof(uint64_t), ctx->stream));
     if (d_bg) PENGK_HIP(hipMemsetAsync(d_bg, 0, 84 * sizeof(uint64_t), ctx->stream));
     return PENGK_OK;
   }
@@ -1272,11 +1359,7 @@
   } else {
     rc = launch_direct_w<W>(ctx, both, d_counts, d_ltot, n_items, d_bg);
   }
-  if (rc) return rc;
-  hipLaunchKernelGGL(count_fixup_kernel, dim3(64), dim3(64), 0, ctx->stream, (const uint32_t*)ctx->d_words, ctx->d_items, W,
-                     both, d_counts, ctx->d_defer);
-  PENGK_HIP(hipGetLastError());
-  return PENGK_OK;
+  return rc;
 }
 
 }
@@ -1288,19 +1371,6 @@
 
 int launch_count(pengk_ctx* ctx, int both, uint32_t* d_counts, uint64_t* d_ltot, uint64_t* d_bg) {
   const int W = ctx->W;
-  const size_t np = (size_t)1 << (2 * W);
-  {
-    const size_t need = (ctx->n_items + 2) * sizeof(uint32_t);
-    size_t have = ctx->defer_cap * sizeof(uint32_t);
-    if (have < need) {
-      int rc = ensure_scratch(ctx, (void**)&ctx->d_defer, &have, need);
-      if (rc) return rc;
-      ctx->defer_cap = have / sizeof(uint32_t);
-    }
-  }
-  PENGK_HIP(hipMemsetAsync(ctx->d_defer, 0, sizeof(uint32_t), ctx->stream));
-  PENGK_HIP(hipMemsetAsync(d_counts, 0, np * sizeof(uint32_t), ctx->stream));
-  PENGK_HIP(hipMemsetAsync(d_ltot, 0, sizeof(uint64_t), ctx->stream));
   switch (W) {
     case 2: return launch_count_w<2>(ctx, both, d_counts, d_ltot, d_bg);
     case 4: return launch_count_w<4>(ctx, both, d_counts, d_ltot, d_bg);
diff --git a/peng-motif_amd/csrc/em.hip b/peng-motif_amd/csrc/em.hip
--- a/peng-motif_amd/csrc/em.hip
+++ b/peng-motif_amd/csrc/em.hip
@@ -263,35 +263,6 @@
       }
       partials[((size_t)(pw0 + q) * G::NB + blockIdx.x) * G::CELLS + tid] = v;
     }
-  }
-}
-
-__global__ __launch_bounds__(1024) void em_bg_range_kernel(const float* __restrict__ bg, uint32_t np, uint32_t* __restrict__ range) {
-  __shared__ uint32_t s_lo[16], s_hi[16];
-  uint32_t lo = 0xFFFFFFFFu, hi = 0u;
-  const uint4* v = reinterpret_cast<const uint4*>(bg);
-  for (uint32_t i = blockIdx.x * 1024u + threadIdx.x; i < np / 4u; i += gridDim.x * 1024u) {
-    const uint4 b = v[i];
-    lo = min(min(lo, b.x), min(min(b.y, b.z), b.w));
-    hi = max(max(hi, b.x), max(max(b.y, b.z), b.w));
-  }
-#pragma unroll
-  for (int m = 1; m < 64; m <<= 1) {
-    lo = min(lo, (uint32_t)__shfl_xor((int)lo, m, 64));
-    hi = max(hi, (uint32_t)__shfl_xor((int)hi, m, 64));
-  }
-  if ((threadIdx.x & 63u) == 0u) {
-    s_lo[threadIdx.x >> 6] = lo;
-    s_hi[threadIdx.x >> 6] = hi;
-  }
-  __syncthreads();
-  if (threadIdx.x == 0) {
-    for (int w = 1; w < 16; ++w) {
-      lo = min(lo, s_lo[w]);
-      hi = max(hi, s_hi[w]);
-    }
-    atomicMin(range, lo);
-    atomicMax(range + 1, hi);
   }
 }
 
@@ -345,7 +316,8 @@
   __shared__ float part[4][28];
   __shared__ uint32_t s_lean;
   const uint32_t t = threadIdx.x, lane = t & 63u, wave = t >> 6;
-  const uint32_t bg_lo = bg_range[0], bg_hi = bg_range[1];
+  uint32_t bg_lo, bg_hi;
+  bg_range_load(bg_range, bg_lo, bg_hi);
   if (!fused_head<W>(fs, pw, k, threshold, max_it, sp == 0u, s_pwm, s_old, t)) return;
   uint32_t* bad = fs.bad + (size_t)(k & 1u) * fs.bad_stride;
   if (t == 0) s_lean = lean_ranges_ok<W>(s_pwm, bg_lo, bg_hi, saturation) ? 1u : 0u;
@@ -703,25 +675,54 @@
   }
 }
 
-__global__ __launch_bounds__(256) void em_serial_setup_kernel(uint32_t n, int W, float threshold, int max_it, int32_t* __restrict__ state,
-                                                             float* __restrict__ change, uint32_t* __restrict__ run,
-                                                             unsigned long long* __restrict__ counters, uint32_t* __restrict__ bg_range,
-                                                             uint32_t lean, uint32_t* __restrict__ bad, uint32_t bad_words) {
-  const uint32_t i = blockIdx.x * 256u + threadIdx.x;
-  if (i < (uint32_t)EM_COUNTERS) counters[i] = 0ull;
-  if (i == 0) {
-    bg_range[0] = lean ? 0xFFFFFFFFu : 0u;
-    bg_range[1] = lean ? 0u : 0xFFFFFFFFu;
-  }
-  for (uint32_t j = i; j < bad_words; j += gridDim.x * 256u) bad[j] = 0u;
-  if (i >= n) return;
+__global__ __launch_bounds__(1024) void em_prologue_kernel(uint32_t n, int W, float threshold, int max_it, int32_t* __restrict__ state,
+                                                           float* __restrict__ change, uint32_t* __restrict__ run,
+                                                           unsigned long long* __restrict__ counters, uint32_t* __restrict__ bg_range,
+                                                           uint32_t lean, uint32_t* __restrict__ bad, uint32_t bad_words,
+                                                           const float* __restrict__ bg, uint32_t np) {
+  const uint32_t i0 = blockIdx.x * 1024u + threadIdx.x, stride = gridDim.x * 1024u;
+  if (i0 < (uint32_t)EM_COUNTERS) counters[i0] = 0ull;
+  for (uint32_t j = i0; j < bad_words; j += stride) bad[j] = 0u;
   const float c0 = (float)W;
   const uint32_t r = !(c0 <= threshold || 0 >= max_it);
-  state[2 * i] = 0;
-  state[2 * i + 1] = (int32_t)r;
-  change[i] = c0;
-  run[i] = r;
-  run[n + i] = r;
+  for (uint32_t i = i0; i < n; i += stride) {
+    state[2 * i] = 0;
+    state[2 * i + 1] = (int32_t)r;
+    change[i] = c0;
+    run[i] = r;
+    run[n + i] = r;
+  }
+  __shared__ uint32_t s_lo[16], s_hi[16];
+  uint32_t lo = 0xFFFFFFFFu, hi = 0u;
+  if (lean) {
+    const uint4* v = reinterpret_cast<const uint4*>(bg);
+    for (uint32_t i = i0; i < np / 4u; i += stride) {
+      const uint4 b = v[i];
+      lo = min(min(lo, b.x), min(min(b.y, b.z), b.w));
+      hi = max(max(hi, b.x), max(max(b.y, b.z), b.w));
+    }
+  } else {
+    lo = 0u;
+    hi = 0xFFFFFFFFu;
+  }
+#pragma unroll
+  for (int m = 1; m < 64; m <<= 1) {
+    lo = min(lo, (uint32_t)__shfl_xor((int)lo, m, 64));
+    hi = max(hi, (uint32_t)__shfl_xor((int)hi, m, 64));
+  }
+  if ((threadIdx.x & 63u) == 0u) {
+    s_lo[threadIdx.x >> 6] = lo;
+    s_hi[threadIdx.x >> 6] = hi;
+  }
+  __syncthreads();
+  if (threadIdx.x == 0) {
+    for (int w = 1; w < 16; ++w) {
+      lo = min(lo, s_lo[w]);
+      hi = max(hi, s_hi[w]);
+    }
+    bg_range[2u * blockIdx.x] = lo;
+    bg_range[2u * blockIdx.x + 1u] = hi;
+  }
 }
 
 template <int W, int HIMAX, bool FAST, int P>
@@ -840,18 +841,17 @@
       ctx->em_epoch = 0;
     }
   }
-  if (!ctx->d_em_counters) PENGK_HIP(hipMalloc((void**)&ctx->d_em_counters, (EM_COUNTERS + 1) * sizeof(unsigned long long)));
+  if (!ctx->d_em_counters)
+    PENGK_HIP(hipMalloc((void**)&ctx->d_em_counters, (EM_COUNTERS + BG_RANGE_PARTS) * sizeof(unsigned long long)));
   uint32_t* bg_range = reinterpret_cast<uint32_t*>(ctx->d_em_counters + EM_COUNTERS);
   char* small = reinterpret_cast<char*>(ctx->d_em_partials);
   uint32_t* run = reinterpret_cast<uint32_t*>(small + run_at);
   float* pwm1 = reinterpret_cast<float*>(small + pwm1_at);
   {
     const uint32_t words = (uint32_t)((run_at - flags_at) / sizeof(uint32_t));
-    hipLaunchKernelGGL(em_serial_setup_kernel, dim3((unsigned)((std::max<int64_t>(n_pwm, 1024) + 255) / 256)), dim3(256), 0, ctx->stream,
-                       (uint32_t)n_pwm, W, threshold, max_it, d_state, d_change, run, ctx->d_em_counters, bg_range,
-                       ctx->em_lean_div ? 1u : 0u, reinterpret_cast<uint32_t*>(small + flags_at), words);
-    if (ctx->em_lean_div)
-      hipLaunchKernelGGL(em_bg_range_kernel, dim3(32), dim3(1024), 0, ctx->stream, d_bg, (uint32_t)np, bg_range);
+    hipLaunchKernelGGL(em_prologue_kernel, dim3(BG_RANGE_PARTS), dim3(1024), 0, ctx->stream, (uint32_t)n_pwm, W, threshold, max_it, d_state,
+                       d_change, run, ctx->d_em_counters, bg_range, ctx->em_lean_div ? 1u : 0u,
+                       reinterpret_cast<uint32_t*>(small + flags_at), words, d_bg, (uint32_t)np);
     PENGK_HIP(hipGetLastError());
   }
   if (max_it <= 0) return PENGK_OK;
@@ -1051,7 +1051,9 @@
 
 int launch_em(pengk_ctx* ctx, int W, int64_t n_pwm, float* d_pwms, float saturation, float threshold, int max_it,
               const uint32_t* d_counts, const float* d_bg, int32_t* d_state, float* d_change) {
-  if (ctx->d_em_counters) PENGK_HIP(hipMemsetAsync(ctx->d_em_counters, 0, EM_COUNTERS * sizeof(unsigned long long), ctx->stream));
+  const bool ahead = ctx->em_fast == 2 && W >= 10 && ctx->em_serial_scan >= 2;
+  if (ctx->d_em_counters && !ahead)
+    PENGK_HIP(hipMemsetAsync(ctx->d_em_counters, 0, EM_COUNTERS * sizeof(unsigned long long), ctx->stream));
   switch (W) {
     case 2:
       hipLaunchKernelGGL(em_init_kernel, dim3((unsigned)((n_pwm + 255) / 256)), dim3(256), 0, ctx->stream, (int)n_pwm, W, threshold, max_it,
diff --git a/peng-motif_amd/csrc/em_fused.hip b/peng-motif_amd/csrc/em_fused.hip
--- a/peng-motif_amd/csrc/em_fused.hip
+++ b/peng-motif_amd/csrc/em_fused.hip
@@ -37,7 +37,8 @@
   const uint32_t t = threadIdx.x, lane = t & 63u;
   const uint32_t wave = (uint32_t)__builtin_amdgcn_readfirstlane((int)(t >> 6));
   uint32_t* bad_now = fs.bad + (size_t)(k & 1u) * fs.bad_stride;
-  const uint32_t bg_lo = bg_range[0], bg_hi = bg_range[1];
+  uint32_t bg_lo, bg_hi;
+  bg_range_load(bg_range, bg_lo, bg_hi);
 
   const uint32_t sl = lin, slot = sl >> 3;
   const uint32_t pw = (sl & 7u) + 8u * (slot / G::SPANS), sp = slot % G::SPANS;
diff --git a/peng-motif_amd/csrc/em_serial.h b/peng-motif_amd/csrc/em_serial.h
--- a/peng-motif_amd/csrc/em_serial.h
+++ b/peng-motif_amd/csrc/em_serial.h
@@ -228,6 +228,16 @@
 }
 
 constexpr int EM_COUNTERS = 4;
+constexpr uint32_t BG_RANGE_PARTS = 32;
+__device__ __forceinline__ void bg_range_load(const uint32_t* __restrict__ parts, uint32_t& lo, uint32_t& hi) {
+  lo = 0xFFFFFFFFu;
+  hi = 0u;
+#pragma unroll
+  for (uint32_t i = 0; i < BG_RANGE_PARTS; ++i) {
+    lo = min(lo, parts[2u * i]);
+    hi = max(hi, parts[2u * i + 1u]);
+  }
+}
 struct FusedGeo {
   static constexpr uint32_t THREADS = 512, WAVES = 8, CHUNK = 64;
   static constexpr unsigned long long LOOKBACK_TICKS = 50000ull;
diff --git a/peng-motif_amd/csrc/pengk_internal.h b/peng-motif_amd/csrc/pengk_internal.h
--- a/peng-motif_amd/csrc/pengk_internal.h
+++ b/peng-motif_amd/csrc/pengk_internal.h
@@ -19,6 +19,7 @@
   int all_whole = 0;
   uint32_t* d_defer = nullptr;
   uint64_t defer_cap = 0;
+  const uint32_t* d_defer_count = nullptr;
   double* d_em_partials = nullptr;
   size_t em_partials_bytes = 0;
   float* d_em_tables = nullptr;
```

Result: no change. 536.7 (median of 6 runs) (+0.9%).
